# mitake/k8s

Measured on AMD Instinct MI355X. Metric: images/sec ResNet-50 TfJob (train, synthetic ImageNet), higher is better.
Workload: dtype bf16; 1 GPU; model=resnet50-v1.5, global_batch=3072, per_gpu_batch=3072, image_size=224, parallelism=dp1, optimizer=fused SGD momentum 0.9 (HIP)

## Files before the change

k8s_amd/csrc/binding/batchnorm.cpp:

```cpp
#include "binding/common.h"

namespace k8s_amd::binding {
namespace {

int bn_channels(const Tensor& x, const char* name, bool mult8) {
  check_bf16_dense(x, -1, name);
  TORCH_CHECK(x.dim() >= 1 && x.size(-1) > 0, name, ": channels last");
  const int C = (int)x.size(-1);
  TORCH_CHECK(!mult8 || C % 8 == 0, "channels must be a multiple of 8");
  return C;
}
void check_affine(const Tensor& gamma, const Tensor& beta, const Tensor& run_mean, const Tensor& run_var, long C) {
  check_channel_f32(gamma, C, "gamma"); check_channel_f32(beta, C, "beta");
  check_channel_f32(run_mean, C, "run_mean"); check_channel_f32(run_var, C, "run_var");
}
void check_bwd_vectors(const Tensor& mean, const Tensor& invstd, const Tensor& gamma, const Tensor& beta,
                       const Tensor& dgamma, const Tensor& dbeta, long C) {
  check_channel_f32(mean, C, "mean"); check_channel_f32(invstd, C, "invstd");
  check_channel_f32(gamma, C, "gamma"); check_channel_f32(beta, C, "beta");
  check_channel_f32(dgamma, C, "dgamma"); check_channel_f32(dbeta, C, "dbeta");
}
void check_same_shape(const Tensor& t, const Tensor& x, const char* name) {
  check_bf16_dense(t, -1, name);
  TORCH_CHECK(t.sizes() == x.sizes(), name, " must have the shape of x");
// ... 93 lines not shown
  if (want_link) {
    xarg = torch::empty({N, Ho, Wo, C}, x.options());
    ybits = torch::empty({(long)N * Ho * Wo * C / 8}, x.options().dtype(at::kByte));
  }
  launch_bn_relu_maxpool_fwd(cbf(x), f32(gamma), f32(beta), f32(sums), nrep, f32(mean), f32(invstd), f32(run_mean),
                             f32(run_var), f32(params), bf(y), idx.data_ptr<uint8_t>(), N, H, W, C, (float)eps,
                             (float)momentum, cur_stream(), want_link ? bf(xarg) : nullptr,
                             want_link ? ybits.data_ptr<uint8_t>() : nullptr);
  if (want_link) return {y, idx, mean, invstd, xarg, ybits};
  return {y, idx, mean, invstd};
}

Tensor pool_bn_bwd_impl(const Tensor& dpool, const Tensor& idx, const Tensor& x, const Tensor& mean,
                        const Tensor& invstd, const Tensor& gamma, const Tensor& beta, const Tensor& dgamma,
                        const Tensor& dbeta, const Tensor* sums) {
  check_bf16_dense(x, 4, "x");
  check_bf16_dense(dpool, 4, "dpool");
  check_cuda(idx, "idx"); check_dtype(idx, at::kByte, "idx");
  const int N = x.size(0), H = x.size(1), W = x.size(2), C = x.size(3);
  TORCH_CHECK(dpool.sizes() == idx.sizes() && dpool.size(0) == N && dpool.size(1) == (H + 1) / 2 &&
                  dpool.size(2) == (W + 1) / 2 && dpool.size(3) == C, "dpool / idx shape mismatch");
  check_bwd_vectors(mean, invstd, gamma, beta, dgamma, dbeta, C);
  const int nrep = sums ? check_stat_sums(*sums, C, "sums", true) : 0;
  auto dx = torch::empty_like(x);
  auto params = torch::empty({4 * C}, gamma.options());
  if (sums) {
    launch_pool_bn_bwd_from_sums(cbf(dpool), idx.data_ptr<uint8_t>(), cbf(x), f32(mean), f32(invstd), f32(gamma),
                                 f32(beta), bf(dx), f32(dgamma), f32(dbeta), f32(*sums), nrep, f32(params), N, H, W, C,
                                 cur_stream());
    return dx;
  }
  auto work = torch::empty({k8s_amd::pool_bn_workspace_floats(C)}, gamma.options());
  launch_pool_bn_bwd(cbf(dpool), idx.data_ptr<uint8_t>(), cbf(x), f32(mean), f32(invstd), f32(gamma), f32(beta), bf(dx),
                     f32(dgamma), f32(dbeta), f32(work), f32(params), N, H, W, C, cur_stream());
  return dx;
}
Tensor pool_bn_bwd_from_sums(Tensor dpool, Tensor idx, Tensor x, Tensor mean, Tensor invstd, Tensor gamma,
                             Tensor beta, Tensor dgamma, Tensor dbeta, Tensor sums) {
  return pool_bn_bwd_impl(dpool, idx, x, mean, invstd, gamma, beta, dgamma, dbeta, &sums);
}
Tensor pool_bn_bwd(Tensor dpool, Tensor idx, Tensor x, Tensor mean, Tensor invstd, Tensor gamma, Tensor beta,
                   Tensor dgamma, Tensor dbeta) {
  return pool_bn_bwd_impl(dpool, idx, x, mean, invstd, gamma, beta, dgamma, dbeta, nullptr);
}

std::vector<Tensor> bn_bwd_impl(const Tensor& dy, const Tensor& x, const OptTensor& y, const Tensor& mean,
                                const Tensor& invstd, const Tensor& gamma, const Tensor& beta, bool relu_x,
                                const Tensor& dgamma, const Tensor& dbeta, bool want_dres, const OptTensor& mask,
                                const Tensor* sums) {
  const int C = bn_channels(x, "x", false);
  const long M = x.numel() / C;
  check_same_shape(dy, x, "dy");
  check_bwd_vectors(mean, invstd, gamma, beta, dgamma, dbeta, C);
  const bool has_mask = mask && mask->defined();
  TORCH_CHECK(!(relu_x && (y || has_mask)) && !(y && has_mask), "relu_x, y and the packed mask are exclusive");
  const uint8_t* mk = has_mask ? check_bit_mask(*mask, x.numel(), "mask") : nullptr;
  const int nrep = sums ? check_stat_sums(*sums, C, "sums", false) : 0;
  Tensor ymask;
  if (y) {
    check_same_shape(*y, x, "y");
    TORCH_CHECK(x.numel() % 8 == 0, "y: a multiple of 8 elements to pack");
    ymask = relu_mask_for(x, true);
    launch_relu_mask(cbf(*y), ymask.data_ptr<uint8_t>(), x.numel() / 8, cur_stream());
    mk = ymask.data_ptr<uint8_t>();
  }
  auto dx = torch::empty_like(x);
  Tensor dres = want_dres ? torch::empty_like(x) : Tensor();
  uint16_t* dr = want_dres ? bf(dres) : nullptr;
  auto params = torch::empty({4 * C}, gamma.options());
  if (sums && mk) {
    launch_bn_bwd_from_sums(cbf(dy), cbf(x), mk, f32(*sums), nrep, f32(mean), f32(invstd), f32(gamma), f32(beta),
                            bf(dx), dr, f32(dgamma), f32(dbeta), f32(params), M, C, cur_stream());
  } else if (sums) {
    launch_bn_bwd_relu_from_sums(cbf(dy), cbf(x), f32(*sums), nrep, f32(mean), f32(invstd), f32(gamma), f32(beta),
                                 bf(dx), f32(dgamma), f32(dbeta), f32(params), M, C, cur_stream());
  } else {
    auto work = torch::empty({k8s_amd::bn_workspace_floats(M, C)}, gamma.options());
    launch_bn_bwd(cbf(dy), cbf(x), f32(mean), f32(invstd), f32(gamma), f32(beta), relu_x, bf(dx), dr, f32(dgamma),
                  f32(dbeta), f32(work), f32(params), M, C, cur_stream(), mk);
  }
  return {dx, dres};
}
std::vector<Tensor> bn_bwd(Tensor dy, Tensor x, OptTensor y, Tensor mean, Tensor invstd, Tensor gamma, Tensor beta,
                           bool relu_x, Tensor dgamma, Tensor dbeta, bool want_dres, OptTensor mask) {
  return bn_bwd_impl(dy, x, y, mean, invstd, gamma, beta, relu_x, dgamma, dbeta, want_dres, mask, nullptr);
}
std::vector<Tensor> bn_bwd_relu_from_sums(Tensor dy, Tensor x, Tensor sums, Tensor mean, Tensor invstd, Tensor gamma,
                                          Tensor beta, Tensor dgamma, Tensor dbeta) {
  return {bn_bwd_impl(dy, x, {}, mean, invstd, gamma, beta, true, dgamma, dbeta, false, {}, &sums)[0]};
}
std::vector<Tensor> bn_bwd_from_sums(Tensor dy, Tensor x, Tensor mask, Tensor sums, Tensor mean, Tensor invstd,
                                     Tensor gamma, Tensor beta, Tensor dgamma, Tensor dbeta, bool want_dres) {
  return bn_bwd_impl(dy, x, {}, mean, invstd, gamma, beta, false, dgamma, dbeta, want_dres, mask, &sums);
}

Tensor bn_bwd_params(Tensor dy, Tensor x, Tensor mask, OptTensor sums, Tensor mean, Tensor invstd, Tensor gamma,
                     Tensor beta, Tensor dgamma, Tensor dbeta) {
  const int C = bn_channels(x, "x", true);
  const long M = x.numel() / C;
  check_same_shape(dy, x, "dy");
  check_bwd_vectors(mean, invstd, gamma, beta, dgamma, dbeta, C);
  const uint8_t* mk = check_bit_mask(mask, x.numel(), "mask");
  const bool pre = sums && sums->defined();
  const int nrep = pre ? check_stat_sums(*sums, C, "sums", false) : 0;
  auto params = torch::empty({4 * C}, gamma.options());
  Tensor work;
  if (!pre) work = torch::empty({k8s_amd::bn_workspace_floats(M, C)}, gamma.options());
  launch_bn_bwd_params(cbf(dy), cbf(x), mk, pre ? f32(*sums) : nullptr, nrep, f32(mean), f32(invstd), f32(gamma),
                       f32(beta), false, f32(dgamma), f32(dbeta), pre ? nullptr : f32(work), f32(params), M, C,
                       cur_stream());
  return params;
}
Tensor bn_bwd_apply(Tensor dy, Tensor x, Tensor mask, Tensor params) {
  const int C = bn_channels(x, "x", true);
  check_same_shape(dy, x, "dy");
  const uint8_t* mk = check_bit_mask(mask, x.numel(), "mask");
  check_channel_f32(params, 4L * C, "params");
  TORCH_CHECK(params.device() == x.device(), "params: on x's device");
  auto dx = torch::empty_like(x);
  launch_bn_bwd_apply_pass(cbf(dy), cbf(x), mk, f32(params), false, bf(dx), nullptr, x.numel() / C, C, cur_stream());
  return dx;
}

std::vector<Tensor> bn_bwd_dual_impl(const Tensor& dy, const Tensor& mask, const Tensor& x, const Tensor& mean,
                                     const Tensor& invstd, const Tensor& gamma, const Tensor& beta,
                                     const Tensor& dgamma, const Tensor& dbeta, const Tensor* sums, const Tensor& x2,
                                     const Tensor& mean2, const Tensor& invstd2, const Tensor& gamma2,
                                     const Tensor& beta2, const Tensor& dgamma2, const Tensor& dbeta2,
                                     const Tensor* sums2) {
  const int C = bn_channels(x, "x", !sums);
  const long M = x.numel() / C;
  check_same_shape(dy, x, "dy");
  check_same_shape(x2, x, "x2");
  check_bwd_vectors(mean, invstd, gamma, beta, dgamma, dbeta, C);
  check_bwd_vectors(mean2, invstd2, gamma2, beta2, dgamma2, dbeta2, C);
  const uint8_t* mk = check_bit_mask(mask, x.numel(), "mask");
  const int nrep = sums ? check_stat_sums(*sums, C, "sums", false) : 0;
  TORCH_CHECK(!sums || check_stat_sums(*sums2, C, "sums2", false) == nrep, "sums / sums2: the same replica count");
  auto dx = torch::empty_like(x), dx2 = torch::empty_like(x);
  auto params = torch::empty({4 * C}, gamma.options()), params2 = torch::empty({4 * C}, gamma.options());
  if (sums) {
    launch_bn_bwd_dual_from_sums(cbf(dy), mk, cbf(x), f32(*sums), nrep, f32(mean), f32(invstd), f32(gamma), f32(beta),
                                 bf(dx), f32(dgamma), f32(dbeta), f32(params), cbf(x2), f32(*sums2), f32(mean2),
                                 f32(invstd2), f32(gamma2), f32(beta2), bf(dx2), f32(dgamma2), f32(dbeta2),
                                 f32(params2), M, C, cur_stream());
    return {dx, dx2};
  }
  auto work = torch::empty({k8s_amd::bn_workspace_floats(M, C)}, gamma.options());
  auto work2 = torch::empty({k8s_amd::bn_workspace_floats(M, C)}, gamma.options());
  launch_bn_bwd_dual(cbf(dy), mk, cbf(x), f32(mean), f32(invstd), f32(gamma), f32(beta), bf(dx), f32(dgamma),
                     f32(dbeta), f32(work), f32(params), cbf(x2), f32(mean2), f32(invstd2), f32(gamma2), f32(beta2),
                     bf(dx2), f32(dgamma2), f32(dbeta2), f32(work2), f32(params2), M, C, cur_stream());
  return {dx, dx2};
}
std::vector<Tensor> bn_bwd_dual(Tensor dy, Tensor mask, Tensor x, Tensor mean, Tensor invstd, Tensor gamma,
                                Tensor beta, Tensor dgamma, Tensor dbeta, Tensor x2, Tensor mean2, Tensor invstd2,
                                Tensor gamma2, Tensor beta2, Tensor dgamma2, Tensor dbeta2) {
  return bn_bwd_dual_impl(dy, mask, x, mean, invstd, gamma, beta, dgamma, dbeta, nullptr, x2, mean2, invstd2, gamma2,
                          beta2, dgamma2, dbeta2, nullptr);
}
std::vector<Tensor> bn_bwd_dual_from_sums(Tensor dy, Tensor mask, Tensor x, Tensor mean, Tensor invstd, Tensor gamma,
                                          Tensor beta, Tensor dgamma, Tensor dbeta, Tensor sums, Tensor x2,
                                          Tensor mean2, Tensor invstd2, Tensor gamma2, Tensor beta2, Tensor dgamma2,
                                          Tensor dbeta2, Tensor sums2) {
  return bn_bwd_dual_impl(dy, mask, x, mean, invstd, gamma, beta, dgamma, dbeta, &sums, x2, mean2, invstd2, gamma2,
                          beta2, dgamma2, dbeta2, &sums2);
}

}

void bind_batchnorm(pybind11::module_& m) {
  m.def("bn_fwd", &bn_fwd, "x"_a, "res"_a, "gamma"_a, "beta"_a, "run_mean"_a, "run_var"_a, "training"_a, "momentum"_a,
        "eps"_a, "relu"_a, "want_mask"_a = false);
  m.def("bn_bwd", &bn_bwd, "dy"_a, "x"_a, "y"_a, "mean"_a, "invstd"_a, "gamma"_a, "beta"_a, "relu_x"_a, "dgamma"_a,
        "dbeta"_a, "want_dres"_a, "mask"_a = py::none());
  m.def("bn_fwd_from_sums", &bn_fwd_from_sums, "x"_a, "res"_a, "gamma"_a, "beta"_a, "sums"_a, "run_mean"_a, "run_var"_a,
        "momentum"_a, "eps"_a, "relu"_a, "want_mask"_a = false, "want_sub2"_a = false);
  m.def("bn_bwd_dual", &bn_bwd_dual, "both BatchNorm backwards of bn_fwd_from_sums_dual from one masked dy");
  m.def("bn_fwd_from_sums_dual", &bn_fwd_from_sums_dual, "relu(BN(x) + BN_r(xr)), statistics from conv sums");
  m.def("bn_finalize", &bn_finalize, "sums"_a, "gamma"_a, "beta"_a, "run_mean"_a, "run_var"_a, "count"_a, "momentum"_a,
        "eps"_a);
  m.def("bn_bwd_relu_from_sums", &bn_bwd_relu_from_sums, "relu_x BatchNorm backward from a producer's sums");
  m.def("bn_bwd_from_sums", &bn_bwd_from_sums, "BatchNorm backward from a producer's reduction sums (final + apply)");
  m.def("bn_bwd_params", &bn_bwd_params, "dy"_a, "x"_a, "mask"_a, "sums"_a, "mean"_a, "invstd"_a, "gamma"_a, "beta"_a,
        "dgamma"_a, "dbeta"_a, "first half of a masked BatchNorm backward: dgamma, dbeta, params [sc | B | D | shift]");
  m.def("bn_bwd_apply", &bn_bwd_apply, "dy"_a, "x"_a, "mask"_a, "params"_a,
        "second half of a masked BatchNorm backward: dx from bn_bwd_params' table");
  m.def("bn_bwd_dual_from_sums", &bn_bwd_dual_from_sums, "bn_bwd_dual from a producer's reduction sums");
  m.def("bn_relu_maxpool", &bn_relu_maxpool, "x"_a, "sums"_a, "gamma"_a, "beta"_a, "run_mean"_a, "run_var"_a,
        "momentum"_a, "eps"_a, "want_link"_a = false);
  m.def("pool_bn_bwd_from_sums", &pool_bn_bwd_from_sums);
  m.def("pool_bn_bwd", &pool_bn_bwd, "dpool"_a, "idx"_a, "x"_a, "mean"_a, "invstd"_a, "gamma"_a, "beta"_a, "dgamma"_a,
        "dbeta"_a);
}

}
```

k8s_amd/csrc/binding/conv.cpp:

```cpp
#include "binding/common.h"

namespace k8s_amd::binding {
namespace {

int conv_out(int in, int k, int st, int pad, int dil) { return (in + 2 * pad - dil * (k - 1) - 1) / st + 1; }

struct ConvGeom {
  int N, H, W, C, K, R, S;
};
ConvGeom conv_geom(const Tensor& x, const Tensor& w) {
  TORCH_CHECK(x.dim() == 4 && w.dim() == 4, "x [N,H,W,C], w [K,R,S,C]");
  ConvGeom g{(int)x.size(0), (int)x.size(1), (int)x.size(2), (int)x.size(3),
             (int)w.size(0), (int)w.size(1), (int)w.size(2)};
  TORCH_CHECK(w.size(3) == g.C, "channel mismatch");
  TORCH_CHECK(g.C % 8 == 0 && g.K % 8 == 0, "implicit-GEMM conv needs C % 8 == 0 and K % 8 == 0");
  return g;
}
Tensor conv_fwd(Tensor x, Tensor w, int64_t stride, int64_t pad, int64_t dil, bool out_f32, OptTensor bias, int64_t act,
                OptTensor stats, OptTensor xform) {
  check_bf16(x, "x"); check_bf16(w, "w");
  const auto [N, H, W, C, K, R, S] = conv_geom(x, w);
  TORCH_CHECK(stride >= 1 && dil >= 1, "conv_fwd: stride >= 1, dilation >= 1");
  const int Ho = conv_out(H, R, stride, pad, dil), Wo = conv_out(W, S, stride, pad, dil);
  if (bias) check_channel_f32(*bias, K, "bias");
  if (stats) check_stat_sums(*stats, K, "stats", true);
  const float* xf = xform_ptr(xform, C);
  if (xf) TORCH_CHECK(C % 64 == 0 && !out_f32 && !bias && act == 0,
                      "normalize-on-load convolution: C % 64 == 0, bf16 output, no bias / activation");
  auto y = torch::empty({N, Ho, Wo, K}, x.options().dtype(out_f32 ? at::kFloat : at::kBFloat16));
  launch_conv_fwd(cbf(x), cbf(w), y.data_ptr(), out_f32, N, H, W, C, K, R, S, (int)stride, (int)pad, (int)dil, Ho, Wo,
                  optf(bias), (int)act, 0, stats ? f32(*stats) : nullptr, cur_stream(), nullptr, xf);
  return y;
}

Tensor conv_infer(Tensor x, Tensor w, int64_t stride, int64_t pad, Tensor scale, Tensor shift, OptTensor res,
                  bool relu, OptTensor out) {
  check_bf16_dense(x, 4, "x"); check_bf16_dense(w, 4, "w");
  const auto [N, H, W, C, K, R, S] = conv_geom(x, w);
  TORCH_CHECK(stride >= 1 && pad >= 0, "conv_infer: stride >= 1, pad >= 0");
  check_channel_f32(scale, K, "scale"); check_channel_f32(shift, K, "shift");
  TORCH_CHECK(H + 2 * pad >= R && W + 2 * pad >= S, "conv_infer: the filter does not fit the padded image");
  const int Ho = conv_out(H, R, stride, pad, 1), Wo = conv_out(W, S, stride, pad, 1);
  TORCH_CHECK((long)N * Ho * Wo < (1L << 31), "conv_infer: fewer than 2^31 output pixels");
  const std::vector<int64_t> oshape{N, Ho, Wo, K};
  if (out) {
    check_bf16_dense(*out, 4, "out");
    TORCH_CHECK(out->sizes().vec() == oshape, "out must be [N, Ho, Wo, K]");
  }
  if (res) {
    check_bf16_dense(*res, 4, "res");
    TORCH_CHECK(res->sizes().vec() == oshape, "res must have the output's shape [N, Ho, Wo, K]");
  }
  Tensor y = out ? *out : torch::empty(oshape, x.options());
  launch_conv_infer(cbf(x), cbf(w), bf(y), N, H, W, C, K, R, S, (int)stride, (int)pad, Ho, Wo, f32(scale), f32(shift),
                    res ? cbf(*res) : nullptr, relu, cur_stream());
  return y;
}

void conv_fwd_subgrid(Tensor x, Tensor w, int64_t pad, int64_t Hs, int64_t Ws, Tensor out, int64_t stride, int64_t a,
                      int64_t b, bool accumulate, OptTensor bn_x, OptTensor bn_mask, OptTensor bn_mean,
                      OptTensor bn_sums, OptTensor bn_gamma, OptTensor bn_beta, OptTensor bn_invstd) {
  check_bf16(x, "x"); check_bf16(w, "w"); check_bf16(out, "out");
  const auto [N, H, W, C, K, R, S] = conv_geom(x, w);
  TORCH_CHECK(out.dim() == 4 && out.size(0) == N && out.size(3) == K, "out shape");
  const int OH = out.size(1), OW = out.size(2);
  TORCH_CHECK(stride >= 1 && a >= 0 && a < stride && b >= 0 && b < stride, "parity out of range");
  TORCH_CHECK(Hs >= 1 && Ws >= 1 && (Hs - 1) * stride + a < OH && (Ws - 1) * stride + b < OW,
              "sub-grid exceeds the output image");
  k8s_amd::SubGrid sg{OH, OW, (int)stride, (int)a, (int)b};
  k8s_amd::BnBwdSums bb;
  if (bn_sums) {
    TORCH_CHECK(bn_x && bn_mean, "bn sums: bn_x and bn_mean");
    TORCH_CHECK(bn_mask ? accumulate : !accumulate,
                "bn sums: bn_mask + accumulate (a correction) or bn_gamma / bn_beta / bn_invstd + a plain store");
    TORCH_CHECK(bn_x->sizes() == out.sizes(), "bn_x: the shape of out");
    bb = bn_bwd_sums(*bn_x, *bn_mean, *bn_sums, bn_mask, bn_gamma, bn_beta, bn_invstd, {}, {}, {});
  }
  launch_conv_fwd(cbf(x), cbf(w), out.data_ptr(), false, N, H, W, C, K, R, S, 1, (int)pad, 1, (int)Hs, (int)Ws, nullptr,
                  0, accumulate ? 1 : 0, nullptr, cur_stream(), &sg, nullptr, bn_sums ? &bb : nullptr);
}

Tensor conv3x3_dgrad_bnstats(Tensor gy, Tensor wt, Tensor x, Tensor gamma, Tensor beta, Tensor mean, Tensor invstd,
                             Tensor sums) {
  check_bf16_dense(gy, 4, "gy"); check_bf16_dense(wt, 4, "wt"); check_bf16_dense(x, 4, "x");
  const int N = (int)gy.size(0), H = (int)gy.size(1), W = (int)gy.size(2), Kc = (int)gy.size(3);
  const int C = (int)wt.size(0);
  TORCH_CHECK(wt.size(1) == 3 && wt.size(2) == 3 && wt.size(3) == Kc, "wt: [C, 3, 3, K]");
  TORCH_CHECK(x.size(0) == N && x.size(1) == H && x.size(2) == W && x.size(3) == C, "x: the shape of dx");
  TORCH_CHECK(k8s_amd::conv3x3_eligible(H, W, Kc, C, 3, 3, 1, 1, 1), "conv3x3_dgrad_bnstats: outside the kernel");
  const k8s_amd::BnBwdSums bb = bn_bwd_sums(x, mean, sums, {}, gamma, beta, invstd, {}, {}, {});
  Tensor dx = torch::empty({N, H, W, C}, gy.options());
  launch_conv3x3(cbf(gy), cbf(wt), bf(dx), nullptr, nullptr, N, H, W, Kc, C, cur_stream(), &bb);
  return dx;
}

Tensor bwd1x1_fused(Tensor gy, Tensor x, Tensor w, Tensor xform, Tensor gamma, Tensor beta, Tensor mean, Tensor invstd,
                    Tensor dw, Tensor sums, bool accumulate, OptTensor x3, OptTensor mask, OptTensor params) {
  check_bf16_dense(gy, 2, "gy"); check_bf16_dense(x, 2, "x"); check_bf16_dense(w, 2, "w");
  const long M = gy.size(0), K = gy.size(1), C = x.size(1);
  TORCH_CHECK(x.size(0) == M && w.size(0) == K && w.size(1) == C, "shapes: gy [M, K], x [M, C], w [K, C]");
  TORCH_CHECK(k8s_amd::bwd1x1_fused_ok(M, (int)C, (int)K),
              "bwd1x1_fused: (C, K) = (64, 256) or (128, 512), 1 <= M < 2^31");
  check_cuda(dw, "dw"); check_dtype(dw, at::kFloat, "dw"); check_aligned(dw, "dw");
  TORCH_CHECK(dw.numel() == K * C, "dw must have K * C fp32 elements");
  check_channel_f32(xform, 2 * C, "xform (BatchNorm scale | shift)");
  const k8s_amd::BnBwdSums bb = bn_bwd_sums(x, mean, sums, {}, gamma, beta, invstd, {}, {}, {});
  k8s_amd::Bwd1x1Bn3 bn3;
  const bool onload = x3 || mask || params;
  if (onload) {
    TORCH_CHECK(x3 && mask && params, "bwd1x1_fused: x3, mask and params come together");
    check_bf16_dense(*x3, 2, "x3");
    TORCH_CHECK(x3->size(0) == M && x3->size(1) == K, "x3: the shape of gy, [M, K]");
    bn3.mask = check_bit_mask(*mask, M * K, "mask");
    check_aligned(*mask, "mask");
    check_cuda(*params, "params"); check_dtype(*params, at::kFloat, "params"); check_aligned(*params, "params");
    TORCH_CHECK(params->numel() >= 3 * K, "params: fp32 [sc | B | D], 3K elements or more");
    TORCH_CHECK(x3->device() == gy.device() && mask->device() == gy.device() && params->device() == gy.device(),
                "x3, mask and params: on gy's device");
    bn3.x3 = cbf(*x3);
    bn3.params = f32(*params);
  }
  Tensor dz = torch::empty({M, C}, gy.options());
  launch_bwd1x1_fused(cbf(gy), cbf(x), cbf(w), f32(xform), bb.gamma, bb.beta, bb.mean, bb.invstd, bf(dz), f32(dw),
                      bb.sums, M, (int)C, (int)K, accumulate, cur_stream(), onload ? &bn3 : nullptr);
  return dz;
}

void conv_wgrad(Tensor x, Tensor dy, Tensor dw, int64_t stride, int64_t pad, int64_t dil, int64_t splits,
                bool accumulate, OptTensor xform) {
  check_bf16(x, "x"); check_bf16(dy, "dy");
  check_cuda(dw, "dw"); check_dtype(dw, at::kFloat, "dw");
  const auto [N, H, W, C, K, R, S] = conv_geom(x, dw);
  TORCH_CHECK(stride >= 1 && dil >= 1, "conv_wgrad: stride >= 1, dilation >= 1");
  const int Ho = conv_out(H, R, stride, pad, dil), Wo = conv_out(W, S, stride, pad, dil);
  TORCH_CHECK(dy.dim() == 4 && dy.size(0) == N && dy.size(1) == Ho && dy.size(2) == Wo && dy.size(3) == K,
              "dy shape mismatch");
  const float* xf = xform_ptr(xform, C);
  if (dil == 1 && Ho == H && Wo == W && H == W && k8s_amd::wgrad3x3_tiled_ok(C, K, R, S, (int)stride, (int)pad, W)) {
    auto wsp = torch::empty({k8s_amd::wgrad3x3_tiled_workspace(N, H, W, C)}, dw.options());
    launch_wgrad3x3_tiled(cbf(x), cbf(dy), f32(wsp), f32(dw), N, H, W, C, accumulate, cur_stream(), xf);
    return;
  }
  if (!xf && dil == 1 && k8s_amd::wgrad_stream_eligible(N, Ho, Wo, C, K, R, S)) {
    launch_wgrad_stream(cbf(x), cbf(dy), f32(dw), N, H, W, C, K, R, S, (int)stride, (int)pad, Ho, Wo, accumulate,
                        cur_stream());
    return;
  }
  if (xf) TORCH_CHECK(C % 64 == 0, "normalize-on-load weight gradient needs C % 64 == 0");
  int sp = splits <= 0 ? k8s_amd::gemm_choose_splits(K, R * S * C, N * Ho * Wo) : (int)splits;
  Tensor ws;
  if (sp > 1) ws = torch::empty({k8s_amd::gemm_splitk_workspace(K, R * S * C, sp)}, dw.options());
  launch_conv_wgrad(cbf(x), cbf(dy), f32(dw), N, H, W, C, K, R, S, (int)stride, (int)pad, (int)dil, Ho, Wo, sp,
                    accumulate, sp > 1 ? f32(ws) : nullptr, cur_stream(), xf);
}

std::vector<Tensor> conv_dgrad_wsub(Tensor w, std::vector<std::vector<int64_t>> taps) {
  check_bf16(w, "w");
  TORCH_CHECK(w.dim() == 4, "w [K,R,S,C]");
  const int K = w.size(0), R = w.size(1), S = w.size(2), C = w.size(3);
  TORCH_CHECK(!taps.empty() && taps.size() <= 16, "1-16 parities");
  k8s_amd::DgradTaps t{};
  long off = 0;
  std::vector<int64_t> offs;
  for (size_t p = 0; p < taps.size(); ++p) {
    TORCH_CHECK(!taps[p].empty() && taps[p].size() <= 16, "1-16 taps per parity");
    t.n[p] = (int)taps[p].size();
    t.off[p] = off;
    offs.push_back(off);
    for (size_t i = 0; i < taps[p].size(); ++i) {
      TORCH_CHECK(taps[p][i] >= 0 && taps[p][i] < R * S, "tap index out of range");
      t.rs[p][i] = (int)taps[p][i];
    }
    off += (long)C * t.n[p] * K;
    off = (off + 7) / 8 * 8;
  }
  auto out = torch::empty({off}, w.options());
  launch_conv_dgrad_wsub(cbf(w), bf(out), K, R * S, C, t, (int)taps.size(), cur_stream());
  return {out, torch::tensor(offs)};
}
Tensor conv_dgrad_wtrans(Tensor w) {
  check_bf16(w, "w");
  TORCH_CHECK(w.dim() == 4, "w [K,R,S,C]");
  const int K = w.size(0), R = w.size(1), S = w.size(2), C = w.size(3);
  auto w2 = torch::empty({C, R, S, K}, w.options());
  launch_conv_dgrad_wtrans(cbf(w), bf(w2), K, R, S, C, cur_stream());
  return w2;
}

}

void bind_conv(pybind11::module_& m) {
  m.def("conv_fwd", &conv_fwd, "x"_a, "w"_a, "stride"_a, "pad"_a, "dil"_a, "out_f32"_a, "bias"_a, "act"_a, "stats"_a,
        "xform"_a = py::none());
  m.def("conv_infer", &conv_infer, "x"_a, "w"_a, "stride"_a, "pad"_a, "scale"_a, "shift"_a, "res"_a = py::none(),
        "relu"_a = true, "out"_a = py::none());
  m.def("conv3x3_staged_ok", [](int H, int W, int C, int K, int R, int S, int stride, int pad) {
    return k8s_amd::conv3x3_eligible(H, W, C, K, R, S, stride, pad, 1) &&
           k8s_amd::conv3x3_eligible(H, W, K, C, R, S, stride, pad, 1) &&
           k8s_amd::wgrad3x3_tiled_ok(C, K, R, S, stride, pad, W);
  });
  m.def("conv3x3_dgrad_bnstats", &conv3x3_dgrad_bnstats,
        "3x3 stride-1 data gradient with the BatchNorm-backward sums of a relu(BN(x)) input (conv3x3.hip)");
  m.def("conv_fwd_subgrid", &conv_fwd_subgrid, "x"_a, "w"_a, "pad"_a, "Hs"_a, "Ws"_a, "out"_a, "stride"_a, "a"_a, "b"_a,
        "accumulate"_a = false, "bn_x"_a = py::none(), "bn_mask"_a = py::none(), "bn_mean"_a = py::none(),
        "bn_sums"_a = py::none(), "bn_gamma"_a = py::none(), "bn_beta"_a = py::none(), "bn_invstd"_a = py::none());
  m.def("conv_wgrad", &conv_wgrad, "x"_a, "dy"_a, "dw"_a, "stride"_a, "pad"_a, "dil"_a, "splits"_a, "accumulate"_a,
        "xform"_a = py::none());
  m.def("bwd1x1_fused", &bwd1x1_fused, "gy"_a, "x"_a, "w"_a, "xform"_a, "gamma"_a, "beta"_a, "mean"_a, "invstd"_a,
        "dw"_a, "sums"_a, "accumulate"_a, "x3"_a = py::none(), "mask"_a = py::none(), "params"_a = py::none(),
        "1x1 data gradient, normalize-on-load weight gradient and BatchNorm-backward sums in one pass (bwd1x1_fused.hip)");
  m.def("bwd1x1_fused_ok", [](int64_t M, int64_t C, int64_t K) {
    return C <= 1024 && K <= 4096 && k8s_amd::bwd1x1_fused_ok(M, (int)C, (int)K);
  }, "M"_a, "C"_a, "K"_a, "whether bwd1x1_fused takes this shape");
  m.def("wgrad_stream_eligible",&k8s_amd::wgrad_stream_eligible, "tall-K weight-gradient kernel takes this shape");
  m.def("conv_dgrad_wtrans", &conv_dgrad_wtrans);
  m.def("conv_dgrad_wsub", &conv_dgrad_wsub);
}

}
```

k8s_amd/csrc/kernels/batchnorm.hip:

```cpp
#include <cstdlib>
#include <stdexcept>

#include "common.h"
#include "launchers.h"

namespace k8s_amd {


constexpr int BN_THREADS = 256;

struct BnGeom {
  int cgroups;
  int tpr;
  int rows_per_iter;
  int grid_y;
};

static inline BnGeom bn_geom(int C, long M) {
  BnGeom g;
  g.cgroups = C / 8;
  g.tpr = g.cgroups < BN_THREADS ? g.cgroups : BN_THREADS;
  const long cus = planner_cus();
  long nbx = M / 64;
  nbx = nbx < 1 ? 1 : (nbx > 4 * cus ? 4 * cus : nbx);
// ... 710 lines not shown

int stream_order_mode() { return 1; }
int stream_dir(int fixed) { return fixed; }

static long bn_rows_per_block(long M, const BnGeom& g) {
  long blocks_x = 4L * planner_cus() / g.grid_y;
  const long cap = M / 64;
  if (blocks_x > cap) blocks_x = cap;
  if (blocks_x < 1) blocks_x = 1;
  long rpb = (M + blocks_x - 1) / blocks_x;
  long minr = (long)g.rows_per_iter * 4;
  if (rpb < minr) rpb = minr;
  rpb = (rpb + g.rows_per_iter - 1) / g.rows_per_iter * g.rows_per_iter;
  return rpb;
}

static int bn_reduce_blocks(long M, const BnGeom& g) {
  long nb = 4L * planner_cus() / g.grid_y;
  const long groups = (M + g.rows_per_iter - 1) / g.rows_per_iter;
  if (nb > groups) nb = groups;
  if (stream_order_mode()) nb = nb < 8 ? 8 : nb & ~7L;
  return (int)(nb < 1 ? 1 : nb);
}

int bn_workspace_floats(long M, int C) {
  BnGeom g = bn_geom(C, M);
  long rpb = bn_rows_per_block(M, g);
  long nb = (M + rpb - 1) / rpb;
  const long nr = bn_reduce_blocks(M, g);
  return (int)((nb > nr ? nb : nr) * C * 2);
}

static void launch_bn_apply(const uint16_t* x, const uint16_t* res, const float* params, uint16_t* y, uint8_t* mask,
                            long M, int C, bool relu, hipStream_t st, const float* rparams = nullptr,
                            uint16_t* ysub = nullptr, int H = 1, int W = 1) {
  const long nvec = M * C / 8;
  if (nvec >= (1L << 31)) throw std::runtime_error("BatchNorm tensor too large (>= 2^31 vectors)");
  if (ysub && (M % ((long)H * W) != 0)) throw std::runtime_error("bn_apply subsample: M must be N * H * W");
  hipLaunchKernelGGL(bn_apply_kernel, dim3(cdiv(nvec, BN_THREADS)), dim3(BN_THREADS), 0, st, x, res, params, rparams,
                     y, mask, (int)nvec, C, make_fastdiv(C / 8), (int)relu,
                     stream_order_mode() ? (stream_dir(1) ? 1 : 2) : 0, ysub, make_fastdiv(W), make_fastdiv(H));
}

void launch_bn_fwd(const uint16_t* x, const uint16_t* res, const float* gamma, const float* beta, uint16_t* y,
                   float* save_mean, float* save_invstd, float* run_mean, float* run_var, float* work, float* params,
                   long M, int C, float eps, float momentum, bool training, bool relu, hipStream_t st,
                   uint8_t* mask) {
  if (training) {
    BnGeom g = bn_geom(C, M);
    long rpb = bn_rows_per_block(M, g);
    int nb = (int)((M + rpb - 1) / rpb);
    hipLaunchKernelGGL(bn_stats_kernel, dim3(nb, g.grid_y), dim3(BN_THREADS), 0, st, x, M, C, g.tpr,
                       g.rows_per_iter, rpb, work);
    hipLaunchKernelGGL(bn_stats_final_kernel, dim3(cdiv(C, FIN_CH)), dim3(256), 0, st, work, nb, M, rpb, C, eps,
                       momentum, save_mean, save_invstd, run_mean, run_var, gamma, beta, params);
  } else {
    hipLaunchKernelGGL(bn_eval_prep_kernel, dim3(cdiv(C, 256)), dim3(256), 0, st, run_mean, run_var, gamma, beta, C,
                       eps, save_mean, save_invstd, params);
  }
  launch_bn_apply(x, res, params, y, mask, M, C, relu, st);
}

void launch_bn_fwd_from_sums(const uint16_t* x, const uint16_t* res, const float* gamma, const float* beta,
                             uint16_t* y, const float* sums, int nrep, float* save_mean, float* save_invstd,
                             float* run_mean, float* run_var, float* params, long M, int C, float eps, float momentum,
                             bool relu, hipStream_t st, uint8_t* mask, uint16_t* ysub, int H, int W) {
  hipLaunchKernelGGL(bn_finalize_sums_kernel, dim3(cdiv(C, 256)), dim3(256), 0, st, sums, nrep, C, (float)M, eps,
                     momentum, save_mean, save_invstd, run_mean, run_var, gamma, beta, params);
  launch_bn_apply(x, res, params, y, mask, M, C, relu, st, nullptr, ysub, H, W);
}

void launch_bn_fwd_from_sums_dual(const uint16_t* x, const float* gamma, const float* beta, const float* sums,
                                  int nrep, float* save_mean, float* save_invstd, float* run_mean, float* run_var,
                                  float* params, const uint16_t* xr, const float* gamma_r, const float* beta_r,
                                  const float* sums_r, int nrep_r, float* save_mean_r, float* save_invstd_r,
                                  float* run_mean_r, float* run_var_r, float* params_r, uint16_t* y, uint8_t* mask,
                                  long M, int C, float eps, float momentum, hipStream_t st) {
  hipLaunchKernelGGL(bn_finalize_sums_kernel, dim3(cdiv(C, 256)), dim3(256), 0, st, sums, nrep, C, (float)M, eps,
                     momentum, save_mean, save_invstd, run_mean, run_var, gamma, beta, params);
  hipLaunchKernelGGL(bn_finalize_sums_kernel, dim3(cdiv(C, 256)), dim3(256), 0, st, sums_r, nrep_r, C, (float)M, eps,
                     momentum, save_mean_r, save_invstd_r, run_mean_r, run_var_r, gamma_r, beta_r, params_r);
  launch_bn_apply(x, xr, params, y, mask, M, C, true, st, params_r);
}

void launch_bn_finalize_sums(const float* gamma, const float* beta, const float* sums, int nrep, float* save_mean,
                             float* save_invstd, float* run_mean, float* run_var, float* params, long M, int C,
                             float eps, float momentum, hipStream_t st) {
  hipLaunchKernelGGL(bn_finalize_sums_kernel, dim3(cdiv(C, 256)), dim3(256), 0, st, sums, nrep, C, (float)M, eps,
                     momentum, save_mean, save_invstd, run_mean, run_var, gamma, beta, params);
}

static void launch_bn_bwd_apply(const uint16_t* dy, const uint16_t* x, const uint8_t* mask, const float* params,
                                bool relu_x, uint16_t* dx, uint16_t* dres, long M, int C, hipStream_t st,
                                int order = -1) {
  const long nvec = M * C / 8;
  if (nvec >= (1L << 31)) throw std::runtime_error("BatchNorm tensor too large (>= 2^31 vectors)");
  if (order < 0) order = stream_order_mode() ? (stream_dir(0) ? 1 : 2) : 0;
  hipLaunchKernelGGL(bn_bwd_apply_kernel, dim3(cdiv(nvec, BN_THREADS)), dim3(BN_THREADS), 0, st, dy, x, mask, params,
                     (int)relu_x, dx, dres, (int)nvec, C, make_fastdiv(C / 8), order);
}

void launch_bn_bwd_params(const uint16_t* dy, const uint16_t* x, const uint8_t* mask, const float* sums, int nrep,
                          const float* mean, const float* invstd, const float* gamma, const float* beta, bool relu_x,
                          float* dgamma, float* dbeta, float* work, float* params, long M, int C, hipStream_t st) {
  if (sums) {
    hipLaunchKernelGGL(bn_bwd_final_sums_kernel, dim3(cdiv(C, 256)), dim3(256), 0, st, sums, sums, nrep, C, dgamma,
                       dbeta, 1.f / (float)M, mean, invstd, gamma, beta, params);
    return;
  }
  BnGeom g = bn_geom(C, M);
  const int nb = bn_reduce_blocks(M, g);
  const int rdir = stream_dir(1);
  if (mask)
    hipLaunchKernelGGL(bn_bwd_reduce_kernel<true>, dim3(nb, g.grid_y), dim3(BN_THREADS), 0, st, dy, x, mean, invstd,
                       gamma, beta, (int)relu_x, M, C, g.tpr, g.rows_per_iter, work, mask, rdir);
  else
    hipLaunchKernelGGL(bn_bwd_reduce_kernel<false>, dim3(nb, g.grid_y), dim3(BN_THREADS), 0, st, dy, x, mean, invstd,
                       gamma, beta, (int)relu_x, M, C, g.tpr, g.rows_per_iter, work, mask, rdir);
  hipLaunchKernelGGL(bn_bwd_final_kernel, dim3(cdiv(C, FIN_CH)), dim3(256), 0, st, work, nb, C, dgamma, dbeta,
                     1.f / (float)M, mean, invstd, gamma, beta, params);
}

void launch_bn_bwd_apply_pass(const uint16_t* dy, const uint16_t* x, const uint8_t* mask, const float* params,
                              bool relu_x, uint16_t* dx, uint16_t* dres, long M, int C, hipStream_t st) {
  launch_bn_bwd_apply(dy, x, mask, params, relu_x, dx, dres, M, C, st);
}

void launch_bn_bwd(const uint16_t* dy, const uint16_t* x, const float* mean, const float* invstd, const float* gamma,
                   const float* beta, bool relu_x, uint16_t* dx, uint16_t* dres, float* dgamma, float* dbeta,
                   float* work, float* params, long M, int C, hipStream_t st, const uint8_t* mask) {
  launch_bn_bwd_params(dy, x, mask, nullptr, 0, mean, invstd, gamma, beta, relu_x, dgamma, dbeta, work, params, M, C,
                       st);
  launch_bn_bwd_apply(dy, x, mask, params, relu_x, dx, dres, M, C, st);
}

void launch_bn_bwd_from_sums(const uint16_t* dy, const uint16_t* x, const uint8_t* mask, const float* sums, int nrep,
                             const float* mean, const float* invstd, const float* gamma, const float* beta,
                             uint16_t* dx, uint16_t* dres, float* dgamma, float* dbeta, float* params, long M, int C,
                             hipStream_t st) {
  launch_bn_bwd_params(dy, x, mask, sums, nrep, mean, invstd, gamma, beta, false, dgamma, dbeta, nullptr, params, M,
                       C, st);
  launch_bn_bwd_apply(dy, x, mask, params, false, dx, dres, M, C, st);
}

void launch_bn_bwd_relu_from_sums(const uint16_t* dy, const uint16_t* x, const float* sums, int nrep,
                                  const float* mean, const float* invstd, const float* gamma, const float* beta,
                                  uint16_t* dx, float* dgamma, float* dbeta, float* params, long M, int C,
                                  hipStream_t st) {
  hipLaunchKernelGGL(bn_bwd_final_sums_kernel, dim3(cdiv(C, 256)), dim3(256), 0, st, sums, sums, nrep, C, dgamma,
                     dbeta, 1.f / (float)M, mean, invstd, gamma, beta, params);
  launch_bn_bwd_apply(dy, x, nullptr, params, true, dx, nullptr, M, C, st);
}

void launch_bn_bwd_dual_from_sums(const uint16_t* dy, const uint8_t* mask, const uint16_t* x, const float* sums,
                                  int nrep, const float* mean, const float* invstd, const float* gamma,
                                  const float* beta, uint16_t* dx, float* dgamma, float* dbeta, float* params,
                                  const uint16_t* x2, const float* sums2, const float* mean2, const float* invstd2,
                                  const float* gamma2, const float* beta2, uint16_t* dx2, float* dgamma2,
                                  float* dbeta2, float* params2, long M, int C, hipStream_t st) {
  hipLaunchKernelGGL(bn_bwd_final_sums_kernel, dim3(cdiv(C, 256)), dim3(256), 0, st, sums, sums, nrep, C, dgamma,
                     dbeta, 1.f / (float)M, mean, invstd, gamma, beta, params);
  hipLaunchKernelGGL(bn_bwd_final_sums_kernel, dim3(cdiv(C, 256)), dim3(256), 0, st, sums, sums2, nrep, C, dgamma2,
                     dbeta2, 1.f / (float)M, mean2, invstd2, gamma2, beta2, params2);
  const long nvec = M * C / 8;
  if (nvec >= (1L << 31)) throw std::runtime_error("BatchNorm tensor too large (>= 2^31 vectors)");
  hipLaunchKernelGGL(bn_bwd_apply_dual_kernel, dim3(cdiv(nvec, BN_THREADS)), dim3(BN_THREADS), 0, st, dy, mask, x,
                     params, dx, x2, params2, dx2, (int)nvec, C, make_fastdiv(C / 8),
                     stream_order_mode() ? (stream_dir(0) ? 1 : 2) : 0);
}

void launch_bn_bwd_dual(const uint16_t* dy, const uint8_t* mask, const uint16_t* x, const float* mean,
                        const float* invstd, const float* gamma, const float* beta, uint16_t* dx, float* dgamma,
                        float* dbeta, float* work, float* params, const uint16_t* x2, const float* mean2,
                        const float* invstd2, const float* gamma2, const float* beta2, uint16_t* dx2, float* dgamma2,
                        float* dbeta2, float* work2, float* params2, long M, int C, hipStream_t st) {
  BnGeom g = bn_geom(C, M);
  const int nb = bn_reduce_blocks(M, g);
  const int rdir = stream_dir(1);
  hipLaunchKernelGGL((bn_bwd_reduce_kernel<true, true>), dim3(nb, g.grid_y), dim3(BN_THREADS), 0, st, dy, x, mean,
                     invstd, gamma, beta, 0, M, C, g.tpr, g.rows_per_iter, work, mask, rdir, x2, mean2, invstd2, work2);
  hipLaunchKernelGGL(bn_bwd_final_kernel, dim3(cdiv(C, FIN_CH)), dim3(256), 0, st, work, nb, C, dgamma, dbeta,
                     1.f / (float)M, mean, invstd, gamma, beta, params);
  hipLaunchKernelGGL(bn_bwd_final_kernel, dim3(cdiv(C, FIN_CH)), dim3(256), 0, st, work2, nb, C, dgamma2, dbeta2,
                     1.f / (float)M, mean2, invstd2, gamma2, beta2, params2);
  const long nvec = M * C / 8;
  if (nvec >= (1L << 31)) throw std::runtime_error("BatchNorm tensor too large (>= 2^31 vectors)");
  hipLaunchKernelGGL(bn_bwd_apply_dual_kernel, dim3(cdiv(nvec, BN_THREADS)), dim3(BN_THREADS), 0, st, dy, mask, x,
                     params, dx, x2, params2, dx2, (int)nvec, C, make_fastdiv(C / 8),
                     stream_order_mode() ? (stream_dir(0) ? 1 : 2) : 0);
}

void launch_bn_relu_maxpool_fwd(const uint16_t* x, const float* gamma, const float* beta, const float* sums, int nrep,
                                float* save_mean, float* save_invstd, float* run_mean, float* run_var, float* params,
                                uint16_t* y, uint8_t* idx, int N, int H, int W, int C, float eps, float momentum,
                                hipStream_t st, uint16_t* xarg, uint8_t* ybits) {
  const int Ho = (H + 1) / 2, Wo = (W + 1) / 2;
  const long total = (long)N * Ho * Wo * (C / 8);
  if ((long)N * H * W * C / 8 >= (1L << 31)) throw std::runtime_error("bn_relu_maxpool: tensor too large");
  hipLaunchKernelGGL(bn_finalize_sums_kernel, dim3(cdiv(C, 256)), dim3(256), 0, st, sums, nrep, C,
                     (float)((long)N * H * W), eps, momentum, save_mean, save_invstd, run_mean, run_var, gamma, beta,
                     params);
  hipLaunchKernelGGL(bn_relu_maxpool_fwd_kernel, dim3(cdiv(total, BN_THREADS)), dim3(BN_THREADS), 0, st, x, params,
                     y, idx, H, W, C, Ho, Wo, (int)total, make_fastdiv(C / 8), make_fastdiv(Wo), make_fastdiv(Ho),
                     xarg, ybits);
}

int pool_bn_workspace_floats(int C) { return 4096 * C * 2; }

void launch_pool_bn_bwd(const uint16_t* dpool, const uint8_t* idx, const uint16_t* x, const float* mean,
                        const float* invstd, const float* gamma, const float* beta, uint16_t* dx, float* dgamma,
                        float* dbeta, float* work, float* params, int N, int H, int W, int C, hipStream_t st) {
  if (C % 8 || BN_THREADS % (C / 8)) throw std::runtime_error("pool_bn_bwd: C / 8 must divide 256");
  const int Ho = (H + 1) / 2, Wo = (W + 1) / 2, Hc = (H + 1) / 2, Wc = (W + 1) / 2;
  const long ncells = (long)N * Hc * Wc;
  if (ncells * (C / 8) >= (1L << 31)) throw std::runtime_error("pool_bn_bwd: tensor too large");
  const int cpb = BN_THREADS / (C / 8);
  long nb = (ncells + cpb - 1) / cpb;
  nb = std::min(nb, 16L * planner_cus());
  hipLaunchKernelGGL(pool_bn_bwd_reduce_kernel, dim3((unsigned)nb), dim3(BN_THREADS), 0, st, dpool, idx, x, mean,
                     invstd, gamma, beta, H, W, C, Ho, Wo, Hc, Wc, (int)ncells, work, make_fastdiv(Wc),
                     make_fastdiv(Hc));
  hipLaunchKernelGGL(bn_bwd_final_kernel, dim3(cdiv(C, FIN_CH)), dim3(256), 0, st, work, (int)nb, C, dgamma, dbeta,
                     1.f / (float)((long)N * H * W), mean, invstd, gamma, beta, params);
  const long total = ncells * (C / 8);
  hipLaunchKernelGGL(pool_bn_bwd_apply_kernel, dim3(cdiv(total, BN_THREADS)), dim3(BN_THREADS), 0, st, dpool, idx, x,
                     params, dx, H, W, C, Ho, Wo, (int)total, make_fastdiv(C / 8), make_fastdiv(Wc),
                     make_fastdiv(Hc));
}

void launch_pool_bn_bwd_from_sums(const uint16_t* dpool, const uint8_t* idx, const uint16_t* x, const float* mean,
                                  const float* invstd, const float* gamma, const float* beta, uint16_t* dx,
                                  float* dgamma, float* dbeta, const float* sums, int nrep, float* params, int N,
                                  int H, int W, int C, hipStream_t st) {
  if (C % 8 || BN_THREADS % (C / 8)) throw std::runtime_error("pool_bn_bwd: C / 8 must divide 256");
  const int Ho = (H + 1) / 2, Wo = (W + 1) / 2, Hc = (H + 1) / 2, Wc = (W + 1) / 2;
  const long ncells = (long)N * Hc * Wc;
  if (ncells * (C / 8) >= (1L << 31)) throw std::runtime_error("pool_bn_bwd: tensor too large");
  hipLaunchKernelGGL(bn_bwd_final_sums_kernel, dim3(cdiv(C, 256)), dim3(256), 0, st, sums, sums, nrep, C, dgamma,
                     dbeta, 1.f / (float)((long)N * H * W), mean, invstd, gamma, beta, params);
  const long total = ncells * (C / 8);
  hipLaunchKernelGGL(pool_bn_bwd_apply_kernel, dim3(cdiv(total, BN_THREADS)), dim3(BN_THREADS), 0, st, dpool, idx, x,
                     params, dx, H, W, C, Ho, Wo, (int)total, make_fastdiv(C / 8), make_fastdiv(Wc),
                     make_fastdiv(Hc));
}

__global__ void __launch_bounds__(BN_THREADS) relu_mask_kernel(const uint16_t* __restrict__ y,
                                                               uint8_t* __restrict__ mask, int nvec) {
  const int e = blockIdx.x * BN_THREADS + threadIdx.x;
  if (e < nvec) mask[e] = relu_bits(*reinterpret_cast<const bf16x8_t*>(y + (long)e * 8));
}

void launch_relu_mask(const uint16_t* y, uint8_t* mask, long nvec, hipStream_t st) {
  if (nvec >= (1L << 31)) throw std::runtime_error("tensor too large (>= 2^31 vectors)");
  hipLaunchKernelGGL(relu_mask_kernel, dim3(cdiv(nvec, BN_THREADS)), dim3(BN_THREADS), 0, st, y, mask, (int)nvec);
}

__global__ void __launch_bounds__(BN_THREADS) mask_apply_kernel(const uint16_t* __restrict__ src,
                                                                const uint8_t* __restrict__ mask,
                                                                uint16_t* __restrict__ out, int nvec) {
  const int e = blockIdx.x * BN_THREADS + threadIdx.x;
  if (e >= nvec) return;
  bf16x8_t v = *reinterpret_cast<const bf16x8_t*>(src + (long)e * 8);
  const uint32_t bits = mask[e];
#pragma unroll
  for (int r = 0; r < 8; ++r) v[r] = ((bits >> r) & 1u) ? v[r] : (short)0;
  *reinterpret_cast<bf16x8_t*>(out + (long)e * 8) = v;
}

void launch_mask_apply(const uint16_t* src, const uint8_t* mask, uint16_t* out, long n, hipStream_t st) {
  if (n % 8) throw std::runtime_error("mask_apply: element count must be a multiple of 8");
  const long nvec = n / 8;
  if (nvec >= (1L << 31)) throw std::runtime_error("tensor too large (>= 2^31 vectors)");
  hipLaunchKernelGGL(mask_apply_kernel, dim3(cdiv(nvec, BN_THREADS)), dim3(BN_THREADS), 0, st, src, mask, out,
                     (int)nvec);
}

}
```

k8s_amd/csrc/kernels/bwd1x1_fused.hip:

```cpp
#include <algorithm>
#include <stdexcept>

#include "common.h"
#include "launchers.h"
#include "mfma.h"

namespace k8s_amd {
namespace b1f {

constexpr int THREADS = 512;
constexpr int CT = 64;

__device__ __attribute__((aligned(64))) uint16_t g_zero16[64];

typedef __attribute__((ext_vector_type(4))) int int4_t;

__device__ __forceinline__ int swz128(int r) { return 2 * (((r >> 1) & 1) | (((r >> 3) & 1) << 1)); }
__device__ __forceinline__ int swz_g(int r) { return (2 * ((r & 3) | (((r >> 3) & 1) << 2))) | ((r >> 2) & 1); }

struct TrRaw {
  short4_t lo, hi;
};
template <int RB, bool G>
__device__ __forceinline__ void tr_load(TrRaw& r, const char* img, int rb, int kk, int lane) {
  const int g = lane >> 4, i = lane & 15, q = i >> 2, p = i & 3;
  const int u = (rb >> 3) + (p >> 1);
  const int r0 = kk * 32 + 8 * g + q, r1 = r0 + 4;
  const int u0 = u ^ (G ? swz_g(r0) : swz128(r0)), u1 = u ^ (G ? swz_g(r1) : swz128(r1));
  tr16_asm(r.lo, img + r0 * RB + (u0 << 4) + (p & 1) * 8);
  tr16_asm(r.hi, img + r1 * RB + (u1 << 4) + (p & 1) * 8);
}
#define K8S_LDS_TIE4(w, a, b, c, d) asm volatile(w : "+v"(a), "+v"(b), "+v"(c), "+v"(d))

struct Args {
  const uint16_t *gy, *x, *w;
  const uint16_t* x3;
  const uint8_t* mask;
  const float* params;
  const float *xform, *gamma, *beta, *mean, *invstd;
  uint16_t* dz;
  float* dw;
  float* sums;
  int M, C, ntiles, npairs;
};

__device__ __forceinline__ void lds_barrier() {
  asm volatile("s_waitcnt lgkmcnt(0)" ::: "memory");
  __builtin_amdgcn_s_barrier();
  asm volatile("" ::: "memory");
}

template <int K, int RS, int NSLOT, int HALVES, bool ONLOAD>
__global__ void __launch_bounds__(THREADS, 1) bwd1x1_fused_kernel(Args a) {
  constexpr int RB = K * 2, UG = K / 8;
  constexpr int IMG_G = RS * RB, IMG_X = RS * 128;
  constexpr int IMG_M = ONLOAD ? RS * UG : 0;
  constexpr int OFF_X = IMG_G + (ONLOAD ? IMG_G + IMG_M : 0);
  constexpr int STAGE = OFF_X + IMG_X, RING = NSLOT * STAGE;
  constexpr int LG = RS * UG / THREADS;
  constexpr int LPS = ONLOAD ? 2 * LG : LG;
  constexpr bool TREG = ONLOAD && (THREADS / UG) % 16 == 0;
  constexpr bool TLDS = ONLOAD && !TREG;
  static_assert(!ONLOAD || (IMG_M % 1024 == 0 && IMG_M / 1024 <= THREADS / 64), "mask tile: whole 1-KB wave loads");
  constexpr int XT = RS * 8;
  constexpr int NKS = K / 32, KW = K / 8, KTW = KW / 16;
  static_assert(LG * THREADS == RS * UG && XT % 64 == 0 && XT <= THREADS && (RS == 32 || RS == 64), "tile");
  static_assert(XT * 64 <= RING, "sums partials reuse the ring");
  constexpr bool PLDS = K > 256;
  __shared__ __attribute__((aligned(1024))) char smem[RING + IMG_X + (PLDS ? 5 * CT * 4 : 0) + (TLDS ? 3 * K * 4 : 0)];
  static_assert(sizeof(smem) <= 160 * 1024, "LDS");
  char* stg = smem + RING;
  float* ptab = reinterpret_cast<float*>(stg + IMG_X);
  float* btab = ptab + (PLDS ? 5 * CT : 0);

  const int tid = threadIdx.x, lane = tid & 63;
  const int wid = __builtin_amdgcn_readfirstlane(tid >> 6);
  const int bid = blockIdx.x;
  int pair = bid, chalf = 0;
  if constexpr (HALVES == 2) {
    const int slot = bid >> 3;
    chalf = slot & 1;
    pair = (slot >> 1) * 8 + (bid & 7);
  }
  const int c0 = chalf * CT;
  const int n = pair < a.ntiles ? (a.ntiles - pair + a.npairs - 1) / a.npairs : 0;
  if (n == 0) return;
  const long M = a.M;
  const int C = a.C;

  const int ct = wid & 3, rh = wid >> 2;
  int4_t wf[NKS];
  {
    const uint16_t* wp = a.w + (long)(8 * (lane >> 4)) * C + c0 + ct * 16 + (lane & 15);
#pragma unroll
    for (int ks = 0; ks < NKS; ++ks) {
      bf16x8_t v;
#pragma unroll
      for (int j = 0; j < 8; ++j) v[j] = (short)wp[(long)(ks * 32 + j) * C];
      wf[ks] = __builtin_bit_cast(int4_t, v);
    }
  }
  const int erow = tid >> 3;
  const int eu = (tid & 7) ^ swz128(erow);
  const int ecol = c0 + eu * 8;
  float xsc[8], xsh[8], gsc[8], gsh[8], mu[8], ps[8], pq[8];
#pragma unroll
  for (int j = 0; j < 8; ++j) {
    xsc[j] = a.xform[ecol + j];
    xsh[j] = a.xform[C + ecol + j];
    mu[j] = a.mean[ecol + j];
    bn_affine_regs(a.gamma[ecol + j], a.beta[ecol + j], mu[j], a.invstd[ecol + j], gsc[j], gsh[j]);
    ps[j] = pq[j] = 0.f;
  }
  if constexpr (PLDS) {
    if (tid < 8) {
#pragma unroll
      for (int j = 0; j < 8; ++j) {
        ptab[0 * CT + tid * 8 + j] = xsc[j];
        ptab[1 * CT + tid * 8 + j] = xsh[j];
        ptab[2 * CT + tid * 8 + j] = gsc[j];
        ptab[3 * CT + tid * 8 + j] = gsh[j];
        ptab[4 * CT + tid * 8 + j] = mu[j];
      }
    }
  }
  const int tup = tid % UG, trow = tid / UG;
  float tsc[8], tB[8], tD[8];
  if constexpr (TREG) {
    const float* t = a.params + (tup ^ swz_g(trow)) * 8;
#pragma unroll
    for (int j = 0; j < 8; ++j) {
      tsc[j] = t[j];
      tB[j] = t[K + j];
      tD[j] = t[2 * K + j];
    }
#pragma unroll
    for (int j = 0; j < 8; ++j) asm volatile("" : "+v"(tsc[j]), "+v"(tB[j]), "+v"(tD[j]));
  }
  if constexpr (TLDS) {
    static_assert(!TLDS || PLDS, "the table's stores are ordered by the PLDS barrier");
    for (int i = tid; i < 3 * K; i += THREADS) btab[i] = a.params[i];
  }
#pragma unroll
  for (int ks = 0; ks < NKS; ++ks) asm volatile("" : "+v"(wf[ks]));
  if constexpr (!PLDS) {
#pragma unroll
    for (int j = 0; j < 8; ++j) asm volatile("" : "+v"(xsc[j]), "+v"(xsh[j]), "+v"(gsc[j]), "+v"(gsh[j]), "+v"(mu[j]));
  } else {
    __syncthreads();
  }

  auto issue = [&](int slot, int i) {
    char* st = smem + slot * STAGE;
    const long m0 = (long)(pair + i * a.npairs) * RS;
    if constexpr (ONLOAD) {
      const unsigned last = (unsigned)min((long)RS - 1, M - 1 - m0);
      const uint16_t* gb = a.gy + m0 * K;
      const uint16_t* xb = a.x3 + m0 * K;
#pragma unroll
      for (int j = 0; j < LG; ++j) {
        const unsigned row = j * (THREADS / UG) + trow;
        const unsigned off = min(row, last) * K + (tup ^ swz_g(row)) * 8;
        glds16(gb + off, st + j * (THREADS * 16) + wid * 1024);
        glds16(xb + off, st + IMG_G + j * (THREADS * 16) + wid * 1024);
      }
      if (wid < IMG_M / 1024) {
        const unsigned q = (wid * 64 + lane) * 16;
        glds16(a.mask + m0 * UG + min(q / UG, last) * UG + q % UG, st + 2 * IMG_G + wid * 1024);
      }
      if (wid < XT / 64) glds16(a.x + m0 * C + min((unsigned)erow, last) * C + ecol, st + OFF_X + wid * 1024);
      return;
    }
#pragma unroll
    for (int j = 0; j < LG; ++j) {
      const int sl = j * THREADS + tid, row = sl / UG, up = sl % UG;
      const int u = up ^ swz_g(row);
      const long m = m0 + row;
      const void* src = m < M ? (const void*)(a.gy + m * K + u * 8) : (const void*)g_zero16;
      glds16(src, st + j * (THREADS * 16) + wid * 1024);
    }
    if (wid < XT / 64) {
      const long m = m0 + erow;
      const void* src = m < M ? (const void*)(a.x + m * C + ecol) : (const void*)g_zero16;
      glds16(src, st + OFF_X + wid * 1024);
    }
  };

  f32x4_t dwa[KTW][4];
#pragma unroll
  for (int i = 0; i < KTW; ++i)
#pragma unroll
    for (int j = 0; j < 4; ++j) dwa[i][j] = f32x4_t{0.f, 0.f, 0.f, 0.f};

  const int pre = min(n, NSLOT - 1);
  for (int s = 0; s < pre; ++s) issue(s, s);
  int slot = 0;
  for (int s = 0; s < n; ++s) {
    const int younger = min(n - 1, s + NSLOT - 2) - s;
    if (younger >= 2) asm volatile("s_waitcnt vmcnt(%0)" ::"n"(2 * LPS) : "memory");
    else if (younger == 1) asm volatile("s_waitcnt vmcnt(%0)" ::"n"(LPS) : "memory");
    else asm volatile("s_waitcnt vmcnt(0)" ::: "memory");
    lds_barrier();
    if (s + NSLOT - 1 < n) issue(slot == 0 ? NSLOT - 1 : slot - 1, s + NSLOT - 1);
    char* G = smem + slot * STAGE;
    char* X = G + OFF_X;

    if constexpr (ONLOAD) {
      const int last = (int)min((long)RS - 1, M - 1 - (long)(pair + s * a.npairs) * RS);
#pragma unroll
      for (int j = 0; j < LG; ++j) {
        const int row = j * (THREADS / UG) + trow;
        const int u = tup ^ swz_g(row);
        char* gp = G + j * (THREADS * 16) + tid * 16;
        const bf16x8_t gv = *reinterpret_cast<const bf16x8_t*>(gp);
        const bf16x8_t xv = *reinterpret_cast<const bf16x8_t*>(gp + IMG_G);
        const uint32_t bits = *reinterpret_cast<const uint8_t*>(G + 2 * IMG_G + row * UG + u);
        float o[8];
#pragma unroll
        for (int h = 0; h < 8; h += 4) {
          if constexpr (TLDS) {
            const float* t = btab + u * 8 + h;
#pragma unroll
            for (int i = 0; i < 4; ++i) {
              tsc[h + i] = t[i];
              tB[h + i] = t[K + i];
              tD[h + i] = t[2 * K + i];
            }
          }
#pragma unroll
          for (int i = h; i < h + 4; ++i) {
            const float g = (bits >> i) & 1u ? bf2f((uint16_t)gv[i]) : 0.f;
            o[i] = __builtin_fmaf(tsc[i], g, __builtin_fmaf(tB[i], bf2f((uint16_t)xv[i]), tD[i]));
            o[i] = row <= last ? o[i] : 0.f;
          }
          if constexpr (TLDS) asm volatile("" ::: "memory");
        }
        *reinterpret_cast<bf16x8_t*>(gp) = pack_bf16x8(o);
      }
      lds_barrier();
    }

    {
      f32x4_t d0 = {0.f, 0.f, 0.f, 0.f}, d1 = {0.f, 0.f, 0.f, 0.f};
      const int row0 = rh * (RS / 2) + (lane & 15);
      const int kq = lane >> 4;
      if constexpr (RS == 64) {
        const int row1 = row0 + 16;
        const char* p0 = G + row0 * RB;
        const char* p1 = G + row1 * RB;
        const int s0 = swz_g(row0), s1 = swz_g(row1);
#pragma unroll
        for (int ks = 0; ks < NKS; ++ks) {
          const bf16x8_t b0 = *reinterpret_cast<const bf16x8_t*>(p0 + (((ks * 4 + kq) ^ s0) << 4));
          const bf16x8_t b1 = *reinterpret_cast<const bf16x8_t*>(p1 + (((ks * 4 + kq) ^ s1) << 4));
          const mfma_bf16x8 wa = __builtin_bit_cast(mfma_bf16x8, wf[ks]);
          d0 = mfma16(wa, __builtin_bit_cast(mfma_bf16x8, b0), d0);
          d1 = mfma16(wa, __builtin_bit_cast(mfma_bf16x8, b1), d1);
        }
      } else {
        const char* p0 = G + row0 * RB;
        const int s0 = swz_g(row0);
#pragma unroll
        for (int ks = 0; ks < NKS; ks += 2) {
          const bf16x8_t b0 = *reinterpret_cast<const bf16x8_t*>(p0 + (((ks * 4 + kq) ^ s0) << 4));
          const bf16x8_t b1 = *reinterpret_cast<const bf16x8_t*>(p0 + (((ks * 4 + 4 + kq) ^ s0) << 4));
          d0 = mfma16(__builtin_bit_cast(mfma_bf16x8, wf[ks]), __builtin_bit_cast(mfma_bf16x8, b0), d0);
          d1 = mfma16(__builtin_bit_cast(mfma_bf16x8, wf[ks + 1]), __builtin_bit_cast(mfma_bf16x8, b1), d1);
        }
        d0 += d1;
      }
      const int unit = ct * 2 + (lane >> 5), half = (lane >> 4) & 1;
      auto put = [&](int row, const f32x4_t& d) {
        bf16x4_t o;
#pragma unroll
        for (int r = 0; r < 4; ++r) o[r] = (short)f2bf(d[r]);
        *reinterpret_cast<bf16x4_t*>(stg + row * 128 + ((unit ^ swz128(row)) << 4) + half * 8) = o;
      };
      put(row0, d0);
      if constexpr (RS == 64) put(row0 + 16, d1);
    }
    lds_barrier();

    if (wid < XT / 64) {
      const bf16x8_t dzv = *reinterpret_cast<const bf16x8_t*>(stg + tid * 16);
      const bf16x8_t xv = *reinterpret_cast<const bf16x8_t*>(X + tid * 16);
      if constexpr (PLDS) {
        const float* t = ptab + (ecol - c0);
#pragma unroll
        for (int j = 0; j < 8; ++j) {
          xsc[j] = t[j];
          xsh[j] = t[CT + j];
          gsc[j] = t[2 * CT + j];
          gsh[j] = t[3 * CT + j];
          mu[j] = t[4 * CT + j];
        }
      }
      float o[8];
#pragma unroll
      for (int j = 0; j < 8; ++j) {
        const float xf = bf2f((uint16_t)xv[j]);
        o[j] = fmaxf(__builtin_fmaf(xf, xsc[j], xsh[j]), 0.f);
        const float g = relu_on(xf, gsc[j], gsh[j]) ? bf2f((uint16_t)dzv[j]) : 0.f;
        ps[j] += g;
        pq[j] = __builtin_fmaf(g, xf - mu[j], pq[j]);
      }
      *reinterpret_cast<bf16x8_t*>(X + tid * 16) = pack_bf16x8(o);
      const long m = (long)(pair + s * a.npairs) * RS + erow;
      if (m < M) *reinterpret_cast<bf16x8_t*>(a.dz + m * C + ecol) = dzv;
    }
    lds_barrier();

#pragma unroll
    for (int kk = 0; kk < RS / 32; ++kk) {
      TrRaw ar[KTW], br[4];
#pragma unroll
      for (int j = 0; j < 4; ++j) tr_load<128, false>(br[j], X, j * 16, kk, lane);
#pragma unroll
      for (int i = 0; i < KTW; ++i) tr_load<RB, true>(ar[i], G, wid * KW + i * 16, kk, lane);
      K8S_LDS_TIE8("s_waitcnt lgkmcnt(0)", br[0].lo, br[0].hi, br[1].lo, br[1].hi, br[2].lo, br[2].hi, br[3].lo,
                   br[3].hi);
#pragma unroll
      for (int i = 0; i < KTW; i += 2)
        K8S_LDS_TIE4("s_waitcnt lgkmcnt(0)", ar[i].lo, ar[i].hi, ar[i + 1].lo, ar[i + 1].hi);
#pragma unroll
      for (int i = 0; i < KTW; ++i)
#pragma unroll
        for (int j = 0; j < 4; ++j)
          dwa[i][j] = __builtin_amdgcn_mfma_f32_16x16x32_bf16(join8(br[j].lo, br[j].hi), join8(ar[i].lo, ar[i].hi),
                                                              dwa[i][j], 0, 0, 0);
    }
    slot = slot + 1 == NSLOT ? 0 : slot + 1;
  }

#pragma unroll
  for (int i = 0; i < KTW; ++i) {
    const int k = wid * KW + i * 16 + (lane & 15);
#pragma unroll
    for (int j = 0; j < 4; ++j) {
      float* d = a.dw + (long)k * C + c0 + j * 16 + 4 * (lane >> 4);
#pragma unroll
      for (int r = 0; r < 4; ++r) atomicAdd(d + r, dwa[i][j][r]);
    }
  }
  __syncthreads();
  float* part = reinterpret_cast<float*>(smem);
  if (tid < XT) {
#pragma unroll
    for (int j = 0; j < 8; ++j) {
      part[tid * 16 + j] = ps[j];
      part[tid * 16 + 8 + j] = pq[j];
    }
  }
  __syncthreads();
  if (tid < 2 * CT) {
    const int col = tid & (CT - 1), which = tid / CT;
    const int u = col >> 3, r = col & 7;
    float v = 0.f;
#pragma unroll 4
    for (int row = 0; row < RS; ++row) v += part[(row * 8 + (u ^ swz128(row))) * 16 + which * 8 + r];
    atomicAdd(a.sums + (long)(bid % kConvStatReplicas) * 2 * C + (long)which * C + c0 + col, v);
  }
}

}

bool bwd1x1_fused_ok(long M, int C, int K) {
  return M >= 1 && M < (1L << 31) && ((C == 64 && K == 256) || (C == 128 && K == 512));
}

void launch_bwd1x1_fused(const uint16_t* gy, const uint16_t* x, const uint16_t* w, const float* xform,
                         const float* gamma, const float* beta, const float* mean, const float* invstd, uint16_t* dz,
                         float* dw, float* sums, long M, int C, int K, bool accumulate, hipStream_t st,
                         const Bwd1x1Bn3* bn3) {
  using namespace b1f;
  if (!bwd1x1_fused_ok(M, C, K)) throw std::runtime_error("bwd1x1_fused: (C, K) = (64, 256) or (128, 512), M < 2^31");
  if (bn3 && !(bn3->x3 && bn3->mask && bn3->params)) throw std::runtime_error("bwd1x1_fused: x3, mask and params");
  if (!accumulate) (void)hipMemsetAsync(dw, 0, (size_t)K * C * sizeof(float), st);
  Args a{gy, x, w, nullptr, nullptr, nullptr, xform, gamma, beta, mean, invstd, dz, dw, sums, (int)M, C, 0, 0};
  if (bn3) a.x3 = bn3->x3, a.mask = bn3->mask, a.params = bn3->params;
  const int cus = std::max(1, planner_cus());
  if (C == 64) {
    a.ntiles = (int)((M + 63) / 64);
    a.npairs = cus;
    if (bn3) hipLaunchKernelGGL((bwd1x1_fused_kernel<256, 64, 2, 1, true>), dim3(cus), dim3(THREADS), 0, st, a);
    else hipLaunchKernelGGL((bwd1x1_fused_kernel<256, 64, 3, 1, false>), dim3(cus), dim3(THREADS), 0, st, a);
  } else {
    const int grid = std::max(16, cus / 16 * 16);
    a.ntiles = (int)((M + 31) / 32);
    a.npairs = grid / 2;
    if (bn3) hipLaunchKernelGGL((bwd1x1_fused_kernel<512, 32, 2, 2, true>), dim3(grid), dim3(THREADS), 0, st, a);
    else hipLaunchKernelGGL((bwd1x1_fused_kernel<512, 32, 4, 2, false>), dim3(grid), dim3(THREADS), 0, st, a);
  }
}

}
```

k8s_amd/csrc/kernels/launchers.h:

```cpp
#pragma once
#include <hip/hip_runtime.h>
#include <stdint.h>

#include "rng.h"

namespace k8s_amd {

int planner_cus();
void set_planner_cus(int n);

void launch_sgd(float* p, float* mom, const void* g, bool g_bf16, uint16_t* pbf, long n, const uint8_t* decay_mask, float lr,
                float mu, float wd, float scale, const float* scale_ptr, const float* hyper, bool nesterov,
                bool first_step, hipStream_t st);
void launch_adam(float* p, float* m1, float* m2, const void* g, bool g_bf16, uint16_t* pbf, long n, const uint8_t* decay_mask,
                 float lr, float b1, float b2, float eps, float wd, float scale, const float* scale_ptr,
                 const float* hyper, float bc1, float bc2, bool decoupled, hipStream_t st);
void launch_sumsq(const void* g, bool g_bf16, long n, float* out, hipStream_t st);
void launch_clip_factor(const float* stats, float max_norm, float* factor, hipStream_t st);
void launch_slice_sum(const uint16_t* in, long n, int world, float* out, uint16_t* out_bf, hipStream_t st);
void launch_cast_bf16(const float* in, uint16_t* out, long n, hipStream_t st);

void launch_grad_accumulate(float* acc, const float* g, long n, bool first, hipStream_t st);
void launch_grad_fold(float* g, const float* acc, uint16_t* out_bf, long n, hipStream_t st);

constexpr int kLayerItemMax = 16384;
void launch_layer_sums(const long* items, int n_items, const float* p, float* m1, float* m2, const void* g,
                       bool g_bf16, const uint8_t* flags, float* partial, bool lamb, float b1, float b2, float eps,
                       float wd, float scale, const float* scale_ptr, const float* hyper, float bc1, float bc2,
                       hipStream_t st);
void launch_layer_fold(const float* partial, const int* seg_start, int n_seg, float* sums, const float* scale_ptr,
                       hipStream_t st);
void launch_layer_ratio(const float* sums, const uint8_t* flags, int n_seg, float* ratio, bool lamb, float eta,
                        float wd, const float* scale_ptr, hipStream_t st);
void launch_layer_update(const long* items, int n_items, float* p, float* m1, const float* m2, const void* g,
                         bool g_bf16, uint16_t* pbf, const uint8_t* flags, const float* ratio, bool lamb, float lr,
                         float mu, float b1, float b2, float eps, float wd, float scale, const float* scale_ptr,
                         const float* hyper, float bc1, float bc2, bool first_step, hipStream_t st);

int bn_workspace_floats(long M, int C);
void launch_bn_fwd(const uint16_t* x, const uint16_t* res, const float* gamma, const float* beta, uint16_t* y,
                   float* save_mean, float* save_invstd, float* run_mean, float* run_var, float* work, float* params,
                   long M, int C, float eps, float momentum, bool training, bool relu, hipStream_t st,
                   uint8_t* mask = nullptr);
void launch_bn_fwd_from_sums(const uint16_t* x, const uint16_t* res, const float* gamma, const float* beta,
                             uint16_t* y, const float* sums, int nrep, float* save_mean, float* save_invstd,
                             float* run_mean, float* run_var, float* params, long M, int C, float eps, float momentum,
                             bool relu, hipStream_t st, uint8_t* mask = nullptr, uint16_t* ysub = nullptr,
                             int H = 1, int W = 1);
void launch_bn_fwd_from_sums_dual(const uint16_t* x, const float* gamma, const float* beta, const float* sums,
                                  int nrep, float* save_mean, float* save_invstd, float* run_mean, float* run_var,
                                  float* params, const uint16_t* xr, const float* gamma_r, const float* beta_r,
                                  const float* sums_r, int nrep_r, float* save_mean_r, float* save_invstd_r,
                                  float* run_mean_r, float* run_var_r, float* params_r, uint16_t* y, uint8_t* mask,
                                  long M, int C, float eps, float momentum, hipStream_t st);
void launch_bn_bwd_from_sums(const uint16_t* dy, const uint16_t* x, const uint8_t* mask, const float* sums, int nrep,
                             const float* mean, const float* invstd, const float* gamma, const float* beta,
                             uint16_t* dx, uint16_t* dres, float* dgamma, float* dbeta, float* params, long M, int C,
                             hipStream_t st);
void launch_bn_bwd_relu_from_sums(const uint16_t* dy, const uint16_t* x, const float* sums, int nrep,
                                  const float* mean, const float* invstd, const float* gamma, const float* beta,
                                  uint16_t* dx, float* dgamma, float* dbeta, float* params, long M, int C,
                                  hipStream_t st);
void launch_bn_bwd_dual_from_sums(const uint16_t* dy, const uint8_t* mask, const uint16_t* x, const float* sums,
                                  int nrep, const float* mean, const float* invstd, const float* gamma,
                                  const float* beta, uint16_t* dx, float* dgamma, float* dbeta, float* params,
                                  const uint16_t* x2, const float* sums2, const float* mean2, const float* invstd2,
                                  const float* gamma2, const float* beta2, uint16_t* dx2, float* dgamma2,
                                  float* dbeta2, float* params2, long M, int C, hipStream_t st);
void launch_bn_bwd_dual(const uint16_t* dy, const uint8_t* mask, const uint16_t* x, const float* mean,
                        const float* invstd, const float* gamma, const float* beta, uint16_t* dx, float* dgamma,
                        float* dbeta, float* work, float* params, const uint16_t* x2, const float* mean2,
                        const float* invstd2, const float* gamma2, const float* beta2, uint16_t* dx2, float* dgamma2,
                        float* dbeta2, float* work2, float* params2, long M, int C, hipStream_t st);
void launch_bn_finalize_sums(const float* gamma, const float* beta, const float* sums, int nrep, float* save_mean,
                             float* save_invstd, float* run_mean, float* run_var, float* params, long M, int C,
                             float eps, float momentum, hipStream_t st);
constexpr int kConvStatReplicas = 32;
void launch_bn_bwd(const uint16_t* dy, const uint16_t* x, const float* mean, const float* invstd, const float* gamma,
                   const float* beta, bool relu_x, uint16_t* dx, uint16_t* dres, float* dgamma, float* dbeta,
                   float* work, float* params, long M, int C, hipStream_t st, const uint8_t* mask = nullptr);
void launch_bn_bwd_params(const uint16_t* dy, const uint16_t* x, const uint8_t* mask, const float* sums, int nrep,
                          const float* mean, const float* invstd, const float* gamma, const float* beta, bool relu_x,
                          float* dgamma, float* dbeta, float* work, float* params, long M, int C, hipStream_t st);
void launch_bn_bwd_apply_pass(const uint16_t* dy, const uint16_t* x, const uint8_t* mask, const float* params,
                              bool relu_x, uint16_t* dx, uint16_t* dres, long M, int C, hipStream_t st);
void launch_relu_mask(const uint16_t* y, uint8_t* mask, long nvec, hipStream_t st);

void launch_norm_fwd(bool rms, const uint16_t* x, const uint16_t* res, uint16_t* xsum, const float* gamma,
                     const float* beta, uint16_t* y, float* mean, float* rstd, long R, int D, float eps,
                     hipStream_t st, const DropArgs* drop = nullptr);
int norm_workspace_floats(long R, int D);
void launch_norm_bwd(bool rms, const uint16_t* dy, const uint16_t* x, const float* gamma, const float* mean,
                     const float* rstd, const uint16_t* dres, uint16_t* dx, float* dgamma, float* dbeta, float* work,
                     long R, int D, hipStream_t st, float* dsum = nullptr, const DropArgs* drop = nullptr,
                     uint16_t* da = nullptr);

void launch_dropout(const uint16_t* x, uint16_t* y, long R, int D, const DropArgs& dr, hipStream_t st);
void launch_dropout_mask(uint8_t* out, long row0, long R, int C, const DropArgs& dr, hipStream_t st);

void launch_xent_fwd(const void* logits, bool bf16, const int64_t* labels, long R, long V, long ld, float* loss,
                     float* lse, long ignore_index, float smoothing, hipStream_t st);
void launch_xent_bwd(const void* logits, bool bf16, const int64_t* labels, const float* lse, const float* dscale,
                     bool per_row, long R, long V, long ld, void* dlogits, long ignore_index, float smoothing,
                     hipStream_t st);
void launch_xent_eval(const void* logits, bool bf16, const int64_t* labels, long R, long V, long ld, float* loss,
                      int* rank, long ignore_index, hipStream_t st);

int gemm_choose_splits(int M, int N, int K);
struct AddEpi {
  const uint16_t* src;
  const uint8_t* mask;
};
bool gemm_short_ok(int M, int N, int K, long lda, long ldc);
bool gemm_short_bnstats_ok(int M, int N, int K, bool dual);
struct BnBwdSums {
  const uint16_t* x = nullptr;
  const float* gamma = nullptr;
  const float* beta = nullptr;
  const float* mean = nullptr;
  const float* invstd = nullptr;
  float* sums = nullptr;
  const uint8_t* mask = nullptr;
  const uint16_t* x2 = nullptr;
  const float* mean2 = nullptr;
  float* sums2 = nullptr;
};
struct GemmShortBnStats {
  const uint16_t* x = nullptr;
  const uint8_t* mask = nullptr;
  const float* mean = nullptr;
  float* sums = nullptr;
  const uint16_t* x2 = nullptr;
  const float* mean2 = nullptr;
  float* sums2 = nullptr;
};
void launch_gemm_short(const uint16_t* A, const uint16_t* B, long ldb, bool b_mn, uint16_t* C, const uint16_t* add,
                       const uint8_t* mask, const float* xf, float* stats, int M, int N, int K, int epi,
                       hipStream_t st, const GemmShortBnStats* bst = nullptr);
void launch_gemm_dgrad_bnstats(const uint16_t* A, const uint16_t* B, uint16_t* C, int M, int N, int K,
                               const BnBwdSums& bb, hipStream_t st, bool accumulate = false,
                               const uint16_t* add_src = nullptr, const uint8_t* add_mask = nullptr);
void launch_gemm(const uint16_t* A, long lda, bool a_kmajor, const uint16_t* B, long ldb, bool b_kmajor, void* C,
                 long ldc, bool c_f32, int M, int N, int K, const float* bias, int act, uint16_t* pre, int mode,
                 float alpha, int splits, float* ws, hipStream_t st, const AddEpi* add = nullptr,
                 const float* xform_b = nullptr, int xform_c = 0);
void launch_mask_apply(const uint16_t* src, const uint8_t* mask, uint16_t* out, long n, hipStream_t st);
long gemm_splitk_workspace(int M, int N, int splits);
bool conv3x3_eligible(int H, int W, int C, int K, int R, int S, int stride, int pad, int dil);
void launch_conv3x3(const uint16_t* x, const uint16_t* w, uint16_t* y, float* stats, const float* xform, int N,
                    int H, int W, int C, int K, hipStream_t st,
                    const BnBwdSums* bsums = nullptr);
bool gemm256_eligible(int M, int N, int K, bool a_kmajor, bool b_kmajor);
int gemm256_choose_splits(int M, int N, int K);
bool gemm_w4_dact_ok(int M, int N, int K, long lda, long ldb, long ldc);
long gemm_w4_dact_part_floats(int M, int N);
void launch_gemm_w4_dact(const uint16_t* A, long lda, const uint16_t* B, long ldb, uint16_t* C, long ldc, int M, int N,
                         int K, const uint16_t* pre, int act, float* part, float* db, bool db_accumulate,
                         float* sk_slabs, int* sk_sync, hipStream_t st);
bool gemm_w4_swiglu_ok(int M, int F, int K, long lda, long ldb);
void launch_gemm_w4_swiglu_bwd(const uint16_t* A, long lda, const uint16_t* B, long ldb, uint16_t* dgu,
                               const uint16_t* gu, int M, int F, int K, int blk, float* sk_slabs, int* sk_sync,
                               hipStream_t st);
bool gemm_w4_stats_ok(int M, int N, int K);
bool gemm_w4_dgrad_bnstats_ok(int M, int N, int K);
void launch_gemm_w4_dgrad_bnstats(const uint16_t* A, const uint16_t* B, uint16_t* y, int M, int N, int K,
                                  const uint16_t* x, const float* tab, float* sums, float* sk_slabs, int* sk_sync,
                                  hipStream_t st);
void launch_gemm_w4_stats(const uint16_t* A, long lda, const uint16_t* B, long ldb, uint16_t* y, int M, int N, int K,
                          float* stats, float* sk_slabs, int* sk_sync, hipStream_t st);
bool gemm_w4_rope_ok(int M, int N, int K, long lda, long ldb, int rot_cols);
void launch_gemm_w4_rope(const uint16_t* A, long lda, const uint16_t* B, long ldb, uint16_t* y, int M, int N, int K,
                         const int* pos, const float* table, int rot_cols, float* sk_slabs, int* sk_sync,
                         hipStream_t st);
bool gemm_w4_swiglu_fwd_ok(int M, int F, int K, long lda, long ldb);
void launch_gemm_w4_swiglu_fwd(const uint16_t* A, long lda, const uint16_t* B, long ldb, uint16_t* gu, uint16_t* h,
                               int M, int F, int K, float* sk_slabs, int* sk_sync, hipStream_t st);
struct Gemm256Plan {
  int tiles, full, sk, kps;
};
Gemm256Plan gemm256_plan(int M, int N, int K);
long gemm256_sk_slab_floats(const Gemm256Plan& p);
long gemm256_sk_sync_ints(const Gemm256Plan& p);
void launch_gemm256(const uint16_t* A, long lda, bool a_kmajor, const uint16_t* B, long ldb, bool b_kmajor, void* C,
                    long ldc, bool c_f32, int M, int N, int K, const float* bias, int act, uint16_t* pre,
                    bool accumulate, float alpha, hipStream_t st, int splits = 1, float* ws = nullptr,
                    float* sk_slabs = nullptr, int* sk_sync = nullptr);
struct SubGrid {
  int H, W, stride, a, b;
};
void launch_conv_fwd(const uint16_t* x, const uint16_t* w, void* y, bool y_f32, int N, int H, int W, int C, int K,
                     int R, int S, int stride, int pad, int dil, int Ho, int Wo, const float* bias, int act,
                     int mode, float* stats, hipStream_t st, const SubGrid* sg = nullptr, const float* xform = nullptr,
                     const BnBwdSums* bb = nullptr);
void launch_conv_infer(const uint16_t* x, const uint16_t* w, uint16_t* y, int N, int H, int W, int C, int K, int R,
                       int S, int stride, int pad, int Ho, int Wo, const float* scale, const float* shift,
                       const uint16_t* res, bool relu, hipStream_t st);
void launch_conv_wgrad(const uint16_t* x, const uint16_t* dy, float* dw, int N, int H, int W, int C, int K, int R,
                       int S, int stride, int pad, int dil, int Ho, int Wo, int splits, bool accumulate, float* ws,
                       hipStream_t st, const float* xform = nullptr);
bool wgrad_stream_eligible(int N, int Ho, int Wo, int C, int K, int R, int S);
void launch_wgrad_stream(const uint16_t* x, const uint16_t* dy, float* dw, int N, int H, int W, int C, int K, int R,
                         int S, int stride, int pad, int Ho, int Wo, bool accumulate, hipStream_t st);
struct Bwd1x1Bn3 {
  const uint16_t* x3 = nullptr;
  const uint8_t* mask = nullptr;
  const float* params = nullptr;
};
bool bwd1x1_fused_ok(long M, int C, int K);
void launch_bwd1x1_fused(const uint16_t* gy, const uint16_t* x, const uint16_t* w, const float* xform,
                         const float* gamma, const float* beta, const float* mean, const float* invstd, uint16_t* dz,
                         float* dw, float* sums, long M, int C, int K, bool accumulate, hipStream_t st,
                         const Bwd1x1Bn3* bn3 = nullptr);
void launch_conv_dgrad_wtrans(const uint16_t* w, uint16_t* w2, int K, int R, int S, int C, hipStream_t st);
struct DgradTaps {
  int n[16];
  long off[16];
  int rs[16][16];
};
void launch_conv_dgrad_wsub(const uint16_t* w, uint16_t* out, int K, int RS, int C, const DgradTaps& taps, int np,
                            hipStream_t st);

void launch_swiglu_fwd(const uint16_t* gu, uint16_t* y, long T, int F, int blk, hipStream_t st);
void launch_swiglu_bwd(const uint16_t* gu, const uint16_t* dy, uint16_t* dgu, long T, int F, int blk, hipStream_t st);
void launch_rope(uint16_t* x, long ld, const int* pos, const float* table, long T, int H, int D, bool inverse,
                 hipStream_t st);
void launch_gelu_bwd(const uint16_t* dy, const uint16_t* pre, uint16_t* dx, long n, hipStream_t st);
void launch_relu_bwd(const uint16_t* dy, const uint16_t* y, uint16_t* dx, long n, hipStream_t st);
int colsum_workspace_floats(long R, int C);
void launch_colsum(const uint16_t* x, long R, int C, float* work, float* out, bool accumulate, hipStream_t st);
void launch_colsum_fold(float* part, int P, int C, float* out, bool accumulate, hipStream_t st);
void launch_colsum_group(float* part, int P, int C, int gs, hipStream_t st);
void launch_act_bwd_colsum(int act, const uint16_t* dy, const uint16_t* pre, uint16_t* g, long R, int C, float* work,
                           float* out, bool accumulate, hipStream_t st);

struct AttnFwdArgs {
  const uint16_t *q, *k, *v;
  uint16_t* o;
  float* lse;
  const int* kv_lens;
  long sqb, sqs, sqh, skb, sks, skh, svb, svs, svh, sob, sos, soh;
  long lse_ld;
  int B, Sq, Sk, Hq, Hkv, causal;
  float scale_log2;
  DropArgs drop;
};
struct AttnBwdArgs {
  const uint16_t *q, *k, *v, *dO;
  const float* lse;
  float* delta;
  uint16_t* dq;
  uint16_t *dk, *dv;
  const int* kv_lens;
  long sqb, sqs, sqh, skb, sks, skh, svb, svs, svh, sdb, sds, sdh;
  long sgqb, sgqs, sgqh, sgkb, sgks, sgkh, sgvb, sgvs, sgvh;
  long lse_ld;
  int B, Sq, Sk, Hq, Hkv, causal;
  float scale_log2, scale;
  int dkv_split = 1;
  float* dkv_ws = nullptr;
  float* cpart = nullptr;
  int cpart_ld = 0;
  DropArgs drop;
};
int flash_dkv_splits(int B, int Sq, int Sk, int Hkv, int causal);
bool flash_bwd_one_block(int D, int Sq, int Sk, int Hq, int Hkv, int dkv_split);
void launch_bn_relu_maxpool_fwd(const uint16_t* x, const float* gamma, const float* beta, const float* sums, int nrep,
                                float* save_mean, float* save_invstd, float* run_mean, float* run_var, float* params,
                                uint16_t* y, uint8_t* idx, int N, int H, int W, int C, float eps, float momentum,
                                hipStream_t st, uint16_t* xarg = nullptr, uint8_t* ybits = nullptr);
void launch_pool_bn_bwd_from_sums(const uint16_t* dpool, const uint8_t* idx, const uint16_t* x, const float* mean,
                                  const float* invstd, const float* gamma, const float* beta, uint16_t* dx,
                                  float* dgamma, float* dbeta, const float* sums, int nrep, float* params, int N,
                                  int H, int W, int C, hipStream_t st);
int pool_bn_workspace_floats(int C);
void launch_pool_bn_bwd(const uint16_t* dpool, const uint8_t* idx, const uint16_t* x, const float* mean,
                        const float* invstd, const float* gamma, const float* beta, uint16_t* dx, float* dgamma,
                        float* dbeta, float* work, float* params, int N, int H, int W, int C, hipStream_t st);

int stream_order_mode();
int stream_dir(int fixed);

void launch_flash_fwd(const AttnFwdArgs& a, int D, hipStream_t st);
void launch_flash_bwd(const AttnBwdArgs& a, int D, const uint16_t* o, long sob, long sos, long soh, hipStream_t st);

struct EmbTable {
  const uint16_t* w;
  float* g;
  const int64_t* ids;
  int V;
};
void launch_embed_fwd(const EmbTable* tabs, int ntab, int T, int D, int S, uint16_t* out, hipStream_t st);
void launch_embed_bwd(const EmbTable* tabs, int ntab, int T, int D, int S, const uint16_t* g, hipStream_t st);

void launch_avgpool_fwd(const uint16_t* x, uint16_t* y, int N, int HW, int C, hipStream_t st);
void launch_avgpool_bwd(const uint16_t* dy, uint16_t* dx, int N, int HW, int C, hipStream_t st);

void launch_stem_s2d_input(const uint16_t* x, int N, int H, int W, int Cin, int pad, uint16_t* out, hipStream_t st);
void launch_stem_w_s2d(const uint16_t* w7, int K, int R, int Cw, uint16_t* w4, hipStream_t st);
bool stem_conv_fwd_ok(int K, int R, int C, int Wo);
void launch_stem_conv_fwd(const uint16_t* xs, const uint16_t* w4, uint16_t* y, float* stats, int N, int Hs, int Ws,
                          hipStream_t st);
void splitk_reduce(const float* ws, int splits, long mn, float* out, bool accumulate, hipStream_t st);
bool wgrad3x3_tiled_ok(int C, int K, int R, int S, int stride, int pad, int W);
int wgrad3x3_tiled_blocks(int N, int H, int W, int C);
long wgrad3x3_tiled_workspace(int N, int H, int W, int C);
void launch_wgrad3x3_tiled(const uint16_t* x, const uint16_t* dy, float* ws, float* dw, int N, int H, int W, int C,
                           bool accumulate, hipStream_t st, const float* xform = nullptr);
int stem_wgrad_blocks(int N, int Hs);
void launch_stem_wgrad(const uint16_t* xs, const uint16_t* dy, float* ws, float* dw4, int N, int Hs, int Ws,
                       hipStream_t st);
void launch_stem_dw_s2d(const float* dw4, int K, int R, int Cw, float* dw7, hipStream_t st);

void launch_subsample_nhwc(const uint16_t* x, uint16_t* y, int N, int H, int W, int C, int s, hipStream_t st);
void launch_maxpool_fwd(const uint16_t* x, uint16_t* y, uint8_t* idx, int N, int H, int W, int C, int Ho, int Wo,
                        int k, int s, int p, hipStream_t st);
void launch_maxpool_bwd(const uint16_t* dy, const uint8_t* idx, uint16_t* dx, int N, int H, int W, int C, int Ho,
                        int Wo, int k, int s, int p, hipStream_t st);

}
```

k8s_amd/models/resnet.py:

```python
from __future__ import annotations

import math
from typing import List

import torch
import torch.nn as nn

from k8s_amd.ops import nn as K
from k8s_amd.parallel.flat import ParamStore, init_const, init_kaiming_normal, init_uniform


class BN(nn.Module):
    def __init__(self, store: ParamStore, name: str, c: int, zero_init: bool = False):
        super().__init__()
        self.gamma = store.new(name + ".weight", (c,), init_const(0.0 if zero_init else 1.0), decay=False, lowp=False)
        self.beta = store.new(name + ".bias", (c,), init_const(0.0), decay=False, lowp=False)
        self.register_buffer("running_mean", torch.zeros(c))
        self.register_buffer("running_var", torch.ones(c))
        self.momentum, self.eps = 0.1, 1e-5

    def forward(self, x, residual=None, relu=True, res_link=None, dy_link=None, sub2=False, bn3_link=None):
        sums = None
        if isinstance(x, tuple):
            x, sums = x
        return K.batch_norm_act(x, self.gamma, self.beta, self.running_mean, self.running_var, residual, relu,
                                self.training, self.momentum, self.eps, sums=sums, res_link=res_link,
                                dy_link=dy_link, sub2=sub2, bn3_link=bn3_link)


class Conv(nn.Module):
    def __init__(self, store: ParamStore, name: str, cin: int, cout: int, k: int, stride: int = 1):
        super().__init__()
        self.w = store.new(name + ".weight", (cout, k, k, cin), init_kaiming_normal(cin * k * k))
        self.stride, self.pad = stride, k // 2

    def forward(self, x, grad_link=None):
        return K.conv2d_nhwc(x, self.w, self.stride, self.pad, with_stats=True, grad_link=grad_link)


class Bottleneck(nn.Module):
    expansion = 4

    def __init__(self, store, name, cin, width, stride, downsample):
        super().__init__()
        cout = width * 4
        self.conv1 = Conv(store, name + ".conv1", cin, width, 1)
        self.bn1 = BN(store, name + ".bn1", width)
        self.conv2 = Conv(store, name + ".conv2", width, width, 3, stride)
        self.bn2 = BN(store, name + ".bn2", width)
        self.conv3 = Conv(store, name + ".conv3", width, cout, 1)
        self.bn3 = BN(store, name + ".bn3", cout, zero_init=True)
        self.down = None
        if downsample:
            self.down = Conv(store, name + ".downsample.0", cin, cout, 1, stride)
            self.down_bn = BN(store, name + ".downsample.1", cout)

    def forward(self, x, sub2=False):
        idn = x
        identity = self.down is None and x.requires_grad
        link = K.GradLink() if identity else None
        dlink = K.GradLink(shared=True) if (self.down is not None and x.requires_grad) else None
        mlink = dn = None
        if self.down is not None:
            mlink = K.MaskLink()
            dn = self.down(x, grad_link=dlink)
            fuse = K.BN_DUAL and isinstance(dn, tuple) and dn[1] is not None and self.training and dn[0].is_cuda
            if not fuse:
                idn = self.down_bn(dn, relu=False, dy_link=mlink)
        t = self.conv1(x, grad_link=link or dlink)
        t = K.bn_relu_conv(t, self.bn1, self.conv2)
        b3 = K.Bn3Link() if (self.down is None and self.training) else None
        t = K.bn_relu_conv(t, self.bn2, self.conv3, bn3_link=b3)
        if dn is not None and fuse:
            y = K.bn_act_dual(t, self.bn3, dn, self.down_bn)
            if y is not None:
                return y
            idn = self.down_bn(dn, relu=False, dy_link=mlink)
        return self.bn3(t, residual=idn, relu=True, res_link=link or mlink, sub2=sub2, bn3_link=b3)


class ResNet(nn.Module):
    def __init__(self, store: ParamStore, layers: List[int] = (3, 4, 6, 3), num_classes: int = 1000,
                 in_ch: int = 3, width: int = 64, stem_s2d: bool = True):
        super().__init__()
        self.store = store
        self.stem_s2d = stem_s2d
        self.in_ch = in_ch
        self.stem_ch = (in_ch + 7) // 8 * 8
        self.conv1 = Conv(store, "conv1", self.stem_ch, width, 7, 2)
        self.bn1 = BN(store, "bn1", width)
        blocks = []
        cin = width
        for i, n in enumerate(layers):
            w = width * (2 ** i)
            for j in range(n):
                stride = 2 if (j == 0 and i > 0) else 1
                blocks.append(Bottleneck(store, "layer%d.%d" % (i + 1, j), cin, w, stride, j == 0))
                cin = w * 4
        self.blocks = nn.ModuleList(blocks)
        self.fc_w = store.new("fc.weight", (num_classes, cin), init_uniform(1.0 / math.sqrt(cin)))
        self.fc_b = store.new("fc.bias", (num_classes,), init_uniform(1.0 / math.sqrt(cin)), decay=False,
                              lowp=False)
        self.num_classes = num_classes

    def finalize(self, device, **kw):
        self.store.finalize(device, **kw)
        if self.stem_ch != self.in_ch:
            with torch.no_grad():
                self.conv1.w.master[..., self.in_ch:].zero_()
            self.store.refresh_lowp()
        return self.to(device)

    def prepare_input(self, images_nhwc: torch.Tensor, s2d: bool = None) -> torch.Tensor:
        use = self.stem_s2d if s2d is None else s2d
        if use and images_nhwc.is_cuda and images_nhwc.dtype == torch.bfloat16 and self.conv1.w.shape[1] == 7:
            return K.stem_s2d_input(images_nhwc, pad=3)
        if images_nhwc.shape[-1] == self.stem_ch:
            return images_nhwc
        pad = self.stem_ch - images_nhwc.shape[-1]
        return torch.nn.functional.pad(images_nhwc, (0, pad))

    def forward(self, x):
        if x.shape[-1] == 16 and self.stem_s2d and x.is_cuda:
            t = K.stem_conv_s2d(x, self.conv1.w)
        else:
            t = self.conv1(x)
        y = K.bn_relu_maxpool(t, self.bn1)
        for i, b in enumerate(self.blocks):
            nxt = self.blocks[i + 1] if i + 1 < len(self.blocks) else None
            y = b(y, sub2=nxt is not None and nxt.down is not None and nxt.down.stride == 2)
        y = K.global_avg_pool_nhwc(y)
        return K.linear(y, self.fc_w, self.fc_b)

    def batch_norms(self):
        out = [self.bn1]
        for b in self.blocks:
            out += [b.bn1, b.bn2, b.bn3] + ([b.down_bn] if b.down is not None else [])
        return out

    def folded_views(self, flat: torch.Tensor):
        views, off = [], 0
        for bn in self.batch_norms():
            c = bn.running_mean.numel()
            views.append((flat[off:off + c], flat[off + c:off + 2 * c]))
            off += 2 * c
        assert off == flat.numel(), "folded BatchNorm tensor of another model"
        return views

    @torch.no_grad()
    def fold_bn(self):
        bns = self.batch_norms()
        dev = self.bn1.running_mean.device
        flat = torch.empty(2 * sum(bn.running_mean.numel() for bn in bns), device=dev, dtype=torch.float32)
        views = self.folded_views(flat)
        for bn, (scale, shift) in zip(bns, views):
            torch.mul(bn.gamma.master.float(), torch.rsqrt(bn.running_var.float() + bn.eps), out=scale)
            torch.sub(bn.beta.master.float(), bn.running_mean.float() * scale, out=shift)
        return flat, views

    @torch.no_grad()
    def forward_infer(self, x, folded=None):
        if folded is None:
            folded = self.fold_bn()
        views = self.folded_views(folded) if torch.is_tensor(folded) else folded[1]
        it = iter(views)
        sc, sh = next(it)
        if x.shape[-1] == 16 and self.stem_s2d and x.is_cuda:
            t = K.stem_conv_s2d(x, self.conv1.w)[0]
            bn = self.bn1
            t = K.batch_norm_act(t, bn.gamma, bn.beta, bn.running_mean, bn.running_var, None, True, False,
                                 bn.momentum, bn.eps)
        else:
            t = K.conv_bn_act_infer(x, self.conv1.w, sc, sh, self.conv1.stride, self.conv1.pad)
        y = K.max_pool_nhwc(t, 3, 2, 1)
        for b in self.blocks:
            (s1, h1), (s2, h2), (s3, h3) = next(it), next(it), next(it)
            idn = y
            if b.down is not None:
                sd, hd = next(it)
                idn = K.conv_bn_act_infer(y, b.down.w, sd, hd, b.down.stride, b.down.pad, relu=False)
            t = K.conv_bn_act_infer(y, b.conv1.w, s1, h1, b.conv1.stride, b.conv1.pad)
            t = K.conv_bn_act_infer(t, b.conv2.w, s2, h2, b.conv2.stride, b.conv2.pad)
            y = K.conv_bn_act_infer(t, b.conv3.w, s3, h3, b.conv3.stride, b.conv3.pad, residual=idn)
        y = K.global_avg_pool_nhwc(y)
        return K.linear(y, self.fc_w, self.fc_b)


def resnet50(store: ParamStore, num_classes: int = 1000) -> ResNet:
    return ResNet(store, (3, 4, 6, 3), num_classes)


def resnet_tiny(store: ParamStore, num_classes: int = 10) -> ResNet:
    return ResNet(store, (1, 1, 1, 1), num_classes, width=8)
```

k8s_amd/ops/conv.py:

```python
from __future__ import annotations

import collections
import os
import warnings

import torch
import torch.nn.functional as F

from k8s_amd.ops._ext import load as _load



STATS = {"hip_fwd": 0, "aten_fwd": 0, "hip_wgrad": 0, "aten_wgrad": 0, "hip_dgrad": 0, "aten_dgrad": 0,
         "bn_bstats": 0, "hip_infer": 0, "aten_infer": 0,
         "bn3_onload": 0, "bn3_apply": 0}
ROUTES = collections.Counter()



def _nchw(x):
    return x.permute(0, 3, 1, 2)


def _nhwc(y):
    return y.permute(0, 2, 3, 1).contiguous()


def _hip(*ts):
    return all(t.is_cuda and t.dtype == torch.bfloat16 for t in ts)


def fwd_ok(x, w):
    return _hip(x, w) and x.shape[-1] % 8 == 0 and w.shape[0] % 8 == 0


def _key(op, x, w, stride, padding):
    return "%s|%s|%s|%d|%d" % (op, "x".join(map(str, x.shape)), "x".join(map(str, w.shape)), stride, padding)


def fwd_uses_hip(x, w, stride, padding) -> bool:
    return fwd_ok(x, w)


_WARNED = set()


def _vendor(op, x, w, stride, padding):
    if x.is_cuda:
        STATS["aten_" + op] += 1
        key = _key("conv_" + op, x, w, stride, padding)
        if key not in _WARNED:
            _WARNED.add(key)
            warnings.warn("k8s_amd conv: %s is outside the MFMA kernels' shape contract; using ATen" % key)


def conv_fwd(x, w, stride, padding, stats=None):
    if fwd_uses_hip(x, w, stride, padding):
        STATS["hip_fwd"] += 1
        return _load().conv_fwd(x, w, stride, padding, 1, False, None, 0, stats)
    _vendor("fwd", x, w, stride, padding)
    return _nhwc(F.conv2d(_nchw(x), _nchw(w), None, stride, padding))


def infer_ok(x, w, scale, shift, residual=None) -> bool:
    ts = [x, w] + ([residual] if residual is not None else [])
    return (_hip(*ts) and x.shape[-1] % 8 == 0 and w.shape[0] % 8 == 0
            and all(t.is_contiguous() and t.data_ptr() % 16 == 0 for t in ts)
            and scale.is_cuda and shift.is_cuda and scale.dtype == torch.float32 and shift.dtype == torch.float32
            and scale.is_contiguous() and shift.is_contiguous())


def conv_infer(x, w, stride, padding, scale, shift, residual=None, relu=True):
    if infer_ok(x, w, scale, shift, residual):
        STATS["hip_infer"] += 1
        return _load().conv_infer(x, w, stride, padding, scale, shift, residual, relu)
    _vendor("infer", x, w, stride, padding)
    y = F.conv2d(_nchw(x), _nchw(w), None, stride, padding).permute(0, 2, 3, 1)
    y = (y.float() * scale.float() + shift.float()).to(x.dtype)
    if residual is not None:
        y = y.float() + residual.float()
    if relu:
        y = torch.relu(y)
    return y.to(x.dtype).contiguous()


def _aten_bwd(gy, x, w, stride, padding, need_dx, need_dw):
    dx, dw, _ = torch.ops.aten.convolution_backward(
        _nchw(gy), _nchw(x), _nchw(w), None, [stride, stride], [padding, padding], [1, 1], False, [0, 0], 1,
        [bool(need_dx), bool(need_dw), False])
    return (_nhwc(dx) if dx is not None else None), (dw.permute(0, 2, 3, 1) if dw is not None else None)


def _wgrad_hip(C_, gy, x, out, stride, padding, acc, xform=None):
    K, R, S, C = out.shape
    N, Ho, Wo = gy.shape[0], gy.shape[1], gy.shape[2]
    if (R == 1 and S == 1 and stride == 1 and padding == 0
            and (xform is not None or not C_.wgrad_stream_eligible(N, Ho, Wo, C, K, R, S))):
        C_.gemm(gy.reshape(-1, K), False, x.reshape(-1, C), False, out.view(K, C), True, None, 0, None, acc, 1.0, 0,
                xform_b=xform, xform_c=C if xform is not None else 0)
    else:
        C_.conv_wgrad(x, gy, out, stride, padding, 1, 0, acc, xform=xform)


BSTATS_3X3 = os.environ.get("K8S_AMD_BN_BSTATS_3X3", "1") != "0"
BSTATS_GEMM = os.environ.get("K8S_AMD_BN_BSTATS_GEMM", "1") != "0"
BSTATS_ENTRY = os.environ.get("K8S_AMD_BN_BSTATS_ENTRY", "1") != "0"
BSTATS_TILE_MASK = os.environ.get("K8S_AMD_BN_BSTATS_TILE_MASK", "1") != "0"
BSTATS_STRIDED = os.environ.get("K8S_AMD_BN_BSTATS_STRIDED", "0") != "0"
BSTATS_TILE_SHORT = os.environ.get("K8S_AMD_BN_BSTATS_TILE_SHORT", "0") != "0"


def _bn_sums(C_, bn_link, C, device):
    R = C_.conv_stat_replicas
    if bn_link.store is not None:
        from k8s_amd.ops.nn import _zero_scratch
        return _zero_scratch(bn_link.store, device, R * 2 * C).view(R, 2, C)
    return torch.zeros(R, 2, C, device=device, dtype=torch.float32)


def _link_kind(bn_link, shape):
    filled = bn_link is not None and bn_link.kind is not None and bn_link.x.shape == shape
    return bn_link.kind if filled else None


def _plan_dgrad(C_, gy, w, padding, addend, bn_link):
    K, R, S, C = w.shape
    N, Ho, Wo = gy.shape[:3]
    masked = addend is not None and not torch.is_tensor(addend)
    kind = _link_kind(bn_link, (N, Ho + R - 1 - 2 * padding, Wo + S - 1 - 2 * padding, C))
    if (BSTATS_3X3 and kind == "relu" and addend is None and R == 3 and S == 3 and padding == 1 and Ho == Wo
            and C_.conv3x3_staged_ok(Ho, Wo, C, K, 3, 3, 1, 1)):
        return "conv3x3_relu_sums"
    if not (R == 1 and S == 1 and padding == 0):
        return "implicit_flipped"
    M = N * Ho * Wo
    if masked:
        residual = kind in ("mask", "dual", "pool")
        if residual and C_.gemm_short_bnstats_ok(M, C, K, kind == "dual"):
            return "short_mask_sums"
        if (residual and BSTATS_TILE_MASK and M < 2 ** 31
                and (BSTATS_TILE_SHORT or kind != "dual" or not C_.gemm_short_bnstats_ok(M, C, K, False))):
            return "tile_mask_sums"
        return "gemm_masked_add"
    if addend is None:
        if BSTATS_GEMM and kind == "relu" and C_.gemm_dgrad_bnstats_ok(M, C, K):
            return "tile_relu_sums"
        if BSTATS_ENTRY and kind == "mask" and C_.gemm_short_bnstats_ok(M, C, K, False):
            return "short_entry_pending"
        return "gemm_plain"
    if kind == "pool" and addend.is_contiguous() and C % 8 == 0 and M < 2 ** 31:
        return "tile_final_sums"
    return "gemm_add"


def _dgrad_hip(C_, gy, w, padding, addend=None, bn_link=None):
    route = _plan_dgrad(C_, gy, w, padding, addend, bn_link)
    ROUTES[route] += 1
    K, R, S, C = w.shape
    ln = bn_link
    if route == "implicit_flipped":
        if addend is not None and not torch.is_tensor(addend):
            addend = addend.materialize()
        dx = C_.conv_fwd(gy, C_.conv_dgrad_wtrans(w), 1, R - 1 - padding, 1, False, None, 0, None)
        return dx if addend is None else dx.add_(addend)
    if route == "conv3x3_relu_sums":
        sums = _bn_sums(C_, ln, C, gy.device)
        dx = C_.conv3x3_dgrad_bnstats(gy, C_.conv_dgrad_wtrans(w), ln.x, ln.gamma, ln.beta, ln.mean, ln.invstd, sums)
        ln.deposit(sums, None, dx)
        return dx
    shape = gy.shape[:3] + (C,)
    gy, w = gy.reshape(-1, K), w.reshape(K, C)
    if route == "gemm_plain":
        return C_.gemm(gy, True, w, False, None, False, None, 0, None, False, 1.0, 1).reshape(shape)
    if route == "gemm_add":
        C_.gemm(gy, True, w, False, addend.view(-1, C), False, None, 0, None, True, 1.0, 1)
        return addend
    if route == "gemm_masked_add":
        out = torch.empty(shape, device=gy.device, dtype=gy.dtype)
        C_.gemm(gy, True, w, False, out.view(-1, C), False, None, 0, None, True, 1.0, 1,
                add_src=addend.dy.view(-1, C), add_mask=addend.mask)
        return out
    sums, sums2, x = _bn_sums(C_, ln, C, gy.device), None, ln.x.view(-1, C)
    if route == "tile_relu_sums":
        out = C_.gemm_dgrad_bnstats(gy, w, x, ln.gamma, ln.beta, ln.mean, ln.invstd, sums).view(shape)
    elif route == "short_entry_pending":
        out = C_.dgrad_short_bnstats(gy, w, None, None, x, ln.mask, ln.mean, sums).view(shape)
        ln.deposit_pending(sums)
        return out
    elif route == "tile_final_sums":
        out = addend
        C_.gemm_dgrad_bnstats_mask(gy, w, out.view(-1, C), x, ln.mask, ln.mean, sums)
    else:
        x2 = None
        if ln.kind == "dual":
            sums2, x2 = _bn_sums(C_, ln, C, gy.device), ln.x2.view(-1, C)
        add = addend.dy.view(-1, C)
        if route == "short_mask_sums":
            out = C_.dgrad_short_bnstats(gy, w, add, addend.mask, x, ln.mask, ln.mean, sums, x2, ln.mean2,
                                         sums2).view(shape)
        else:
            out = torch.empty(shape, device=gy.device, dtype=gy.dtype)
            C_.gemm_dgrad_bnstats_mask(gy, w, out.view(-1, C), x, ln.mask, ln.mean, sums, add, addend.mask, x2,
                                       ln.mean2, sums2)
    ln.deposit(sums, sums2, out)
    return out


def _parity_taps(R, a, pad, stride):
    taps = sorted(((a + pad - r) // stride, r) for r in range(R) if (a + pad - r) % stride == 0)
    if taps and [d for d, _ in taps] != list(range(taps[0][0], taps[0][0] + len(taps))):
        return None
    return taps


def strided_dgrad_ok(gy, w, stride, padding):
    K, R, S, C = w.shape
    if stride < 2 or K % 8 or C % 8:
        return False
    for a in range(stride):
        for b in range(stride):
            tr, ts = _parity_taps(R, a, padding, stride), _parity_taps(S, b, padding, stride)
            if tr is None or ts is None:
                return False
            if tr and ts and tr[0][0] != ts[0][0]:
                return False
    return True


def _plan_dgrad_strided(gy, w, stride, padding, H, W, addend, bn_link):
    K, R, S, C = w.shape
    kind = _link_kind(bn_link, (gy.shape[0], H, W, C))
    if bn_link is not None and bn_link.pending:
        if (kind is not None and R == 1 and S == 1 and padding == 0 and torch.is_tensor(addend)
                and addend.is_contiguous() and addend.shape == bn_link.x.shape):
            return "parity_complete_sums"
        bn_link.drop_pending()
    if BSTATS_STRIDED and kind == "relu" and addend is None and C > 64 and K % 64 == 0:
        return "parity_relu_sums"
    return "parity"


def _dgrad_strided_hip(C_, gy, w, stride, padding, H, W, addend=None, bn_link=None):
    route = _plan_dgrad_strided(gy, w, stride, padding, H, W, addend, bn_link)
    ROUTES[route] += 1
    K, R, S, C = w.shape
    ln = bn_link
    tail = (addend is not None,)
    if route == "parity_complete_sums":
        tail = (True, ln.x, ln.mask, ln.mean, ln.sums)
    elif route == "parity_relu_sums":
        rsums = _bn_sums(C_, ln, C, gy.device)
        tail = (False, ln.x, None, ln.mean, rsums, ln.gamma, ln.beta, ln.invstd)
    live = [(a, b, _parity_taps(R, a, padding, stride), _parity_taps(S, b, padding, stride))
            for a in range(stride) for b in range(stride)]
    live = [(a, b, tr, ts) for a, b, tr, ts in live if tr and ts]
    if addend is not None:
        dx = addend
    else:
        alloc = torch.zeros if len(live) < stride * stride else torch.empty
        dx = alloc(gy.shape[0], H, W, C, device=gy.device, dtype=gy.dtype)
    packed, offs = C_.conv_dgrad_wsub(w, [[r * S + s_ for _, r in tr for _, s_ in ts] for _, _, tr, ts in live])
    offs = offs.tolist()
    for i, (a, b, tr, ts) in enumerate(live):
        n = C * len(tr) * len(ts) * K
        wsub = packed[offs[i]:offs[i] + n].view(C, len(tr), len(ts), K)
        Hs, Ws = (H - a + stride - 1) // stride, (W - b + stride - 1) // stride
        C_.conv_fwd_subgrid(gy, wsub, -tr[0][0], Hs, Ws, dx, stride, a, b, *tail)
    if route == "parity_complete_sums":
        ln.complete(dx)
    elif route == "parity_relu_sums":
        ln.deposit(rsums, None, dx)
    return dx


def _plan_bwd(C_, gy, x, w, stride, padding, addend, xform, bn_link):
    K, R, S, C = w.shape
    if (xform is not None and addend is None and R == 1 and S == 1 and stride == 1 and padding == 0
            and os.environ.get("K8S_AMD_BWD1X1_FUSED", "1") != "0" and _link_kind(bn_link, x.shape) == "relu"
            and bn_link.x.data_ptr() == x.data_ptr() and gy.is_contiguous() and x.is_contiguous()
            and C_.bwd1x1_fused_ok(gy.numel() // K, C, K)):
        return "fused_1x1"
    if _hip(gy, x, w) and stride == 1 and K % 8 == 0 and C % 8 == 0:
        return "stride1"
    if _hip(gy, x, w) and strided_dgrad_ok(gy, w, stride, padding):
        return "strided"
    return "aten"


def _slot_written(p):
    p.store._notify(p) if p.written else p.store.mark_written(p)


def _finish_dw(p, gy, x, w, stride, padding):
    if p is not None:
        _vendor("wgrad", x, w, stride, padding)
        _, dw = _aten_bwd(gy, x, w, stride, padding, False, True)
        p.store.deposit(p, dw)


def conv_bwd(gy, x, w, stride, padding, need_dx, p=None, addend=None, xform=None, x_sub=None, bn_link=None, bn3=None):
    K, R, S, C = w.shape
    C_ = _load() if gy.is_cuda else None
    if bn3 is not None and not (need_dx and bn3.covers(gy)
                                and _plan_bwd(C_, gy, x, w, stride, padding, addend, xform, bn_link) == "fused_1x1"):
        STATS["bn3_apply"] += 1
        gy = C_.bn_bwd_apply(gy.contiguous(), bn3.x3, bn3.mask, bn3.params)
        bn3 = None
    if x_sub is not None:
        _wgrad_hip(C_, gy, x_sub, p.grad.view(p.shape), 1, 0, p.written)
        STATS["hip_wgrad"] += 1
        _slot_written(p)
        p = None
    hip = _hip(gy, x, w)
    if xform is not None and not (hip and C % 64 == 0 and K % 8 == 0 and p is not None
                                  and p.grad.dtype == torch.float32):
        raise RuntimeError("normalize-on-load weight gradient outside the kernels' contract")
    if addend is not None and not torch.is_tensor(addend) and not (
            hip and stride == 1 and K % 8 == 0 and C % 8 == 0):
        addend = addend.materialize()
    family = _plan_bwd(C_, gy, x, w, stride, padding, addend, xform, bn_link) if need_dx else None
    if family == "fused_1x1":
        ROUTES[family] += 1
        STATS["bn3_onload"] += bn3 is not None
        STATS["hip_wgrad"] += 1
        STATS["hip_dgrad"] += 1
        sums = _bn_sums(C_, bn_link, C, gy.device)
        onload = {} if bn3 is None else {"x3": bn3.x3.view(-1, K), "mask": bn3.mask, "params": bn3.params}
        dz = C_.bwd1x1_fused(gy.view(-1, K), x.view(-1, C), w.view(K, C), xform, bn_link.gamma, bn_link.beta,
                             bn_link.mean, bn_link.invstd, p.grad.view(K, C), sums, p.written, **onload).view(x.shape)
        _slot_written(p)
        bn_link.deposit(sums, None, dz)
        return dz
    if hip and C % 8 == 0 and K % 8 == 0 and p is not None and p.grad.dtype == torch.float32:
        STATS["hip_wgrad"] += 1
        _wgrad_hip(C_, gy, x, p.grad.view(p.shape), stride, padding, p.written, xform)
        _slot_written(p)
        p = None
    dx = None
    if family in ("stride1", "strided"):
        STATS["hip_dgrad"] += 1
        if family == "stride1":
            dx = _dgrad_hip(C_, gy, w, padding, addend, bn_link)
        else:
            dx = _dgrad_strided_hip(C_, gy, w, stride, padding, x.shape[1], x.shape[2], addend, bn_link)
    elif family == "aten":
        ROUTES[family] += 1
        _vendor("dgrad", x, w, stride, padding)
        dx, _ = _aten_bwd(gy, x, w, stride, padding, True, False)
        if addend is not None:
            dx = dx + addend
    _finish_dw(p, gy, x, w, stride, padding)
    return dx


SUB1X1 = os.environ.get("K8S_AMD_SUB1X1", "1") != "0"


def subsample_ok(x, w, stride, padding) -> bool:
    K, R, S, C = w.shape
    return (SUB1X1 and stride > 1 and R == 1 and S == 1 and padding == 0 and _hip(x, w) and C % 64 == 0
            and K % 8 == 0 and x.is_contiguous())
```

k8s_amd/ops/nn.py:

```python
from __future__ import annotations

import os
from typing import Optional

import torch
import torch.nn.functional as F

from k8s_amd.ops import reference as ref
from k8s_amd.ops._ext import load as _load_ext


def _gpu(t: torch.Tensor) -> bool:
    return t.is_cuda


def _C():
    return _load_ext()


def _conv_impl():
    from k8s_amd.ops import conv as _conv

    return _conv


def _zero_scratch(store, device, n):
    from k8s_amd.parallel.flat import ZeroArena

    arena = store.__dict__.get("zero_arena")
    if arena is None or arena.device != torch.device(device):
        arena = store.zero_arena = ZeroArena(device)
    return arena.take(n)


class GradLink:
    __slots__ = ("grad", "shared")

    def __init__(self, shared: bool = False):
        self.grad = None
        self.shared = shared


class BiasLink:
    __slots__ = ("pb", "done")

    def __init__(self):
        self.pb, self.done = None, False


class ActLink:
    __slots__ = ("saved", "act", "pb", "done")

    def __init__(self):
        self.saved, self.act, self.pb, self.done = None, None, None, False


class SwiGLULink:
    __slots__ = ("saved", "dgu", "blk")

    def __init__(self, blk: int = 0):
        self.saved, self.dgu, self.blk = None, None, blk


class MaskedGrad:
    __slots__ = ("dy", "mask")

    def __init__(self, dy, mask):
        self.dy, self.mask = dy, mask

    def materialize(self):
        return _C().mask_apply(self.dy, self.mask)


class BnStatLink:
    __slots__ = ("kind", "x", "mask", "mean", "x2", "mean2", "invstd", "gamma", "beta", "sums", "sums2", "dy_key",
                 "store", "pending")

    def __init__(self):
        self.sums = self.sums2 = self.dy_key = None
        self.pending = False
        self._fill(None, None, None, None)

    def _fill(self, kind, store, x, mean, mask=None, x2=None, mean2=None, invstd=None, gamma=None, beta=None):
        self.kind, self.store = kind, store
        self.x, self.mean, self.mask, self.x2, self.mean2 = x, mean, mask, x2, mean2
        self.invstd, self.gamma, self.beta = invstd, gamma, beta

    def fill_relu(self, x, mean, invstd, gamma, beta, store=None):
        self._fill("relu", store, x, mean, invstd=invstd, gamma=gamma, beta=beta)

    def fill_mask(self, x, mask, mean, store=None):
        self._fill("mask", store, x, mean, mask)

    def fill_dual(self, x, mask, mean, x2, mean2, store=None):
        self._fill("dual", store, x, mean, mask, x2, mean2)

    def fill_pool(self, x, mask, mean, store=None):
        self._fill("pool", store, x, mean, mask)

    @staticmethod
    def _key(t):
        return t.data_ptr(), tuple(t.shape), t._version

    def deposit(self, sums, sums2, over):
        self.sums, self.sums2, self.dy_key = sums, sums2, self._key(over)
        _conv_impl().STATS["bn_bstats"] += 1

    def deposit_pending(self, sums):
        self.sums, self.sums2, self.dy_key, self.pending = sums, None, None, True
        _conv_impl().STATS["bn_bstats"] += 1

    def complete(self, over):
        self.dy_key, self.pending = self._key(over), False

    def drop_pending(self):
        self.sums, self.pending = None, False

    def covers(self, t) -> bool:
        return self.sums is not None and self.dy_key == self._key(t)

    def take(self, dy):
        pre = (self.sums, self.sums2) if self.covers(dy) else None
        self.sums = self.sums2 = self.dy_key = None
        self._fill(None, self.store, None, None)
        return pre


BN_BSTATS = os.environ.get("K8S_AMD_BN_BSTATS", "1") != "0"
BSTATS_POOL = os.environ.get("K8S_AMD_BN_BSTATS_POOL", "1") != "0"


class MaskLink:
    __slots__ = ("mask",)

    def __init__(self):
        self.mask = None


def bn3_onload_on() -> bool:
    return os.environ.get("K8S_AMD_BN3_ONLOAD", "1") != "0" and os.environ.get("K8S_AMD_BWD1X1_FUSED", "1") != "0"


class Bn3Link:
    __slots__ = ("y_key", "x3", "mask", "params", "dy_key")

    def __init__(self):
        self.y_key = self.x3 = self.mask = self.params = self.dy_key = None

    def offer(self, y):
        self.y_key = (y.data_ptr(), tuple(y.shape))

    def offered(self, x) -> bool:
        return self.y_key == (x.data_ptr(), tuple(x.shape))

    def fill(self, dy, x3, mask, params):
        self.x3, self.mask, self.params, self.dy_key = x3, mask, params, BnStatLink._key(dy)

    def covers(self, t) -> bool:
        return self.dy_key == BnStatLink._key(t)

    def take(self):
        if self.params is None:
            return None
        out = Bn3Link()
        out.x3, out.mask, out.params, out.dy_key = self.x3, self.mask, self.params, self.dy_key
        self.x3 = self.mask = self.params = self.dy_key = None
        return out


class _Conv2dNHWC(torch.autograd.Function):
    @staticmethod
    def forward(ctx, x, anchor, p, stride, padding, with_stats, link=None, bn_link=None):
        impl = _conv_impl()
        w = p.weight if x.dtype == p.weight.dtype else p.master.to(x.dtype)
        sums = None
        if with_stats and impl.fwd_uses_hip(x, w, stride, padding):
            sums = _zero_scratch(p.store, x.device, _C().conv_stat_replicas * 2 * w.shape[0]).view(
                _C().conv_stat_replicas, 2, w.shape[0])
        xs = None
        if impl.subsample_ok(x, w, stride, padding):
            xs = getattr(x, "_k8s_sub2", None) if stride == 2 else None
            if xs is None or xs.shape[:3] != ((x.shape[0], (x.shape[1] + 1) // 2, (x.shape[2] + 1) // 2)):
                xs = _C().subsample_nhwc(x, stride)
            y = impl.conv_fwd(xs, w, 1, 0, sums)
        else:
            y = impl.conv_fwd(x, w, stride, padding, sums)
        ctx.save_for_backward(x, xs)
        ctx.p, ctx.stride, ctx.padding, ctx.link, ctx.bn_link = p, stride, padding, link, bn_link
        ctx.x_requires_grad = x.requires_grad
        if sums is not None:
            ctx.mark_non_differentiable(sums)
        ctx.set_materialize_grads(False)
        return y, sums

    @staticmethod
    def backward(ctx, gy, _gsums=None):
        x, xs = ctx.saved_tensors
        p = ctx.p
        impl = _conv_impl()
        w = p.weight if x.dtype == p.weight.dtype else p.master.to(x.dtype)
        gy = gy.contiguous()
        addend = None
        if ctx.link is not None:
            addend, ctx.link.grad = ctx.link.grad, None
            if addend is None and ctx.link.shared and ctx.x_requires_grad:
                ctx.link.grad = impl.conv_bwd(gy, x, w, ctx.stride, ctx.padding, True, p, x_sub=xs,
                                              bn_link=ctx.bn_link)
                return None, None, None, None, None, None, None, None
        dx = impl.conv_bwd(gy, x, w, ctx.stride, ctx.padding, ctx.x_requires_grad, p, addend=addend, x_sub=xs,
                           bn_link=ctx.bn_link)
        return dx, None, None, None, None, None, None, None


def conv2d_nhwc(x: torch.Tensor, p, stride: int = 1, padding: int = 0, with_stats: bool = False,
                grad_link: "GradLink" = None):
    bn_link = getattr(x, "_k8s_bnstat", None)
    y, sums = _Conv2dNHWC.apply(x, p.store.anchor, p, stride, padding, with_stats, grad_link, bn_link)
    return (y, sums) if with_stats else y


def conv_bn_act_infer(x, pw, scale, shift, stride: int = 1, padding: int = 0, residual=None, relu: bool = True):
    assert not torch.is_grad_enabled(), "conv_bn_act_infer is an inference op: call it under torch.no_grad()"
    if torch.is_tensor(pw):
        w = pw
    else:
        w = pw.weight if x.dtype == pw.weight.dtype else pw.master.to(x.dtype)
    if _gpu(x):
        return _conv_impl().conv_infer(x, w, stride, padding, scale, shift, residual, relu)
    return ref.conv_bn_act_infer(x, w, scale, shift, stride, padding, residual, relu)


class _StemS2D(torch.autograd.Function):

    @staticmethod
    def forward(ctx, xs, anchor, p):
        C_ = _C()
        w7 = p.weight if p.weight.dtype == xs.dtype else p.master.to(xs.dtype)
        w4 = C_.stem_w_s2d(w7.contiguous())
        sums = _zero_scratch(p.store, xs.device, C_.conv_stat_replicas * 2 * w4.shape[0]).view(
            C_.conv_stat_replicas, 2, w4.shape[0])
        if tuple(w4.shape) == (64, 4, 4, 16) and (xs.shape[2] - 3) % 16 == 0 and xs.shape[2] - 3 <= 112:
            y = C_.stem_conv_fwd(xs.contiguous(), w4, sums)
        else:
            y = C_.conv_fwd(xs, w4, 1, 0, 1, False, None, 0, sums)
        _conv_impl().STATS["hip_fwd"] += 1
        ctx.save_for_backward(xs)
        ctx.p, ctx.kshape = p, tuple(w4.shape)
        ctx.mark_non_differentiable(sums)
        ctx.set_materialize_grads(False)
        return y, sums

    @staticmethod
    def backward(ctx, gy, _gsums=None):
        (xs,) = ctx.saved_tensors
        p, C_ = ctx.p, _C()
        dw4 = torch.empty(ctx.kshape, device=xs.device, dtype=torch.float32)
        if ctx.kshape == (64, 4, 4, 16) and (xs.shape[2] - 3) % 16 == 0 and xs.shape[2] - 3 <= 112:
            C_.stem_wgrad(xs.contiguous(), gy.contiguous(), dw4)
        else:
            _conv_impl()._wgrad_hip(C_, gy.contiguous(), xs, dw4, 1, 0, False)
        _conv_impl().STATS["hip_wgrad"] += 1
        dw7, finish = _param_grad(p, xs.device)
        C_.stem_dw_s2d(dw4, dw7)
        finish()
        return None, None, None


def stem_conv_s2d(xs, p):
    return _StemS2D.apply(xs, p.store.anchor, p)


def stem_s2d_input(images, pad: int = 3):
    return _C().stem_s2d_input(images.contiguous(), pad)


class _BnAct(torch.autograd.Function):
    @staticmethod
    def forward(ctx, x, res, anchor, pg, pb, run_mean, run_var, training, momentum, eps, relu, sums=None,
                res_link=None, dy_link=None, stat_link=None, sub2=None, bn3_link=None):
        x = x.contiguous()
        if res is not None:
            res = res.contiguous()
        want_mask = relu and res is not None and _gpu(x)
        mask = None
        want_sub = sub2 is not None and x.dim() == 4
        if _gpu(x) and sums is not None and training:
            out = _C().bn_fwd_from_sums(x, res, pg.master, pb.master, sums, run_mean, run_var, momentum, eps, relu,
                                        want_mask, want_sub)
            if want_sub:
                sub2.y = out[-1]
        elif _gpu(x):
            out = _C().bn_fwd(x, res, pg.master, pb.master, run_mean, run_var, training, momentum, eps, relu,
                              want_mask)
        else:
            out = ref.bn_fwd(x, res, pg.master, pb.master, run_mean, run_var, training, momentum, eps, relu)
        y, mean, invstd = out[0], out[1], out[2]
        if want_mask:
            mask = out[3]
        keep_y = relu and (res is not None or not _gpu(x)) and mask is None
        ctx.save_for_backward(x, y if keep_y else None, mean, invstd, mask)
        ctx.pg, ctx.pb, ctx.has_res, ctx.res_link = pg, pb, res is not None, res_link
        ctx.relu_x = relu and not keep_y and mask is None
        ctx.dy_link = dy_link if (dy_link is not None and not relu and res is None) else None
        ctx.stat_link = None
        if stat_link is not None and training and (mask is not None or ctx.relu_x):
            if mask is None:
                stat_link.fill_relu(x, mean, invstd, pg.master, pb.master, pg.store)
            else:
                stat_link.fill_mask(x, mask, mean, pg.store)
            ctx.stat_link = stat_link
        ctx.bn3_link = bn3_link if (bn3_link is not None and mask is not None and training
                                    and bn3_link.offered(x)) else None
        return y

    @staticmethod
    def backward(ctx, dy):
        x, y, mean, invstd, mask = ctx.saved_tensors
        pg, pb = ctx.pg, ctx.pb
        store = pg.store
        dy = dy.contiguous()
        if ctx.dy_link is not None and ctx.dy_link.mask is not None:
            mask, ctx.dy_link.mask = ctx.dy_link.mask, None
        mask_out = isinstance(ctx.res_link, MaskLink) and mask is not None and ctx.has_res
        if _gpu(x):
            dg, db, finish = _bn_param_grads(pg, pb, x.device)
            handoff = isinstance(ctx.res_link, GradLink) and ctx.has_res and mask is not None
            want_dres = ctx.has_res and not (handoff or mask_out)
            pre = ctx.stat_link.take(dy) if ctx.stat_link is not None else None
            if ctx.bn3_link is not None and not want_dres and bn3_onload_on():
                params = _C().bn_bwd_params(dy, x, mask, pre[0] if pre is not None else None, mean, invstd,
                                            pg.master, pb.master, dg, db)
                ctx.bn3_link.fill(dy, x, mask, params)
                dx, dres = dy, None
            elif pre is not None and mask is None:
                dx, dres = _C().bn_bwd_relu_from_sums(dy, x, pre[0], mean, invstd, pg.master, pb.master, dg, db)[0], None
            elif pre is not None:
                dx, dres = _C().bn_bwd_from_sums(dy, x, mask, pre[0], mean, invstd, pg.master, pb.master, dg, db,
                                                 want_dres)
            else:
                dx, dres = _C().bn_bwd(dy, x, y, mean, invstd, pg.master, pb.master, ctx.relu_x, dg, db, want_dres,
                                       mask)
            if ctx.bn3_link is not None and dx is not dy:
                _conv_impl().STATS["bn3_apply"] += 1
            if handoff:
                dres = MaskedGrad(dy, mask)
            elif mask_out:
                dres = dy
                ctx.res_link.mask = mask
            finish()
        else:
            dx, dres, dg, db = ref.bn_bwd(dy, x, y, mean, invstd, pg.master)
            store.deposit(pg, dg)
            store.deposit(pb, db)
        if ctx.has_res and isinstance(ctx.res_link, GradLink):
            ctx.res_link.grad, dres = dres, None
        return (dx, (dres if ctx.has_res else None), None, None, None, None, None, None, None, None, None, None, None,
                None, None, None, None)


BN_ONLOAD = os.environ.get("K8S_AMD_BN_ONLOAD", "1x1")
if BN_ONLOAD not in ("0", "1x1", "3x3"):
    raise ValueError("K8S_AMD_BN_ONLOAD must be 0 (BN applied by its own pass), 1x1 or 3x3, not %r" % BN_ONLOAD)


def _param_grad(p, device):
    slot = p.store.slot_for_write(p)
    g = slot.view(p.shape) if slot is not None else torch.empty(p.shape, device=device, dtype=torch.float32)
    return g, lambda: p.store.mark_written(p) if slot is not None else p.store.deposit(p, g)


# ... 411 lines not shown
    return out


class _Embedding(torch.autograd.Function):
    @staticmethod
    def forward(ctx, ids, anchor, pw, dtype):
        w = pw.weight if pw.weight.dtype == dtype else pw.master.to(dtype)
        ctx.save_for_backward(ids)
        ctx.pw = pw
        return F.embedding(ids, w)

    @staticmethod
    def backward(ctx, gy):
        (ids,) = ctx.saved_tensors
        pw = ctx.pw
        V, D = pw.shape
        store = pw.store
        slot = store.slot_for_write(pw)
        if slot is not None:
            slot.zero_()
            slot.index_add_(0, ids.reshape(-1), gy.reshape(-1, D).to(slot.dtype))
            store.mark_written(pw)
        elif pw.grad.dtype == torch.float32:
            pw.grad.index_add_(0, ids.reshape(-1), gy.reshape(-1, D).float())
            store._notify(pw)
        else:
            dw = torch.zeros((V, D), device=gy.device, dtype=torch.float32)
            dw.index_add_(0, ids.reshape(-1), gy.reshape(-1, D).float())
            store.deposit(pw, dw)
        return None, None, None, None


def embedding(ids, pw, dtype=torch.bfloat16):
    return _Embedding.apply(ids, pw.store.anchor, pw, dtype)


class _CrossEntropy(torch.autograd.Function):
    @staticmethod
    def forward(ctx, logits, labels, ignore_index, smoothing, valid):
        logits = logits if logits.stride(-1) == 1 else logits.contiguous()
        ctx.valid = valid
        full = logits
        if valid is not None and valid != logits.shape[1]:
            logits = logits[:, :valid]
        if _gpu(logits):
            loss, lse = _C().xent_fwd(logits, labels, ignore_index, smoothing)
        else:
            loss, lse = ref.xent_fwd(logits, labels, ignore_index, smoothing)
        nvalid = (labels != ignore_index).sum().clamp_min(1).float()
        ctx.save_for_backward(full, labels, lse, nvalid)
        ctx.ignore_index, ctx.smoothing = ignore_index, smoothing
        return loss.sum() / nvalid

    @staticmethod
    def backward(ctx, gl):
        full, labels, lse, nvalid = ctx.saved_tensors
        dscale = (gl.float() / nvalid).reshape(1)
        V = ctx.valid if ctx.valid is not None else full.shape[1]
        if _gpu(full):
            d = _C().xent_bwd(full, labels, lse, dscale, ctx.ignore_index, ctx.smoothing, V)
        else:
            d = torch.zeros_like(full)
            d[:, :V] = ref.xent_bwd(full[:, :V], labels, lse, dscale, ctx.ignore_index, ctx.smoothing)
        return d, None, None, None, None


def cross_entropy(logits, labels, ignore_index: int = -100, smoothing: float = 0.0, valid: int = None):
    return _CrossEntropy.apply(logits.reshape(-1, logits.shape[-1]), labels.reshape(-1), ignore_index, smoothing,
                               valid)


def xent_eval(logits, labels, ignore_index: int = -100, valid: int = None):
    logits = logits.reshape(-1, logits.shape[-1])
    labels = labels.reshape(-1)
    logits = logits if logits.stride(-1) == 1 else logits.contiguous()
    if valid is not None and valid != logits.shape[1]:
        logits = logits[:, :valid]
    if _gpu(logits):
        loss, rank = _C().xent_eval(logits.detach(), labels.contiguous(), ignore_index)
        return loss, rank
    return ref.xent_eval(logits.detach(), labels, ignore_index)


class _MaxPoolNHWC(torch.autograd.Function):
    @staticmethod
    def forward(ctx, x, k, s, p):
        y, idx = _C().maxpool_fwd(x.contiguous(), k, s, p)
        ctx.save_for_backward(idx)
        ctx.hw, ctx.ksp = x.shape[1:3], (k, s, p)
        return y

    @staticmethod
    def backward(ctx, dy):
        (idx,) = ctx.saved_tensors
        H, W = ctx.hw
        return _C().maxpool_bwd(dy.contiguous(), idx, H, W, *ctx.ksp), None, None, None


def max_pool_nhwc(x, k=3, s=2, p=1):
    if _gpu(x) and x.dtype == torch.bfloat16 and x.shape[-1] % 8 == 0:
        return _MaxPoolNHWC.apply(x, k, s, p)
    y = F.max_pool2d(x.permute(0, 3, 1, 2), k, s, p)
    return y.permute(0, 2, 3, 1).contiguous()


class _BnReluMaxPool(torch.autograd.Function):

    @staticmethod
    def forward(ctx, x, sums, anchor, pg, pb, run_mean, run_var, momentum, eps):
        x = x.contiguous()
        want = BN_BSTATS and BSTATS_POOL
        outs = _C().bn_relu_maxpool(x, sums, pg.master, pb.master, run_mean, run_var, momentum, eps, want)
        y, idx, mean, invstd = outs[:4]
        ctx.save_for_backward(x, idx, mean, invstd)
        ctx.pg, ctx.pb = pg, pb
        ctx.link = None
        if want:
            y._k8s_bnstat = ctx.link = BnStatLink()
            ctx.link.fill_pool(outs[4], outs[5], mean, pg.store)
        ctx.mark_non_differentiable(idx)
        return y

    @staticmethod
    def backward(ctx, dy):
        x, idx, mean, invstd = ctx.saved_tensors
        pg, pb = ctx.pg, ctx.pb
        dg, db, finish = _bn_param_grads(pg, pb, x.device)
        dy = dy.contiguous()
        pre = ctx.link.take(dy) if ctx.link is not None else None
        if pre is not None:
            dx = _C().pool_bn_bwd_from_sums(dy, idx, x, mean, invstd, pg.master, pb.master, dg, db, pre[0])
        else:
            dx = _C().pool_bn_bwd(dy, idx, x, mean, invstd, pg.master, pb.master, dg, db)
        finish()
        return (dx,) + (None,) * 8


def bn_relu_maxpool(t, bn):
    x, sums = t if isinstance(t, tuple) else (t, None)
    if (sums is not None and bn.training and _gpu(x) and x.dtype == torch.bfloat16 and x.dim() == 4
            and x.shape[-1] % 8 == 0 and 256 % (x.shape[-1] // 8) == 0):
        return _BnReluMaxPool.apply(x, sums, bn.gamma.store.anchor, bn.gamma, bn.beta, bn.running_mean,
                                    bn.running_var, bn.momentum, bn.eps)
    return max_pool_nhwc(bn(t), 3, 2, 1)


BN_DUAL = True


class _BnActDual(torch.autograd.Function):

    @staticmethod
    def forward(ctx, x, sums, xr, sums_r, anchor, pg, pb, run_mean, run_var, pgr, pbr, run_mean_r, run_var_r,
                momentum, eps, stat_link=None):
        x, xr = x.contiguous(), xr.contiguous()
        y, mean, invstd, mask, mean_r, invstd_r = _C().bn_fwd_from_sums_dual(
            x, sums, pg.master, pb.master, run_mean, run_var, xr, sums_r, pgr.master, pbr.master, run_mean_r,
            run_var_r, momentum, eps)
        ctx.save_for_backward(x, xr, mean, invstd, mask, mean_r, invstd_r)
        ctx.p = (pg, pb, pgr, pbr)
        ctx.stat_link = stat_link
        if stat_link is not None:
            stat_link.fill_dual(x, mask, mean, xr, mean_r, pg.store)
        return y

    @staticmethod
    def backward(ctx, dy):
        x, xr, mean, invstd, mask, mean_r, invstd_r = ctx.saved_tensors
        pg, pb, pgr, pbr = ctx.p
        dy = dy.contiguous()
        C_ = _C()
        dg, db, finish = _bn_param_grads(pg, pb, x.device)
        dgr, dbr, finish_r = _bn_param_grads(pgr, pbr, x.device)
        pre = ctx.stat_link.take(dy) if ctx.stat_link is not None else None
        if pre is not None and pre[1] is not None:
            dx, dxr = C_.bn_bwd_dual_from_sums(dy, mask, x, mean, invstd, pg.master, pb.master, dg, db, pre[0], xr,
                                               mean_r, invstd_r, pgr.master, pbr.master, dgr, dbr, pre[1])
        else:
            dx, dxr = C_.bn_bwd_dual(dy, mask, x, mean, invstd, pg.master, pb.master, dg, db, xr, mean_r, invstd_r,
                                     pgr.master, pbr.master, dgr, dbr)
        finish()
        finish_r()
        return (dx, None, dxr) + (None,) * 13


def bn_act_dual(t, bn, tr, bn_r):
    if not BN_DUAL or not (isinstance(t, tuple) and isinstance(tr, tuple)):
        return None
    (x, sums), (xr, sums_r) = t, tr
    if (sums is None or sums_r is None or not (bn.training and bn_r.training) or not _gpu(x)
            or x.dtype != torch.bfloat16 or xr.shape != x.shape or x.shape[-1] % 8 != 0):
        return None
    link = BnStatLink() if BN_BSTATS else None
    y = _BnActDual.apply(x, sums, xr, sums_r, bn.gamma.store.anchor, bn.gamma, bn.beta, bn.running_mean,
                         bn.running_var, bn_r.gamma, bn_r.beta, bn_r.running_mean, bn_r.running_var, bn.momentum,
                         bn.eps, link)
    if link is not None:
        y._k8s_bnstat = link
    return y


class _AvgPoolNHWC(torch.autograd.Function):
    @staticmethod
    def forward(ctx, x):
        ctx.hw = x.shape[1:3]
        return _C().avgpool_fwd(x.contiguous())

    @staticmethod
    def backward(ctx, dy):
        return _C().avgpool_bwd(dy.contiguous(), *ctx.hw)


def global_avg_pool_nhwc(x):
    if _gpu(x) and x.dtype == torch.bfloat16 and x.shape[-1] % 8 == 0:
        return _AvgPoolNHWC.apply(x)
    return x.mean(dim=(1, 2))


def _swiglu_split(gu, blk):
    F2 = gu.shape[-1] // 2
    if not blk:
        return gu.float().split(F2, -1)
    v = gu.float().reshape(*gu.shape[:-1], F2 // blk, 2, blk)
    return v[..., 0, :].reshape(*gu.shape[:-1], F2), v[..., 1, :].reshape(*gu.shape[:-1], F2)


def _swiglu_join(dg, du, blk):
    if not blk:
        return torch.cat([dg, du], -1)
    F2 = dg.shape[-1]
    lead = dg.shape[:-1]
    return torch.stack([dg.reshape(*lead, F2 // blk, blk), du.reshape(*lead, F2 // blk, blk)], -2).reshape(
        *lead, 2 * F2)


def _swiglu_bwd_any(gu, dy, blk):
    F2 = gu.shape[-1] // 2
    if _gpu(gu) and gu.dtype == torch.bfloat16 and F2 % 8 == 0:
        return _C().swiglu_bwd(gu, dy.contiguous(), blk)
    g, u = _swiglu_split(gu, blk)
    s_ = torch.sigmoid(g)
    d = dy.float()
    return _swiglu_join(d * u * s_ * (1 + g * (1 - s_)), d * g * s_, blk).to(gu.dtype)


class _SwiGLU(torch.autograd.Function):
    @staticmethod
    def forward(ctx, gu, link=None, blk=0):
        gu = gu.contiguous()
        F2 = gu.shape[-1] // 2
        if _gpu(gu) and gu.dtype == torch.bfloat16 and F2 % 8 == 0:
            y = _C().swiglu_fwd(gu, blk)
        else:
            g, u = _swiglu_split(gu, blk)
            y = (torch.nn.functional.silu(g) * u).to(gu.dtype)
        ctx.save_for_backward(gu)
        ctx.link, ctx.blk = link, blk
        if link is not None:
            link.saved, link.dgu, link.blk = gu.reshape(-1, 2 * F2), None, blk
        return y

    @staticmethod
    def backward(ctx, dy):
        (gu,) = ctx.saved_tensors
        link = ctx.link
        if link is not None and link.dgu is not None:
            dgu, link.dgu, link.saved = link.dgu, None, None
            return dgu.reshape(gu.shape), None, None
        if link is not None:
            link.saved = None
        return _swiglu_bwd_any(gu, dy, ctx.blk), None, None


def swiglu(gu, link=None, blk: int = 0):
    return _SwiGLU.apply(gu, link if SWIGLU_FUSE else None, blk)


SWIGLU_EPI = os.environ.get("K8S_AMD_SWIGLU_EPI", "1") != "0"


class _LinearSwiGLU(torch.autograd.Function):

    @staticmethod
    def forward(ctx, x, anchor, pw, link=None):
        x2 = x.reshape(-1, x.shape[-1])
        gu, h = _C().gemm_swiglu_fwd(x2, pw.weight)
        ctx.save_for_backward(x2, gu)
        ctx.pw, ctx.link, ctx.xshape = pw, link, x.shape
        if link is not None:
            link.saved, link.dgu, link.blk = gu, None, 64
        return h.reshape(*x.shape[:-1], h.shape[-1])

    @staticmethod
    def backward(ctx, dh):
        x2, gu = ctx.saved_tensors
        link, pw = ctx.link, ctx.pw
        if link is not None and link.dgu is not None:
            dgu, link.dgu, link.saved = link.dgu, None, None
        else:
            if link is not None:
                link.saved = None
            dgu = _swiglu_bwd_any(gu, dh.reshape(gu.shape[0], -1), 64)
        dx, dw, _ = _gemm().linear_bwd(dgu.reshape(gu.shape), x2, pw.weight, None, None, pw=pw, store=pw.store,
                                       need_db=False)
        if dw is not None:
            pw.store.deposit(pw, dw)
        return dx.reshape(ctx.xshape), None, None, None


ROPE_EPI = os.environ.get("K8S_AMD_ROPE_EPI", "1") != "0"


class _LinearRope(torch.autograd.Function):

    @staticmethod
    def forward(ctx, x, anchor, pw, pos, table, rot_cols):
        x2 = x.reshape(-1, x.shape[-1])
        y = _C().gemm_rope(x2, pw.weight, pos, table, rot_cols)
        ctx.save_for_backward(x2)
        ctx.pw, ctx.xshape = pw, x.shape
        return y.reshape(*x.shape[:-1], y.shape[-1])

    @staticmethod
    def backward(ctx, gy):
        (x2,) = ctx.saved_tensors
        pw = ctx.pw
        gy2 = gy.reshape(-1, gy.shape[-1]).contiguous()
        dx, dw, _ = _gemm().linear_bwd(gy2, x2, pw.weight, None, None, pw=pw, store=pw.store, need_db=False)
        if dw is not None:
            pw.store.deposit(pw, dw)
        return dx.reshape(ctx.xshape), None, None, None, None, None


def linear_rope(x, pw, pos, table, rot_cols: int):
    x2 = x.reshape(-1, x.shape[-1])
    if (ROPE_EPI and _gpu(x) and x.dtype == torch.bfloat16 and pw.weight.dtype == torch.bfloat16 and x2.is_contiguous()
            and pw.grad.dtype == torch.float32 and table.dim() == 3 and table.shape[1] == 64
            and bool(_C().gemm_rope_ok(x2.shape[0], pw.shape[0], x2.shape[1], rot_cols))):
        return _LinearRope.apply(x, pw.store.anchor, pw, pos, table, rot_cols), True
    return linear(x, pw), False


def linear_swiglu(x, pw, link=None, blk: int = 64):
    x2 = x.reshape(-1, x.shape[-1])
    F = pw.shape[0] // 2
    if (SWIGLU_EPI and blk == 64 and _gpu(x) and x.dtype == torch.bfloat16 and pw.weight.dtype == torch.bfloat16
            and x2.is_contiguous() and pw.grad.dtype == torch.float32
            and bool(_C().gemm_swiglu_fwd_ok(x2.shape[0], F, x2.shape[1]))):
        return _LinearSwiGLU.apply(x, pw.store.anchor, pw, link if SWIGLU_FUSE else None)
# ... 45 lines not shown
```

Baseline: 16760 images/s.

## Fuse dual BN backward apply into downstream 1x1 conv backward via onload params

Splits the dual BatchNorm backward into a params-only stage and, when the following 1x1 convs can take it, skips materializing dx/dxr by handing the params table to the conv backward kernels to apply on load. Adds a 'final' form of bwd1x1_fused for (C,K)=(64,256) that writes straight into the residual addend and also does the maxpool-winner BN backward, using global_load_lds staging and dw partials. This removes full-tensor elementwise passes and their memory traffic in the first bottleneck stage. In exchange it adds more LDS per stage, a separate dw-partials reduction, and complex linkage conditions across autograd functions.

Measured after the change: 17100 images/s, median of 6. +2.0%, better.

```diff
diff --git a/k8s_amd/csrc/binding/batchnorm.cpp b/k8s_amd/csrc/binding/batchnorm.cpp
--- a/k8s_amd/csrc/binding/batchnorm.cpp
+++ b/k8s_amd/csrc/binding/batchnorm.cpp
@@ -269,6 +269,33 @@
                      f32(dbeta), f32(work), f32(params), cbf(x2), f32(mean2), f32(invstd2), f32(gamma2), f32(beta2),
                      bf(dx2), f32(dgamma2), f32(dbeta2), f32(work2), f32(params2), M, C, cur_stream());
   return {dx, dx2};
+}
+std::vector<Tensor> bn_bwd_dual_params(Tensor dy, Tensor mask, Tensor x, Tensor mean, Tensor invstd, Tensor gamma,
+                                       Tensor beta, Tensor dgamma, Tensor dbeta, OptTensor sums, Tensor x2,
+                                       Tensor mean2, Tensor invstd2, Tensor gamma2, Tensor beta2, Tensor dgamma2,
+                                       Tensor dbeta2, OptTensor sums2) {
+  const bool pre = sums && sums->defined();
+  TORCH_CHECK(pre == (sums2 && sums2->defined()), "sums and sums2 come together");
+  const int C = bn_channels(x, "x", !pre);
+  const long M = x.numel() / C;
+  check_same_shape(dy, x, "dy");
+  check_same_shape(x2, x, "x2");
+  check_bwd_vectors(mean, invstd, gamma, beta, dgamma, dbeta, C);
+  check_bwd_vectors(mean2, invstd2, gamma2, beta2, dgamma2, dbeta2, C);
+  const uint8_t* mk = check_bit_mask(mask, x.numel(), "mask");
+  const int nrep = pre ? check_stat_sums(*sums, C, "sums", false) : 0;
+  TORCH_CHECK(!pre || check_stat_sums(*sums2, C, "sums2", false) == nrep, "sums / sums2: the same replica count");
+  auto params = torch::empty({4 * C}, gamma.options()), params2 = torch::empty({4 * C}, gamma.options());
+  Tensor work, work2;
+  if (!pre) {
+    work = torch::empty({k8s_amd::bn_workspace_floats(M, C)}, gamma.options());
+    work2 = torch::empty({k8s_amd::bn_workspace_floats(M, C)}, gamma.options());
+  }
+  launch_bn_bwd_dual_params(cbf(dy), mk, cbf(x), pre ? f32(*sums) : nullptr, nrep, f32(mean), f32(invstd), f32(gamma),
+                            f32(beta), f32(dgamma), f32(dbeta), pre ? nullptr : f32(work), f32(params), cbf(x2),
+                            pre ? f32(*sums2) : nullptr, f32(mean2), f32(invstd2), f32(gamma2), f32(beta2),
+                            f32(dgamma2), f32(dbeta2), pre ? nullptr : f32(work2), f32(params2), M, C, cur_stream());
+  return {params, params2};
 }
 std::vector<Tensor> bn_bwd_dual(Tensor dy, Tensor mask, Tensor x, Tensor mean, Tensor invstd, Tensor gamma,
                                 Tensor beta, Tensor dgamma, Tensor dbeta, Tensor x2, Tensor mean2, Tensor invstd2,
@@ -304,6 +331,10 @@
   m.def("bn_bwd_apply", &bn_bwd_apply, "dy"_a, "x"_a, "mask"_a, "params"_a,
         "second half of a masked BatchNorm backward: dx from bn_bwd_params' table");
   m.def("bn_bwd_dual_from_sums", &bn_bwd_dual_from_sums, "bn_bwd_dual from a producer's reduction sums");
+  m.def("bn_bwd_dual_params", &bn_bwd_dual_params, "dy"_a, "mask"_a, "x"_a, "mean"_a, "invstd"_a, "gamma"_a, "beta"_a,
+        "dgamma"_a, "dbeta"_a, "sums"_a, "x2"_a, "mean2"_a, "invstd2"_a, "gamma2"_a, "beta2"_a, "dgamma2"_a,
+        "dbeta2"_a, "sums2"_a,
+        "first half of bn_bwd_dual(_from_sums): both dgamma / dbeta and (params, params2), each [sc | B | D | shift]");
   m.def("bn_relu_maxpool", &bn_relu_maxpool, "x"_a, "sums"_a, "gamma"_a, "beta"_a, "run_mean"_a, "run_var"_a,
         "momentum"_a, "eps"_a, "want_link"_a = false);
   m.def("pool_bn_bwd_from_sums", &pool_bn_bwd_from_sums);
diff --git a/k8s_amd/csrc/binding/conv.cpp b/k8s_amd/csrc/binding/conv.cpp
--- a/k8s_amd/csrc/binding/conv.cpp
+++ b/k8s_amd/csrc/binding/conv.cpp
@@ -94,8 +94,10 @@
   return dx;
 }
 
-Tensor bwd1x1_fused(Tensor gy, Tensor x, Tensor w, Tensor xform, Tensor gamma, Tensor beta, Tensor mean, Tensor invstd,
-                    Tensor dw, Tensor sums, bool accumulate, OptTensor x3, OptTensor mask, OptTensor params) {
+Tensor bwd1x1_fused(Tensor gy, Tensor x, Tensor w, OptTensor xform, OptTensor gamma, OptTensor beta, OptTensor mean,
+                    OptTensor invstd, Tensor dw, Tensor sums, bool accumulate, OptTensor x3, OptTensor mask,
+                    OptTensor params, OptTensor addend, OptTensor winner_x, OptTensor winner_bits,
+                    OptTensor winner_mean) {
   check_bf16_dense(gy, 2, "gy"); check_bf16_dense(x, 2, "x"); check_bf16_dense(w, 2, "w");
   const long M = gy.size(0), K = gy.size(1), C = x.size(1);
   TORCH_CHECK(x.size(0) == M && w.size(0) == K && w.size(1) == C, "shapes: gy [M, K], x [M, C], w [K, C]");
@@ -103,8 +105,35 @@
               "bwd1x1_fused: (C, K) = (64, 256) or (128, 512), 1 <= M < 2^31");
   check_cuda(dw, "dw"); check_dtype(dw, at::kFloat, "dw"); check_aligned(dw, "dw");
   TORCH_CHECK(dw.numel() == K * C, "dw must have K * C fp32 elements");
-  check_channel_f32(xform, 2 * C, "xform (BatchNorm scale | shift)");
-  const k8s_amd::BnBwdSums bb = bn_bwd_sums(x, mean, sums, {}, gamma, beta, invstd, {}, {}, {});
+  const bool fin = addend || winner_x || winner_bits || winner_mean;
+  k8s_amd::BnBwdSums bb;
+  k8s_amd::Bwd1x1Final fn;
+  if (fin) {
+    TORCH_CHECK(addend && winner_x && winner_bits && winner_mean,
+                "bwd1x1_fused: addend, winner_x, winner_bits and winner_mean come together");
+    TORCH_CHECK(!xform && !gamma && !beta && !mean && !invstd,
+                "bwd1x1_fused: the final form takes x as stored -- no xform, gamma, beta, mean or invstd");
+    TORCH_CHECK(k8s_amd::bwd1x1_final_ok(M, (int)C, (int)K), "bwd1x1_fused: the final form is (C, K) = (64, 256) only");
+    check_bf16_dense(*addend, 2, "addend"); check_bf16_dense(*winner_x, 2, "winner_x");
+    TORCH_CHECK(addend->size(0) == M && addend->size(1) == C, "addend: the shape of x, [M, C]");
+    TORCH_CHECK(winner_x->size(0) == M && winner_x->size(1) == C, "winner_x: the shape of x, [M, C]");
+    fn.winner_bits = check_bit_mask(*winner_bits, M * C, "winner_bits");
+    TORCH_CHECK((reinterpret_cast<uintptr_t>(fn.winner_bits) & 3) == 0, "winner_bits must be 4-byte aligned");
+    check_channel_f32(*winner_mean, C, "winner_mean");
+    check_stat_sums(sums, C, "bn sums", true);
+    TORCH_CHECK(addend->device() == gy.device() && winner_x->device() == gy.device() &&
+                    winner_bits->device() == gy.device() && winner_mean->device() == gy.device() &&
+                    sums.device() == gy.device(),
+                "addend, winner_x, winner_bits, winner_mean and sums: on gy's device");
+    fn.addend = cbf(*addend);
+    fn.winner_x = cbf(*winner_x);
+    fn.winner_mean = f32(*winner_mean);
+    bb.sums = f32(sums);
+  } else {
+    TORCH_CHECK(xform && gamma && beta && mean && invstd, "bwd1x1_fused: xform, gamma, beta, mean and invstd");
+    check_channel_f32(*xform, 2 * C, "xform (BatchNorm scale | shift)");
+    bb = bn_bwd_sums(x, *mean, sums, {}, gamma, beta, invstd, {}, {}, {});
+  }
   k8s_amd::Bwd1x1Bn3 bn3;
   const bool onload = x3 || mask || params;
   if (onload) {
@@ -120,9 +149,15 @@
     bn3.x3 = cbf(*x3);
     bn3.params = f32(*params);
   }
-  Tensor dz = torch::empty({M, C}, gy.options());
-  launch_bwd1x1_fused(cbf(gy), cbf(x), cbf(w), f32(xform), bb.gamma, bb.beta, bb.mean, bb.invstd, bf(dz), f32(dw),
-                      bb.sums, M, (int)C, (int)K, accumulate, cur_stream(), onload ? &bn3 : nullptr);
+  Tensor dz = fin ? *addend : torch::empty({M, C}, gy.options());
+  Tensor part;
+  if (fin) {
+    part = torch::empty({k8s_amd::bwd1x1_final_workspace(M, (int)C, (int)K)}, dw.options());
+    fn.dw_partials = f32(part);
+  }
+  launch_bwd1x1_fused(cbf(gy), cbf(x), cbf(w), fin ? nullptr : f32(*xform), bb.gamma, bb.beta, bb.mean, bb.invstd,
+                      bf(dz), f32(dw), bb.sums, M, (int)C, (int)K, accumulate, cur_stream(), onload ? &bn3 : nullptr,
+                      fin ? &fn : nullptr);
   return dz;
 }
 
@@ -208,10 +243,15 @@
         "xform"_a = py::none());
   m.def("bwd1x1_fused", &bwd1x1_fused, "gy"_a, "x"_a, "w"_a, "xform"_a, "gamma"_a, "beta"_a, "mean"_a, "invstd"_a,
         "dw"_a, "sums"_a, "accumulate"_a, "x3"_a = py::none(), "mask"_a = py::none(), "params"_a = py::none(),
+        "addend"_a = py::none(), "winner_x"_a = py::none(), "winner_bits"_a = py::none(),
+        "winner_mean"_a = py::none(),
         "1x1 data gradient, normalize-on-load weight gradient and BatchNorm-backward sums in one pass (bwd1x1_fused.hip)");
   m.def("bwd1x1_fused_ok", [](int64_t M, int64_t C, int64_t K) {
     return C <= 1024 && K <= 4096 && k8s_amd::bwd1x1_fused_ok(M, (int)C, (int)K);
   }, "M"_a, "C"_a, "K"_a, "whether bwd1x1_fused takes this shape");
+  m.def("bwd1x1_final_ok", [](int64_t M, int64_t C, int64_t K) {
+    return C <= 1024 && K <= 4096 && k8s_amd::bwd1x1_final_ok(M, (int)C, (int)K);
+  }, "M"_a, "C"_a, "K"_a, "whether bwd1x1_fused's final form (addend, winner_*) takes this shape");
   m.def("wgrad_stream_eligible",&k8s_amd::wgrad_stream_eligible, "tall-K weight-gradient kernel takes this shape");
   m.def("conv_dgrad_wtrans", &conv_dgrad_wtrans);
   m.def("conv_dgrad_wsub", &conv_dgrad_wsub);
diff --git a/k8s_amd/csrc/kernels/batchnorm.hip b/k8s_amd/csrc/kernels/batchnorm.hip
--- a/k8s_amd/csrc/kernels/batchnorm.hip
+++ b/k8s_amd/csrc/kernels/batchnorm.hip
@@ -886,28 +886,19 @@
   launch_bn_bwd_apply(dy, x, nullptr, params, true, dx, nullptr, M, C, st);
 }
 
-void launch_bn_bwd_dual_from_sums(const uint16_t* dy, const uint8_t* mask, const uint16_t* x, const float* sums,
-                                  int nrep, const float* mean, const float* invstd, const float* gamma,
-                                  const float* beta, uint16_t* dx, float* dgamma, float* dbeta, float* params,
-                                  const uint16_t* x2, const float* sums2, const float* mean2, const float* invstd2,
-                                  const float* gamma2, const float* beta2, uint16_t* dx2, float* dgamma2,
-                                  float* dbeta2, float* params2, long M, int C, hipStream_t st) {
-  hipLaunchKernelGGL(bn_bwd_final_sums_kernel, dim3(cdiv(C, 256)), dim3(256), 0, st, sums, sums, nrep, C, dgamma,
-                     dbeta, 1.f / (float)M, mean, invstd, gamma, beta, params);
-  hipLaunchKernelGGL(bn_bwd_final_sums_kernel, dim3(cdiv(C, 256)), dim3(256), 0, st, sums, sums2, nrep, C, dgamma2,
-                     dbeta2, 1.f / (float)M, mean2, invstd2, gamma2, beta2, params2);
-  const long nvec = M * C / 8;
-  if (nvec >= (1L << 31)) throw std::runtime_error("BatchNorm tensor too large (>= 2^31 vectors)");
-  hipLaunchKernelGGL(bn_bwd_apply_dual_kernel, dim3(cdiv(nvec, BN_THREADS)), dim3(BN_THREADS), 0, st, dy, mask, x,
-                     params, dx, x2, params2, dx2, (int)nvec, C, make_fastdiv(C / 8),
-                     stream_order_mode() ? (stream_dir(0) ? 1 : 2) : 0);
-}
-
-void launch_bn_bwd_dual(const uint16_t* dy, const uint8_t* mask, const uint16_t* x, const float* mean,
-                        const float* invstd, const float* gamma, const float* beta, uint16_t* dx, float* dgamma,
-                        float* dbeta, float* work, float* params, const uint16_t* x2, const float* mean2,
-                        const float* invstd2, const float* gamma2, const float* beta2, uint16_t* dx2, float* dgamma2,
-                        float* dbeta2, float* work2, float* params2, long M, int C, hipStream_t st) {
+void launch_bn_bwd_dual_params(const uint16_t* dy, const uint8_t* mask, const uint16_t* x, const float* sums, int nrep,
+                               const float* mean, const float* invstd, const float* gamma, const float* beta,
+                               float* dgamma, float* dbeta, float* work, float* params, const uint16_t* x2,
+                               const float* sums2, const float* mean2, const float* invstd2, const float* gamma2,
+                               const float* beta2, float* dgamma2, float* dbeta2, float* work2, float* params2, long M,
+                               int C, hipStream_t st) {
+  if (sums) {
+    hipLaunchKernelGGL(bn_bwd_final_sums_kernel, dim3(cdiv(C, 256)), dim3(256), 0, st, sums, sums, nrep, C, dgamma,
+                       dbeta, 1.f / (float)M, mean, invstd, gamma, beta, params);
+    hipLaunchKernelGGL(bn_bwd_final_sums_kernel, dim3(cdiv(C, 256)), dim3(256), 0, st, sums, sums2, nrep, C, dgamma2,
+                       dbeta2, 1.f / (float)M, mean2, invstd2, gamma2, beta2, params2);
+    return;
+  }
   BnGeom g = bn_geom(C, M);
   const int nb = bn_reduce_blocks(M, g);
   const int rdir = stream_dir(1);
@@ -917,11 +908,37 @@
                      1.f / (float)M, mean, invstd, gamma, beta, params);
   hipLaunchKernelGGL(bn_bwd_final_kernel, dim3(cdiv(C, FIN_CH)), dim3(256), 0, st, work2, nb, C, dgamma2, dbeta2,
                      1.f / (float)M, mean2, invstd2, gamma2, beta2, params2);
+}
+
+static void launch_bn_bwd_apply_dual(const uint16_t* dy, const uint8_t* mask, const uint16_t* x, const float* params,
+                                     uint16_t* dx, const uint16_t* x2, const float* params2, uint16_t* dx2, long M,
+                                     int C, hipStream_t st) {
   const long nvec = M * C / 8;
   if (nvec >= (1L << 31)) throw std::runtime_error("BatchNorm tensor too large (>= 2^31 vectors)");
   hipLaunchKernelGGL(bn_bwd_apply_dual_kernel, dim3(cdiv(nvec, BN_THREADS)), dim3(BN_THREADS), 0, st, dy, mask, x,
                      params, dx, x2, params2, dx2, (int)nvec, C, make_fastdiv(C / 8),
                      stream_order_mode() ? (stream_dir(0) ? 1 : 2) : 0);
+}
+
+void launch_bn_bwd_dual_from_sums(const uint16_t* dy, const uint8_t* mask, const uint16_t* x, const float* sums,
+                                  int nrep, const float* mean, const float* invstd, const float* gamma,
+                                  const float* beta, uint16_t* dx, float* dgamma, float* dbeta, float* params,
+                                  const uint16_t* x2, const float* sums2, const float* mean2, const float* invstd2,
+                                  const float* gamma2, const float* beta2, uint16_t* dx2, float* dgamma2,
+                                  float* dbeta2, float* params2, long M, int C, hipStream_t st) {
+  launch_bn_bwd_dual_params(dy, mask, x, sums, nrep, mean, invstd, gamma, beta, dgamma, dbeta, nullptr, params, x2,
+                            sums2, mean2, invstd2, gamma2, beta2, dgamma2, dbeta2, nullptr, params2, M, C, st);
+  launch_bn_bwd_apply_dual(dy, mask, x, params, dx, x2, params2, dx2, M, C, st);
+}
+
+void launch_bn_bwd_dual(const uint16_t* dy, const uint8_t* mask, const uint16_t* x, const float* mean,
+                        const float* invstd, const float* gamma, const float* beta, uint16_t* dx, float* dgamma,
+                        float* dbeta, float* work, float* params, const uint16_t* x2, const float* mean2,
+                        const float* invstd2, const float* gamma2, const float* beta2, uint16_t* dx2, float* dgamma2,
+                        float* dbeta2, float* work2, float* params2, long M, int C, hipStream_t st) {
+  launch_bn_bwd_dual_params(dy, mask, x, nullptr, 0, mean, invstd, gamma, beta, dgamma, dbeta, work, params, x2,
+                            nullptr, mean2, invstd2, gamma2, beta2, dgamma2, dbeta2, work2, params2, M, C, st);
+  launch_bn_bwd_apply_dual(dy, mask, x, params, dx, x2, params2, dx2, M, C, st);
 }
 
 void launch_bn_relu_maxpool_fwd(const uint16_t* x, const float* gamma, const float* beta, const float* sums, int nrep,
diff --git a/k8s_amd/csrc/kernels/bwd1x1_fused.hip b/k8s_amd/csrc/kernels/bwd1x1_fused.hip
--- a/k8s_amd/csrc/kernels/bwd1x1_fused.hip
+++ b/k8s_amd/csrc/kernels/bwd1x1_fused.hip
@@ -42,6 +42,9 @@
   float* dw;
   float* sums;
   int M, C, ntiles, npairs;
+  const uint16_t *addend, *xw;
+  const uint8_t* bits;
+  float* dwpart;
 };
 
 __device__ __forceinline__ void lds_barrier() {
@@ -50,13 +53,19 @@
   asm volatile("" ::: "memory");
 }
 
-template <int K, int RS, int NSLOT, int HALVES, bool ONLOAD>
+__device__ __forceinline__ void glds4(const void* src, void* lds_base) {
+  __builtin_amdgcn_global_load_lds(src, (lds_void*)lds_base, 4, 0, 0);
+}
+
+template <int K, int RS, int NSLOT, int HALVES, bool ONLOAD, bool FINAL = false>
 __global__ void __launch_bounds__(THREADS, 1) bwd1x1_fused_kernel(Args a) {
   constexpr int RB = K * 2, UG = K / 8;
   constexpr int IMG_G = RS * RB, IMG_X = RS * 128;
   constexpr int IMG_M = ONLOAD ? RS * UG : 0;
   constexpr int OFF_X = IMG_G + (ONLOAD ? IMG_G + IMG_M : 0);
-  constexpr int STAGE = OFF_X + IMG_X, RING = NSLOT * STAGE;
+  constexpr int OFF_A = OFF_X + IMG_X, OFF_W = OFF_A + IMG_X, OFF_B = OFF_W + IMG_X;
+  constexpr int STAGE = FINAL ? OFF_B + 1024 : OFF_X + IMG_X, RING = NSLOT * STAGE;
+  static_assert(!FINAL || (K == 256 && RS == 32 && HALVES == 1), "the final form: (C, K) = (64, 256), 32-row tiles");
   constexpr int LG = RS * UG / THREADS;
   constexpr int LPS = ONLOAD ? 2 * LG : LG;
   constexpr bool TREG = ONLOAD && (THREADS / UG) % 16 == 0;
@@ -106,10 +115,14 @@
   float xsc[8], xsh[8], gsc[8], gsh[8], mu[8], ps[8], pq[8];
 #pragma unroll
   for (int j = 0; j < 8; ++j) {
-    xsc[j] = a.xform[ecol + j];
-    xsh[j] = a.xform[C + ecol + j];
     mu[j] = a.mean[ecol + j];
-    bn_affine_regs(a.gamma[ecol + j], a.beta[ecol + j], mu[j], a.invstd[ecol + j], gsc[j], gsh[j]);
+    if constexpr (!FINAL) {
+      xsc[j] = a.xform[ecol + j];
+      xsh[j] = a.xform[C + ecol + j];
+      bn_affine_regs(a.gamma[ecol + j], a.beta[ecol + j], mu[j], a.invstd[ecol + j], gsc[j], gsh[j]);
+    } else {
+      xsc[j] = xsh[j] = gsc[j] = gsh[j] = 0.f;
+    }
     ps[j] = pq[j] = 0.f;
   }
   if constexpr (PLDS) {
@@ -143,7 +156,10 @@
   }
 #pragma unroll
   for (int ks = 0; ks < NKS; ++ks) asm volatile("" : "+v"(wf[ks]));
-  if constexpr (!PLDS) {
+  if constexpr (FINAL) {
+#pragma unroll
+    for (int j = 0; j < 8; ++j) asm volatile("" : "+v"(mu[j]));
+  } else if constexpr (!PLDS) {
 #pragma unroll
     for (int j = 0; j < 8; ++j) asm volatile("" : "+v"(xsc[j]), "+v"(xsh[j]), "+v"(gsc[j]), "+v"(gsh[j]), "+v"(mu[j]));
   } else {
@@ -168,7 +184,18 @@
         const unsigned q = (wid * 64 + lane) * 16;
         glds16(a.mask + m0 * UG + min(q / UG, last) * UG + q % UG, st + 2 * IMG_G + wid * 1024);
       }
-      if (wid < XT / 64) glds16(a.x + m0 * C + min((unsigned)erow, last) * C + ecol, st + OFF_X + wid * 1024);
+      if (wid < XT / 64) {
+        const unsigned eoff = min((unsigned)erow, last) * C + ecol;
+        glds16(a.x + m0 * C + eoff, st + OFF_X + wid * 1024);
+        if constexpr (FINAL) {
+          glds16(a.addend + m0 * C + eoff, st + OFF_A + wid * 1024);
+          glds16(a.xw + m0 * C + eoff, st + OFF_W + wid * 1024);
+        }
+      }
+      if constexpr (FINAL) {
+        if (wid == THREADS / 64 - 1)
+          glds4(a.bits + m0 * 8 + min((unsigned)lane >> 1, last) * 8 + (lane & 1) * 4, st + OFF_B);
+      }
       return;
     }
 #pragma unroll
@@ -183,6 +210,16 @@
       const long m = m0 + erow;
       const void* src = m < M ? (const void*)(a.x + m * C + ecol) : (const void*)g_zero16;
       glds16(src, st + OFF_X + wid * 1024);
+      if constexpr (FINAL) {
+        glds16(m < M ? (const void*)(a.addend + m * C + ecol) : (const void*)g_zero16, st + OFF_A + wid * 1024);
+        glds16(m < M ? (const void*)(a.xw + m * C + ecol) : (const void*)g_zero16, st + OFF_W + wid * 1024);
+      }
+    }
+    if constexpr (FINAL) {
+      if (wid == THREADS / 64 - 1) {
+        const long m = m0 + (lane >> 1);
+        glds4(m < M ? (const void*)(a.bits + m * 8 + (lane & 1) * 4) : (const void*)g_zero16, st + OFF_B);
+      }
     }
   };
 
@@ -281,7 +318,26 @@
     }
     lds_barrier();
 
-    if (wid < XT / 64) {
+    if constexpr (FINAL) {
+      if (wid < XT / 64) {
+        const bf16x8_t dzv = *reinterpret_cast<const bf16x8_t*>(stg + tid * 16);
+        const bf16x8_t adv = *reinterpret_cast<const bf16x8_t*>(G + OFF_A + tid * 16);
+        const bf16x8_t xv = *reinterpret_cast<const bf16x8_t*>(G + OFF_W + tid * 16);
+        const long m = (long)(pair + s * a.npairs) * RS + erow;
+        const uint32_t bits = m < M ? (uint32_t) * reinterpret_cast<const uint8_t*>(G + OFF_B + erow * 8 + eu) : 0u;
+        float o[8];
+#pragma unroll
+        for (int j = 0; j < 8; ++j) o[j] = bf2f((uint16_t)dzv[j]) + bf2f((uint16_t)adv[j]);
+        const bf16x8_t ov = pack_bf16x8(o);
+#pragma unroll
+        for (int j = 0; j < 8; ++j) {
+          const float g = (bits >> j) & 1u ? bf2f((uint16_t)ov[j]) : 0.f;
+          ps[j] += g;
+          pq[j] = __builtin_fmaf(g, bf2f((uint16_t)xv[j]) - mu[j], pq[j]);
+        }
+        if (m < M) *reinterpret_cast<bf16x8_t*>(a.dz + m * C + ecol) = ov;
+      }
+    } else if (wid < XT / 64) {
       const bf16x8_t dzv = *reinterpret_cast<const bf16x8_t*>(stg + tid * 16);
       const bf16x8_t xv = *reinterpret_cast<const bf16x8_t*>(X + tid * 16);
       if constexpr (PLDS) {
@@ -332,6 +388,16 @@
     slot = slot + 1 == NSLOT ? 0 : slot + 1;
   }
 
+  if constexpr (FINAL) {
+    float* slab = a.dwpart + (long)bid * K * CT;
+#pragma unroll
+    for (int i = 0; i < KTW; ++i) {
+      const int k = wid * KW + i * 16 + (lane & 15);
+#pragma unroll
+      for (int j = 0; j < 4; ++j)
+        *reinterpret_cast<f32x4_t*>(slab + (long)k * CT + j * 16 + 4 * (lane >> 4)) = dwa[i][j];
+    }
+  } else
 #pragma unroll
   for (int i = 0; i < KTW; ++i) {
     const int k = wid * KW + i * 16 + (lane & 15);
@@ -367,19 +433,40 @@
 bool bwd1x1_fused_ok(long M, int C, int K) {
   return M >= 1 && M < (1L << 31) && ((C == 64 && K == 256) || (C == 128 && K == 512));
 }
+bool bwd1x1_final_ok(long M, int C, int K) { return bwd1x1_fused_ok(M, C, K) && C == 64; }
+long bwd1x1_final_workspace(long M, int C, int K) {
+  return std::min<long>(std::max(1, planner_cus()), (M + 31) / 32) * K * C;
+}
 
 void launch_bwd1x1_fused(const uint16_t* gy, const uint16_t* x, const uint16_t* w, const float* xform,
                          const float* gamma, const float* beta, const float* mean, const float* invstd, uint16_t* dz,
                          float* dw, float* sums, long M, int C, int K, bool accumulate, hipStream_t st,
-                         const Bwd1x1Bn3* bn3) {
+                         const Bwd1x1Bn3* bn3, const Bwd1x1Final* fin) {
   using namespace b1f;
   if (!bwd1x1_fused_ok(M, C, K)) throw std::runtime_error("bwd1x1_fused: (C, K) = (64, 256) or (128, 512), M < 2^31");
   if (bn3 && !(bn3->x3 && bn3->mask && bn3->params)) throw std::runtime_error("bwd1x1_fused: x3, mask and params");
-  if (!accumulate) (void)hipMemsetAsync(dw, 0, (size_t)K * C * sizeof(float), st);
-  Args a{gy, x, w, nullptr, nullptr, nullptr, xform, gamma, beta, mean, invstd, dz, dw, sums, (int)M, C, 0, 0};
+  if (fin) {
+    if (!bwd1x1_final_ok(M, C, K)) throw std::runtime_error("bwd1x1_fused, final form: (C, K) = (64, 256)");
+    if (!(fin->addend && fin->winner_x && fin->winner_bits && fin->winner_mean) || dz != fin->addend)
+      throw std::runtime_error("bwd1x1_fused, final form: addend (the output), winner_x, winner_bits, winner_mean");
+    if (xform || gamma || beta || mean || invstd)
+      throw std::runtime_error("bwd1x1_fused, final form: no xform operands");
+  }
+  if (fin && !fin->dw_partials) throw std::runtime_error("bwd1x1_fused, final form: dw_partials");
+  if (!accumulate && !fin) (void)hipMemsetAsync(dw, 0, (size_t)K * C * sizeof(float), st);
+  Args a{gy, x, w, nullptr, nullptr, nullptr, xform, gamma, beta, mean, invstd, dz, dw, sums, (int)M, C, 0, 0,
+         nullptr, nullptr, nullptr, nullptr};
   if (bn3) a.x3 = bn3->x3, a.mask = bn3->mask, a.params = bn3->params;
   const int cus = std::max(1, planner_cus());
-  if (C == 64) {
+  if (fin) {
+    a.mean = fin->winner_mean, a.addend = fin->addend, a.xw = fin->winner_x, a.bits = fin->winner_bits;
+    a.dwpart = fin->dw_partials;
+    a.ntiles = (int)((M + 31) / 32);
+    a.npairs = cus;
+    if (bn3) hipLaunchKernelGGL((bwd1x1_fused_kernel<256, 32, 3, 1, true, true>), dim3(cus), dim3(THREADS), 0, st, a);
+    else hipLaunchKernelGGL((bwd1x1_fused_kernel<256, 32, 4, 1, false, true>), dim3(cus), dim3(THREADS), 0, st, a);
+    splitk_reduce(fin->dw_partials, std::min(cus, a.ntiles), (long)K * C, dw, accumulate, st);
+  } else if (C == 64) {
     a.ntiles = (int)((M + 63) / 64);
     a.npairs = cus;
     if (bn3) hipLaunchKernelGGL((bwd1x1_fused_kernel<256, 64, 2, 1, true>), dim3(cus), dim3(THREADS), 0, st, a);
diff --git a/k8s_amd/csrc/kernels/launchers.h b/k8s_amd/csrc/kernels/launchers.h
--- a/k8s_amd/csrc/kernels/launchers.h
+++ b/k8s_amd/csrc/kernels/launchers.h
@@ -72,6 +72,12 @@
                         float* dbeta, float* work, float* params, const uint16_t* x2, const float* mean2,
                         const float* invstd2, const float* gamma2, const float* beta2, uint16_t* dx2, float* dgamma2,
                         float* dbeta2, float* work2, float* params2, long M, int C, hipStream_t st);
+void launch_bn_bwd_dual_params(const uint16_t* dy, const uint8_t* mask, const uint16_t* x, const float* sums, int nrep,
+                               const float* mean, const float* invstd, const float* gamma, const float* beta,
+                               float* dgamma, float* dbeta, float* work, float* params, const uint16_t* x2,
+                               const float* sums2, const float* mean2, const float* invstd2, const float* gamma2,
+                               const float* beta2, float* dgamma2, float* dbeta2, float* work2, float* params2, long M,
+                               int C, hipStream_t st);
 void launch_bn_finalize_sums(const float* gamma, const float* beta, const float* sums, int nrep, float* save_mean,
                              float* save_invstd, float* run_mean, float* run_var, float* params, long M, int C,
                              float eps, float momentum, hipStream_t st);
@@ -206,11 +212,20 @@
   const uint8_t* mask = nullptr;
   const float* params = nullptr;
 };
+struct Bwd1x1Final {
+  const uint16_t* addend = nullptr;
+  const uint16_t* winner_x = nullptr;
+  const uint8_t* winner_bits = nullptr;
+  const float* winner_mean = nullptr;
+  float* dw_partials = nullptr;
+};
 bool bwd1x1_fused_ok(long M, int C, int K);
+bool bwd1x1_final_ok(long M, int C, int K);
+long bwd1x1_final_workspace(long M, int C, int K);
 void launch_bwd1x1_fused(const uint16_t* gy, const uint16_t* x, const uint16_t* w, const float* xform,
                          const float* gamma, const float* beta, const float* mean, const float* invstd, uint16_t* dz,
                          float* dw, float* sums, long M, int C, int K, bool accumulate, hipStream_t st,
-                         const Bwd1x1Bn3* bn3 = nullptr);
+                         const Bwd1x1Bn3* bn3 = nullptr, const Bwd1x1Final* fin = nullptr);
 void launch_conv_dgrad_wtrans(const uint16_t* w, uint16_t* w2, int K, int R, int S, int C, hipStream_t st);
 struct DgradTaps {
   int n[16];
diff --git a/k8s_amd/models/resnet.py b/k8s_amd/models/resnet.py
--- a/k8s_amd/models/resnet.py
+++ b/k8s_amd/models/resnet.py
@@ -34,8 +34,9 @@
         self.w = store.new(name + ".weight", (cout, k, k, cin), init_kaiming_normal(cin * k * k))
         self.stride, self.pad = stride, k // 2
 
-    def forward(self, x, grad_link=None):
-        return K.conv2d_nhwc(x, self.w, self.stride, self.pad, with_stats=True, grad_link=grad_link)
+    def forward(self, x, grad_link=None, bn3_link=None):
+        return K.conv2d_nhwc(x, self.w, self.stride, self.pad, with_stats=True, grad_link=grad_link,
+                             bn3_link=bn3_link)
 
 
 class Bottleneck(nn.Module):
@@ -60,23 +61,25 @@
         identity = self.down is None and x.requires_grad
         link = K.GradLink() if identity else None
         dlink = K.GradLink(shared=True) if (self.down is not None and x.requires_grad) else None
-        mlink = dn = None
+        mlink = dn = b3r = None
         if self.down is not None:
             mlink = K.MaskLink()
-            dn = self.down(x, grad_link=dlink)
+            b3r = K.Bn3Link() if self.training else None
+            dn = self.down(x, grad_link=dlink, bn3_link=b3r)
             fuse = K.BN_DUAL and isinstance(dn, tuple) and dn[1] is not None and self.training and dn[0].is_cuda
             if not fuse:
                 idn = self.down_bn(dn, relu=False, dy_link=mlink)
         t = self.conv1(x, grad_link=link or dlink)
         t = K.bn_relu_conv(t, self.bn1, self.conv2)
-        b3 = K.Bn3Link() if (self.down is None and self.training) else None
+        b3 = K.Bn3Link() if self.training else None
         t = K.bn_relu_conv(t, self.bn2, self.conv3, bn3_link=b3)
         if dn is not None and fuse:
-            y = K.bn_act_dual(t, self.bn3, dn, self.down_bn)
+            y = K.bn_act_dual(t, self.bn3, dn, self.down_bn, bn3_link=b3, bn3_link_r=b3r)
             if y is not None:
                 return y
             idn = self.down_bn(dn, relu=False, dy_link=mlink)
-        return self.bn3(t, residual=idn, relu=True, res_link=link or mlink, sub2=sub2, bn3_link=b3)
+        return self.bn3(t, residual=idn, relu=True, res_link=link or mlink, sub2=sub2,
+                        bn3_link=b3 if self.down is None else None)
 
 
 class ResNet(nn.Module):
diff --git a/k8s_amd/ops/conv.py b/k8s_amd/ops/conv.py
--- a/k8s_amd/ops/conv.py
+++ b/k8s_amd/ops/conv.py
@@ -13,8 +13,14 @@
 
 STATS = {"hip_fwd": 0, "aten_fwd": 0, "hip_wgrad": 0, "aten_wgrad": 0, "hip_dgrad": 0, "aten_dgrad": 0,
          "bn_bstats": 0, "hip_infer": 0, "aten_infer": 0,
-         "bn3_onload": 0, "bn3_apply": 0}
+         "bn3_onload": 0, "bn3_apply": 0,
+         "dual_onload": 0, "dual_apply": 0, "fused_final": 0}
 ROUTES = collections.Counter()
+
+
+def dual_onload_on() -> bool:
+    return all(os.environ.get(k, "1") != "0"
+               for k in ("K8S_AMD_DUAL_ONLOAD", "K8S_AMD_BN3_ONLOAD", "K8S_AMD_BWD1X1_FUSED"))
 
 
 
@@ -273,8 +279,13 @@
     return dx
 
 
-def _plan_bwd(C_, gy, x, w, stride, padding, addend, xform, bn_link):
-    K, R, S, C = w.shape
+def _plan_bwd(C_, gy, x, w, stride, padding, addend, xform, bn_link, dw_ok=True):
+    K, R, S, C = w.shape
+    if (xform is None and dw_ok and torch.is_tensor(addend) and addend.is_contiguous() and addend.shape == x.shape
+            and R == 1 and S == 1 and stride == 1 and padding == 0 and dual_onload_on()
+            and _link_kind(bn_link, x.shape) == "pool" and _hip(gy, x, w, addend) and gy.is_contiguous()
+            and x.is_contiguous() and C_.bwd1x1_final_ok(gy.numel() // K, C, K)):
+        return "fused_final"
     if (xform is not None and addend is None and R == 1 and S == 1 and stride == 1 and padding == 0
             and os.environ.get("K8S_AMD_BWD1X1_FUSED", "1") != "0" and _link_kind(bn_link, x.shape) == "relu"
             and bn_link.x.data_ptr() == x.data_ptr() and gy.is_contiguous() and x.is_contiguous()
@@ -301,9 +312,11 @@
 def conv_bwd(gy, x, w, stride, padding, need_dx, p=None, addend=None, xform=None, x_sub=None, bn_link=None, bn3=None):
     K, R, S, C = w.shape
     C_ = _load() if gy.is_cuda else None
+    dw_ok = p is not None and x_sub is None and p.grad.dtype == torch.float32
     if bn3 is not None and not (need_dx and bn3.covers(gy)
-                                and _plan_bwd(C_, gy, x, w, stride, padding, addend, xform, bn_link) == "fused_1x1"):
-        STATS["bn3_apply"] += 1
+                                and _plan_bwd(C_, gy, x, w, stride, padding, addend, xform, bn_link, dw_ok)
+                                in ("fused_1x1", "fused_final")):
+        STATS["dual_apply" if bn3.dual else "bn3_apply"] += 1
         gy = C_.bn_bwd_apply(gy.contiguous(), bn3.x3, bn3.mask, bn3.params)
         bn3 = None
     if x_sub is not None:
@@ -318,7 +331,20 @@
     if addend is not None and not torch.is_tensor(addend) and not (
             hip and stride == 1 and K % 8 == 0 and C % 8 == 0):
         addend = addend.materialize()
-    family = _plan_bwd(C_, gy, x, w, stride, padding, addend, xform, bn_link) if need_dx else None
+    family = _plan_bwd(C_, gy, x, w, stride, padding, addend, xform, bn_link, dw_ok) if need_dx else None
+    if family == "fused_final":
+        ROUTES[_plan_dgrad(C_, gy, w, padding, addend, bn_link)] += 1
+        STATS["fused_final"] += 1
+        STATS["hip_wgrad"] += 1
+        STATS["hip_dgrad"] += 1
+        sums = _bn_sums(C_, bn_link, C, gy.device)
+        onload = {} if bn3 is None else {"x3": bn3.x3.view(-1, K), "mask": bn3.mask, "params": bn3.params}
+        C_.bwd1x1_fused(gy.view(-1, K), x.view(-1, C), w.view(K, C), None, None, None, None, None, p.grad.view(K, C),
+                        sums, p.written, addend=addend.view(-1, C), winner_x=bn_link.x.view(-1, C),
+                        winner_bits=bn_link.mask.view(-1), winner_mean=bn_link.mean, **onload)
+        _slot_written(p)
+        bn_link.deposit(sums, None, addend)
+        return addend
     if family == "fused_1x1":
         ROUTES[family] += 1
         STATS["bn3_onload"] += bn3 is not None
diff --git a/k8s_amd/ops/nn.py b/k8s_amd/ops/nn.py
--- a/k8s_amd/ops/nn.py
+++ b/k8s_amd/ops/nn.py
@@ -142,10 +142,11 @@
 
 
 class Bn3Link:
-    __slots__ = ("y_key", "x3", "mask", "params", "dy_key")
+    __slots__ = ("y_key", "x3", "mask", "params", "dy_key", "dual")
 
     def __init__(self):
         self.y_key = self.x3 = self.mask = self.params = self.dy_key = None
+        self.dual = False
 
     def offer(self, y):
         self.y_key = (y.data_ptr(), tuple(y.shape))
@@ -153,8 +154,8 @@
     def offered(self, x) -> bool:
         return self.y_key == (x.data_ptr(), tuple(x.shape))
 
-    def fill(self, dy, x3, mask, params):
-        self.x3, self.mask, self.params, self.dy_key = x3, mask, params, BnStatLink._key(dy)
+    def fill(self, dy, x3, mask, params, dual=False):
+        self.x3, self.mask, self.params, self.dy_key, self.dual = x3, mask, params, BnStatLink._key(dy), dual
 
     def covers(self, t) -> bool:
         return self.dy_key == BnStatLink._key(t)
@@ -163,14 +164,14 @@
         if self.params is None:
             return None
         out = Bn3Link()
-        out.x3, out.mask, out.params, out.dy_key = self.x3, self.mask, self.params, self.dy_key
+        out.x3, out.mask, out.params, out.dy_key, out.dual = self.x3, self.mask, self.params, self.dy_key, self.dual
         self.x3 = self.mask = self.params = self.dy_key = None
         return out
 
 
 class _Conv2dNHWC(torch.autograd.Function):
     @staticmethod
-    def forward(ctx, x, anchor, p, stride, padding, with_stats, link=None, bn_link=None):
+    def forward(ctx, x, anchor, p, stride, padding, with_stats, link=None, bn_link=None, bn3_link=None):
         impl = _conv_impl()
         w = p.weight if x.dtype == p.weight.dtype else p.master.to(x.dtype)
         sums = None
@@ -188,6 +189,15 @@
         ctx.save_for_backward(x, xs)
         ctx.p, ctx.stride, ctx.padding, ctx.link, ctx.bn_link = p, stride, padding, link, bn_link
         ctx.x_requires_grad = x.requires_grad
+        ctx.bn3_link = None
+        K_, R, S, C = w.shape
+        if (bn3_link is not None and BN_BSTATS and R == 1 and S == 1 and stride == 1 and padding == 0 and xs is None
+                and link is not None and link.shared and x.requires_grad and x.is_contiguous()
+                and bn_link is not None and bn_link.kind == "pool" and bn_link.x.shape == x.shape
+                and impl._hip(x, w) and impl.dual_onload_on() and p.grad.dtype == torch.float32
+                and _C().bwd1x1_final_ok(x.numel() // C, C, K_)):
+            bn3_link.offer(y)
+            ctx.bn3_link = bn3_link
         if sums is not None:
             ctx.mark_non_differentiable(sums)
         ctx.set_materialize_grads(False)
@@ -200,22 +210,23 @@
         impl = _conv_impl()
         w = p.weight if x.dtype == p.weight.dtype else p.master.to(x.dtype)
         gy = gy.contiguous()
+        bn3 = ctx.bn3_link.take() if ctx.bn3_link is not None else None
         addend = None
         if ctx.link is not None:
             addend, ctx.link.grad = ctx.link.grad, None
             if addend is None and ctx.link.shared and ctx.x_requires_grad:
                 ctx.link.grad = impl.conv_bwd(gy, x, w, ctx.stride, ctx.padding, True, p, x_sub=xs,
-                                              bn_link=ctx.bn_link)
-                return None, None, None, None, None, None, None, None
+                                              bn_link=ctx.bn_link, bn3=bn3)
+                return None, None, None, None, None, None, None, None, None
         dx = impl.conv_bwd(gy, x, w, ctx.stride, ctx.padding, ctx.x_requires_grad, p, addend=addend, x_sub=xs,
-                           bn_link=ctx.bn_link)
-        return dx, None, None, None, None, None, None, None
+                           bn_link=ctx.bn_link, bn3=bn3)
+        return dx, None, None, None, None, None, None, None, None
 
 
 def conv2d_nhwc(x: torch.Tensor, p, stride: int = 1, padding: int = 0, with_stats: bool = False,
-                grad_link: "GradLink" = None):
+                grad_link: "GradLink" = None, bn3_link: "Bn3Link" = None):
     bn_link = getattr(x, "_k8s_bnstat", None)
-    y, sums = _Conv2dNHWC.apply(x, p.store.anchor, p, stride, padding, with_stats, grad_link, bn_link)
+    y, sums = _Conv2dNHWC.apply(x, p.store.anchor, p, stride, padding, with_stats, grad_link, bn_link, bn3_link)
     return (y, sums) if with_stats else y
 
 
@@ -933,7 +944,7 @@
 
     @staticmethod
     def forward(ctx, x, sums, xr, sums_r, anchor, pg, pb, run_mean, run_var, pgr, pbr, run_mean_r, run_var_r,
-                momentum, eps, stat_link=None):
+                momentum, eps, stat_link=None, bn3_link=None, bn3_link_r=None):
         x, xr = x.contiguous(), xr.contiguous()
         y, mean, invstd, mask, mean_r, invstd_r = _C().bn_fwd_from_sums_dual(
             x, sums, pg.master, pb.master, run_mean, run_var, xr, sums_r, pgr.master, pbr.master, run_mean_r,
@@ -943,6 +954,9 @@
         ctx.stat_link = stat_link
         if stat_link is not None:
             stat_link.fill_dual(x, mask, mean, xr, mean_r, pg.store)
+        ctx.bn3_links = None
+        if (bn3_link is not None and bn3_link_r is not None and bn3_link.offered(x) and bn3_link_r.offered(xr)):
+            ctx.bn3_links = (bn3_link, bn3_link_r)
         return y
 
     @staticmethod
@@ -954,7 +968,18 @@
         dg, db, finish = _bn_param_grads(pg, pb, x.device)
         dgr, dbr, finish_r = _bn_param_grads(pgr, pbr, x.device)
         pre = ctx.stat_link.take(dy) if ctx.stat_link is not None else None
-        if pre is not None and pre[1] is not None:
+        if pre is not None and pre[1] is None:
+            pre = None
+        if ctx.bn3_links is not None and _conv_impl().dual_onload_on():
+            params, params_r = C_.bn_bwd_dual_params(dy, mask, x, mean, invstd, pg.master, pb.master, dg, db,
+                                                     pre[0] if pre is not None else None, xr, mean_r, invstd_r,
+                                                     pgr.master, pbr.master, dgr, dbr,
+                                                     pre[1] if pre is not None else None)
+            ctx.bn3_links[0].fill(dy, x, mask, params, dual=True)
+            ctx.bn3_links[1].fill(dy, xr, mask, params_r, dual=True)
+            _conv_impl().STATS["dual_onload"] += 1
+            dx = dxr = dy
+        elif pre is not None:
             dx, dxr = C_.bn_bwd_dual_from_sums(dy, mask, x, mean, invstd, pg.master, pb.master, dg, db, pre[0], xr,
                                                mean_r, invstd_r, pgr.master, pbr.master, dgr, dbr, pre[1])
         else:
@@ -962,10 +987,10 @@
                                      pgr.master, pbr.master, dgr, dbr)
         finish()
         finish_r()
-        return (dx, None, dxr) + (None,) * 13
-
-
-def bn_act_dual(t, bn, tr, bn_r):
+        return (dx, None, dxr) + (None,) * 15
+
+
+def bn_act_dual(t, bn, tr, bn_r, bn3_link=None, bn3_link_r=None):
     if not BN_DUAL or not (isinstance(t, tuple) and isinstance(tr, tuple)):
         return None
     (x, sums), (xr, sums_r) = t, tr
@@ -975,7 +1000,7 @@
     link = BnStatLink() if BN_BSTATS else None
     y = _BnActDual.apply(x, sums, xr, sums_r, bn.gamma.store.anchor, bn.gamma, bn.beta, bn.running_mean,
                          bn.running_var, bn_r.gamma, bn_r.beta, bn_r.running_mean, bn_r.running_var, bn.momentum,
-                         bn.eps, link)
+                         bn.eps, link, bn3_link, bn3_link_r)
     if link is not None:
         y._k8s_bnstat = link
     return y
```
